# tsy935/eeg-gnn-ssl

Hardware: AMD Instinct MI355X
Metric: EEG clips/sec (60s, 19ch, K=2, 2-layer x64) fwd+bwd (higher is better)
Workload: dtype f32

## Files before the change

eeg_gnn_ssl_amd/_lib.py:

```python
from __future__ import annotations

import ctypes
import os
from ctypes import POINTER, c_char_p, c_float, c_int, c_int32, c_int64, c_size_t, c_void_p

_HERE = os.path.dirname(os.path.abspath(__file__))
HIP_LIB_PATH = os.path.join(_HERE, "libeeg_dcrnn_hip.so")
DEV_LIB_PATH = os.path.join(_HERE, "libeeg_dcrnn_hip_dev.so")
ABI_VERSION = 5


class LayerDims(ctypes.Structure):
    _fields_ = [("T", c_int32), ("B", c_int32), ("N", c_int32), ("H", c_int32), ("Fin", c_int32),
                ("M", c_int32), ("act", c_int32), ("p_batched", c_int32), ("x_planes_ready", c_int32),
                ("x_batch_major", c_int32), ("x_plane_stride", c_int64), ("pack3", c_void_p), ("spectral", c_void_p),
                ("spack", c_void_p)]


class DecoderDims(ctypes.Structure):
    _fields_ = [("T", c_int32), ("B", c_int32), ("N", c_int32), ("H", c_int32), ("Dout", c_int32),
                ("M", c_int32), ("L", c_int32), ("act", c_int32), ("p_batched", c_int32), ("dropout_p", c_float),
                ("teacher_on_device", c_int32)]


# ... 39 lines not shown
    "eeg_dcrnn_decoder_bwd_ws_floats": (c_size_t, [POINTER(DecoderDims)]),
    "eeg_dcrnn_decoder_is_persistent": (c_int, [POINTER(DecoderDims)]),
    "eeg_dcrnn_decoder_fwd": (c_int, [POINTER(DecoderDims), _FP, c_void_p, _FP, _FP, POINTER(c_void_p), _FP, _FP,
                                      _FP, _FP, _FP, _FP, c_void_p]),
    "eeg_dcrnn_decoder_bwd": (c_int, [POINTER(DecoderDims), c_void_p, _FP, POINTER(c_void_p), _FP, _FP, _FP, _FP, _FP,
                                      POINTER(c_void_p), POINTER(c_void_p), POINTER(c_void_p), POINTER(c_void_p),
                                      _FP, _FP, _FP, c_void_p]),
    "eeg_dcrnn_teacher_flags": (c_int, [_FP, _FP, c_int64, ctypes.c_double, c_int, _FP, c_void_p]),
    "eeg_dcrnn_fft_features_pair": (c_int, [_FP, _FP, c_int, c_int, c_int, c_int, c_int, _FP, _FP, c_float, c_float, _FP, _FP, _FP, c_void_p]),
    "eeg_dcrnn_augment_features": (c_int, [_FP, _FP, c_int, c_int, c_int, c_int, c_int, _FP, _FP, _FP, _FP, c_void_p]),
    "eeg_dcrnn_window_features": (c_int, [_FP, c_int, c_int, c_int, c_int, _FP, _FP, c_float, c_float, _FP, c_void_p]),
    "eeg_dcrnn_window_features_pair": (c_int, [_FP, _FP, c_int, c_int, c_int, c_int, c_int, _FP, _FP, c_float, c_float, _FP, _FP, c_void_p]),
    "eeg_dcrnn_augment_windows": (c_int, [_FP, _FP, c_int, c_int, c_int, c_int, c_int, _FP, _FP, _FP, _FP, _FP, c_void_p]),
    "eeg_dcrnn_corr_graph_rows_ws_floats": (c_size_t, [c_int, c_int, c_int]),
    "eeg_dcrnn_corr_graph_rows": (c_int, [_FP, c_int, c_int, c_int, c_int, ctypes.c_longlong, c_int, _FP, _FP, _FP, _FP, c_void_p]),
    "eeg_dcrnn_fft_features_len": (c_int, [_FP, c_int, c_int, c_int, c_int, _FP, _FP, c_float, c_float, _FP, c_float, _FP, _FP, c_void_p]),
    "eeg_dcrnn_window_features_len": (c_int, [_FP, c_int, c_int, c_int, c_int, _FP, _FP, c_float, c_float, _FP, c_float, _FP, c_void_p]),
    "eeg_dcrnn_corr_graph_len": (c_int, [_FP, c_int, c_int, c_int, c_int, c_int, _FP, _FP, _FP, _FP, _FP, c_void_p]),
    "eeg_dcrnn_corr_graph_rows_len": (c_int, [_FP, c_int, c_int, c_int, c_int, ctypes.c_longlong, c_int, _FP, c_int, _FP, _FP, _FP, _FP, c_void_p]),
    "eeg_dcrnn_augment_draw": (c_int, [_FP, c_int, c_int, _FP, _FP, _FP, _FP, _FP, _FP, c_int, _FP, c_void_p]),
    "eeg_dcrnn_epoch_keys": (c_int, [ctypes.c_uint64, c_int64, c_int64, _FP, c_void_p]),
    "eeg_dcrnn_gather_clips": (c_int, [_FP, _FP, c_size_t, _FP, _FP, c_size_t, _FP, _FP, c_int, _FP, _FP, _FP, c_int64, c_int64, _FP, c_int, c_int,
                                       c_int, c_void_p]),
    "eeg_dcrnn_gather_clips_tail": (c_int, [_FP, _FP, c_size_t, _FP, _FP, c_size_t, _FP, _FP, c_int, _FP, _FP, _FP, c_int64, c_int64, _FP, c_int, c_int,
                                            c_int, _FP, _FP, _FP, c_void_p]),
    "eeg_dcrnn_cls_head_loss_w": (c_int, [_FP, _FP, _FP, _FP, c_int, c_int, c_int, c_int, c_int, c_float, _FP, _FP, _FP, _FP, _FP, _FP, _FP, _FP, _FP,
                                          _FP, _FP, c_void_p]),
    "eeg_dcrnn_bce_logits_w": (c_int, [_FP, _FP, c_int, _FP, _FP, _FP, _FP, c_void_p]),
    "eeg_dcrnn_ce_logits_w": (c_int, [_FP, _FP, c_int, c_int, _FP, _FP, _FP, _FP, c_void_p]),
    "eeg_dcrnn_masked_loss_w": (c_int, [_FP, _FP, c_size_t, c_int, _FP, _FP, c_int, c_float, c_float, c_float, c_int, _FP, _FP, _FP, c_void_p]),
    "eeg_dcrnn_teacher_flags_dev": (c_int, [_FP, _FP, _FP, ctypes.c_double, c_int, _FP, c_void_p]),
    "eeg_dcrnn_pack_cells": (c_int, [c_int, POINTER(c_void_p), POINTER(c_void_p), POINTER(c_void_p), POINTER(c_void_p), POINTER(ctypes.c_int32),
                             c_int, c_int, POINTER(c_void_p), _FP, c_int, POINTER(c_void_p), c_void_p]),
    "eeg_dcrnn_cls_head_loss_ws_floats": (c_size_t, [c_int, c_int, c_int]),
    "eeg_dcrnn_cls_head_loss": (c_int, [_FP, _FP, _FP, _FP, c_int, c_int, c_int, c_int, c_int, c_float, _FP, _FP, _FP, _FP, _FP, _FP, _FP, _FP, _FP,
                                c_void_p]),
    "eeg_dcrnn_gather_last": (c_int, [_FP, _FP, c_int, c_int, c_int, _FP, c_void_p]),
    "eeg_dcrnn_rng_take": (c_int, [_FP, ctypes.c_uint64, _FP, c_void_p]),
    "eeg_dcrnn_cls_head_fwd": (c_int, [_FP, _FP, _FP, c_int, c_int, c_int, c_int, c_float, _FP, _FP, _FP, c_void_p]),
    "eeg_dcrnn_cls_head_bwd": (c_int, [_FP, _FP, _FP, _FP, c_int, c_int, c_int, c_int, c_float, _FP, _FP, _FP, _FP, c_void_p]),
    "eeg_dcrnn_dropout_mask": (c_int, [_FP, c_size_t, c_float, _FP, c_void_p]),
    "eeg_dcrnn_bce_logits": (c_int, [_FP, _FP, c_int, _FP, _FP, c_void_p]),
    "eeg_dcrnn_ce_logits": (c_int, [_FP, _FP, c_int, c_int, _FP, _FP, c_void_p]),
    "eeg_dcrnn_masked_loss_ws_floats": (c_size_t, []),
    "eeg_dcrnn_masked_loss": (c_int, [_FP, _FP, c_size_t, c_int, c_float, c_float, c_float, c_int, _FP, _FP, _FP, c_void_p]),
    "eeg_dcrnn_clip_adam_ws_floats": (c_size_t, []),
    "eeg_dcrnn_clip_adam": (c_int, [_FP, _FP, _FP, _FP, c_size_t, c_float, c_float, c_float, c_float, c_float, c_float,
                                    c_int, c_float, _FP, _FP, c_void_p]),
    "eeg_dcrnn_clip_adam_dev": (c_int, [_FP, _FP, _FP, _FP, c_size_t, c_float, _FP, c_float, c_float, c_float, c_float,
                                        _FP, c_float, _FP, _FP, c_void_p]),
}


_SIGNATURES_DEV = {
    "eeg_dcrnn_set_seq_probe": (c_int, [_FP]),
    "eeg_dcrnn_set_tuning": (c_int, [c_int, c_int]),
}


class EegDcrnnError(RuntimeError):
    """Raised when a library call reports an error (shape/dtype/launch problems)."""


class EegDcrnnLib:
    def __init__(self, path: str = HIP_LIB_PATH, strict: bool = True):
        if not os.path.exists(path):
            raise ImportError(
                f"{path} not found: the MI355X HIP library is not built. Run `python -c 'import "
                f"__graft_entry__ as g; g.build()'` (or `make -C eeg_gnn_ssl_amd/csrc`). There is no CPU fallback.")
        self.path = path
# ... 43 lines not shown
```

eeg_gnn_ssl_amd/csrc/api.cpp:

```cpp
#include <atomic>
#include <cmath>
#include <cstdarg>
#include <cstdio>
#include <cstring>

#include <string>
#include <vector>

#include "../../include/eeg_dcrnn.h"
#include "../../include/eeg_dcrnn_dev.h"
#include "../../include/eeg_dcrnn_prof.h"
#include "kernels_decoder.h"
#include "kernels_diffuse.h"
#include "kernels_data.h"
#include "kernels_feat.h"
#include "kernels_gemm.h"
#include "kernels_gemm_bf.h"
#include "kernels_graph.h"
#include "kernels_head.h"
#include "kernels_pack.h"
#include "spec_common.h"
#include "spec_launch.h"
#include "kernels_tail.h"
#include "prof.h"
// ... 345 lines not shown
    size_t rs = h_stride;
    if (rpl == nullptr) {
        if (diffuse_fwd(RHs, P, d->p_batched, S, d->B, N, H, M, rpl_ws, st)) return 1;
        rpl = rpl_ws;
        rs = (size_t)R * H;
    }
    SegPtrs sr;
    for (int m = 0; m < kMaxM; ++m) sr.p[m] = m == 0 ? RHs : (m < M ? rpl + (size_t)(m - 1) * rs : nullptr);
    if (w.pair) {
        if (launch_tnq_pair(w.thg.q, w.thc.q, sh, sr, M, H, R, dXW, 3 * H, 0, 2 * H, part_g, 2 * H, H, part_c, st, "gemm_tn_h"))
            return fail("gemm_tnq_pair: launch failed");
    } else {
        if (gemm_tn(w.thg, w.chg, sh, dXW, 3 * H, 0, part_g, st, "gemm_tn_hg")) return 1;
        if (gemm_tn(w.thc, w.chc, sr, dXW, 3 * H, 2 * H, part_c, st, "gemm_tn_hc")) return 1;
    }
    ReduceJobs jobs;
    const int Ks[3] = {M * Fin, M * H, M * H}, Os[3] = {3 * H, 2 * H, H}, ns[3] = {w.tx.nsplit, w.thg.nsplit, w.thc.nsplit};
    const float* parts[3] = {part, part_g, part_c};
    int nblocks = 0;
    for (int j = 0; j < 3; ++j) {
        jobs.part[j] = parts[j]; jobs.nsplit[j] = ns[j]; jobs.K[j] = Ks[j]; jobs.O[j] = Os[j];
        jobs.nblocks[j] = ceil_div(Ks[j] * Os[j], 64);
        nblocks += jobs.nblocks[j];
    }
    jobs.bias_part = bias_part; jobs.bias_B = d->B; jobs.dbg = dbg; jobs.dbc = dbc;
    if (bias_part != nullptr) nblocks += ceil_div(3 * H, 16);
    EEG_LAUNCH_P("reduce_unpack", reduce_unpack3_kernel, dim3(nblocks), dim3(256), 256 * sizeof(float4), st, jobs, acc, Fin, H, M, dWg, dWc);
    return check_launch("reduce_unpack");
}

size_t xs_spec(const eeg_layer_dims* d) { return d->x_plane_stride > 0 ? (size_t)d->x_plane_stride : 0; }
int cell_weight_grads_spectral(const eeg_layer_dims* d, const float* Xh, size_t x_gs, const float* hh, size_t hh_gs, const float* rhh,
                               const float* dYh, float* part, const BwdWs& w, float* dWg, float* dWc, hipStream_t st,
                               const float* bias_part, float* dbg, float* dbc) {
    const int S = d->T * d->B, H = d->H, M = d->M, Fin = d->Fin, N = d->N, Sp = spec_rows(S);
    float* part_g = part + (w.part_g - w.partial);
    float* part_c = part + (w.part_c - w.partial);
    const SpecTnPlan& g = w.gs;
    if (spec_plan_error("weight gradients (spectral)", g.error)) return 1;
    if (g.fused) {
        if (launch_tnf(g, Xh, x_gs, Fin, hh, hh_gs, rhh, dYh, Sp, N, part, part_g, part_c, st, "gemm_tn_f")) return fail("gemm_tnf: launch failed");
    } else {
        if (launch_tng(g, Xh, x_gs, Fin, Sp, N, dYh, part, st, "gemm_tn_x")) return fail("gemm_tng: launch failed");
        if (launch_tng_pair(g, hh, hh_gs, rhh, Sp, N, dYh, part_g, part_c, st, "gemm_tn_h")) return fail("gemm_tng_pair: launch failed");
    }
    ReduceJobs jobs{};
    SpecFoldJobs sj{};
    sj.basis = d->spectral; sj.N = N;
    sj.j[0] = SpecFoldJob{part, g.spg_x, Fin, 3 * H, ceil_div(Fin * 3 * H, 64)};
    sj.j[1] = SpecFoldJob{part_g, g.spg_h, H, 2 * H, ceil_div(H * 2 * H, 64)};
    sj.j[2] = SpecFoldJob{part_c, g.spg_h, H, H, ceil_div(H * H, 64)};
    int nblocks = sj.j[0].nblocks + sj.j[1].nblocks + sj.j[2].nblocks;
    jobs.bias_part = bias_part; jobs.bias_B = d->B; jobs.dbg = dbg; jobs.dbc = dbc;
    if (bias_part != nullptr) nblocks += ceil_div(3 * H, 16);
    const int ns_max = N * (g.spg_x > g.spg_h ? g.spg_x : g.spg_h);
    const size_t fold_lds = spec_fold_lds_bytes(M, ns_max);
    EEG_SET_MAX_LDS(reduce_unpack3s_kernel, fold_lds);
    EEG_LAUNCH_P("reduce_unpack", reduce_unpack3s_kernel, dim3(nblocks), dim3(256), fold_lds, st, jobs, sj, 0, Fin, H, M, dWg, dWc);
    return check_launch("reduce_unpack (spectral)");
}

int colsum_rows_per_chunk(int R) { int rpc = ceil_div(R, 512); return rpc < 64 ? 64 : rpc; }
size_t colsum_ws(int R, int C) { return (size_t)ceil_div(R, colsum_rows_per_chunk(R)) * C; }
int colsum(const float* A, int R, int C, int split, float* ws, float* out0, float* out1, hipStream_t st) {
    const int rpc = colsum_rows_per_chunk(R), nchunk = ceil_div(R, rpc);
    if (C % 4 == 0 && C <= 1024) {
        const int nrs = 256 / (C / 4);
        EEG_LAUNCH_P("reduce_bias", colsum_partial4_kernel, dim3(nchunk), dim3(256), (size_t)nrs * C * sizeof(float), st, A, R, C, rpc, ws);
    } else {
        EEG_LAUNCH_P("reduce_bias", colsum_partial_kernel, dim3(nchunk, ceil_div(C, 128)), dim3(256), 256 * sizeof(float), st, A, R, C, rpc, ws);
    }
    if (check_launch("colsum_partial")) return 1;
    EEG_LAUNCH_P("reduce_bias", colsum_final_kernel, dim3(ceil_div(C, 128)), dim3(128), 0, st, ws, nchunk, C, split, out0, out1);
    return check_launch("colsum_final");
}

struct DecLayout {
    size_t xin, proj_pack, proj_bias, hd, saved_total;
    size_t planes[8], hext[8], rs[8], us[8], cs[8], rhs[8], hpl[8], rpl[8];
    size_t dxw[8], dbias[8], dotot, da, dhn, z, partial, projt_pack, colsum, bwd_total;
    TnCall cp;
    TnPlan tp;
    BwdWs lw[8];
    eeg_layer_dims ld[8];
};
size_t align64(size_t v) { return (v + 63) / 64 * 64; }
DecLayout dec_layout(const eeg_decoder_dims* d) {
    DecLayout y;
    const size_t state = (size_t)d->B * d->N * d->H, R = (size_t)d->T * d->B * d->N;
    const int nct_o = ceil_div(d->Dout, 16), nct_h = ceil_div(d->H, 16);
    size_t o = 0;
// ... 171 lines not shown
    if (N < 1 || N > kMaxNodes || F < 4 || F % 4 != 0 || M < 1 || M > kMaxM) return fail("diffuse_adj: bad dims N=%d F=%d M=%d", N, F, M);
    if (S < 1 || B < 1) return fail("diffuse_adj: empty input (S=%d, B=%d)", S, B);
    return diffuse_adj(Z, P, p_batched, S, B, N, F, M, dX, S_(stream));
}

static bool layer_dims_positive(const eeg_layer_dims* d) {
    return d != nullptr && d->T >= 1 && d->B >= 1 && d->N >= 1 && d->H >= 1 && d->Fin >= 1 && d->M >= 1;
}
size_t eeg_dcrnn_layer_fwd_ws_floats(const eeg_layer_dims* d) {
    if (!layer_dims_positive(d)) return 0;
    const size_t xw = (size_t)d->T * d->B * d->N * 3 * d->H;
    return d->spectral != nullptr ? xw + (size_t)d->N * spec_rows(d->T * d->B) * 3 * d->H : xw;
}

size_t eeg_dcrnn_spectral_basis_floats(int N) { return (N >= 1 && N <= kMaxNodes) ? (size_t)spec_basis_floats(N) : 0; }
size_t eeg_dcrnn_spectral_rows(size_t S) { return (S + 15) / 16 * 16; }
int eeg_dcrnn_spectral_basis(const float* support, int N, float* basis, void* stream) {
    if (N < 2 || N > kMaxNodes) return fail("spectral_basis: num_nodes=%d unsupported (2..%d)", N, kMaxNodes);
    if (support == nullptr || basis == nullptr) return fail("spectral_basis: null pointer");
    if (launch_spec_basis(support, N, basis, S_(stream))) return fail("spectral_basis: launch failed");
    return check_launch("spectral_basis");
}
size_t eeg_dcrnn_spectral_pack_floats(int Fin, int H, int M, int N) {
    return (Fin >= 4 && Fin % 4 == 0 && H == 64 && M >= 1 && M <= kMaxM && N >= 1 && N <= kMaxNodes) ? spec_pack_floats(Fin, H, M, N) : 0;
}
int eeg_dcrnn_pack_cell_spectral(const float* Wg, const float* Wc, const float* basis, int Fin, int H, int M, int N, float* spack,
                                 void* stream) {
    if (eeg_dcrnn_spectral_pack_floats(Fin, H, M, N) == 0)
        return fail("pack_cell_spectral: input_dim=%d rnn_units=%d hop matrices=%d nodes=%d: the spectral form exists for 64 units", Fin, H, M, N);
    if (Wg == nullptr || Wc == nullptr || basis == nullptr || spack == nullptr) return fail("pack_cell_spectral: null pointer");
    if (launch_spec_pack(Wg, Wc, basis, Fin, H, M, N, spack, S_(stream))) return fail("pack_cell_spectral: launch failed");
    return check_launch("pack_cell_spectral");
}
int eeg_dcrnn_pack_cells(int n_cells, const float* const* Wg, const float* const* bg, const float* const* Wc, const float* const* bc,
                         const int32_t* Fin, int H, int M, float* const* packs, const float* basis, int N, float* const* spacks,
                         void* stream) {
    if (n_cells < 1 || n_cells > 4) return fail("pack_cells: %d cells (1..4 per launch)", n_cells);
    if (Wg == nullptr || bg == nullptr || Wc == nullptr || bc == nullptr || Fin == nullptr || packs == nullptr) return fail("pack_cells: null pointer table");
    if (!seq_h_supported(H)) return fail("pack_cells: rnn_units=%d unsupported", H);
    if (!seq_m_supported(M)) return fail("pack_cells: num hop matrices M=%d unsupported (1,2,3,4,5,7)", M);
    if ((basis == nullptr) != (spacks == nullptr)) return fail("pack_cells: the per-frequency packs need the basis block and their output table");
    int fin[4];
    for (int c = 0; c < n_cells; ++c) {
        fin[c] = Fin[c];
        if (fin[c] < 4 || fin[c] % 4 != 0) return fail("pack_cells: input dim %d of cell %d must be a positive multiple of 4", fin[c], c);
        if (Wg[c] == nullptr || bg[c] == nullptr || Wc[c] == nullptr || bc[c] == nullptr || packs[c] == nullptr || (spacks != nullptr && spacks[c] == nullptr))
            return fail("pack_cells: null pointer in the tables of cell %d", c);
        if (spacks != nullptr && eeg_dcrnn_spectral_pack_floats(fin[c], H, M, N) == 0)
            return fail("pack_cells: input_dim=%d rnn_units=%d hop matrices=%d nodes=%d: the spectral form exists for 64 units", fin[c], H, M, N);
    }
    if (launch_pack_cells(n_cells, Wg, bg, Wc, bc, fin, H, M, packs, basis, N, spacks, S_(stream))) return fail("pack_cells: launch failed");
    return check_launch("pack_cells");
}
int eeg_dcrnn_spectral_ok(const eeg_layer_dims* d, int need_dx) {
    if (!layer_dims_positive(d) || d->p_batched) return 0;
    if (d->x_planes_ready && d->Fin != d->H) return 0;
    if (check_dims(d->N, d->H, d->Fin, d->M)) return 0;
    return spec_supported(d->T, d->B, d->N, d->H, d->Fin, d->M, need_dx) ? 1 : 0;
}

int eeg_dcrnn_batch_major_ok(const eeg_layer_dims* d) {
    if (!diffuse_streams(d->p_batched, d->T * d->B, d->B, d->N, d->Fin)) return 0;
    const int R = d->T * d->B * d->N;
    const GemmKnobs k = gemm_knobs();
    return (nn_dma_applies(d->Fin, R, 3 * d->H, k) && tn_dma_applies(d->Fin, 3 * d->H, k)) ? 2 : 1;
}

int eeg_dcrnn_layer_fwd(const eeg_layer_dims* d, const float* X, float* Xtm, const float* h0, const float* P,
                        const float* pack, float* planes, float* Hext, float* Rs, float* Us, float* Cs, float* RHs,
                        float* Hplanes, float* RHplanes, float* ws, void* stream) {
    if (check_dims(d->N, d->H, d->Fin, d->M)) return 1;
    if (d->T < 1 || d->B < 1) return fail("layer_fwd: empty sequence/batch (T=%d, B=%d)", d->T, d->B);
    const bool save = Rs != nullptr;
    if (save != (Us != nullptr) || save != (Cs != nullptr) || save != (RHs != nullptr))
        return fail("layer_fwd: Rs/Us/Cs/RHs must be all NULL or all non-NULL");
    hipStream_t st = S_(stream);
    const int S = d->T * d->B, R = S * d->N, H = d->H, M = d->M, Fin = d->Fin;
    const size_t state = (size_t)d->B * d->N * H;
    CellPack p = make_cell_pack(Fin, H, M);
    if (h0 != nullptr && h0 != Hext && copy_floats(Hext, h0, state, st)) return 1;
    const size_t xs = d->x_plane_stride > 0 ? (size_t)d->x_plane_stride : (size_t)R * Fin;
    BtMap bt;
    if (d->x_batch_major) {
        if (Xtm != nullptr || d->x_planes_ready) return fail("layer_fwd: x_batch_major excludes Xtm and x_planes_ready");
        if (d->spectral == nullptr && eeg_dcrnn_batch_major_ok(d) != 2) return fail("layer_fwd: x_batch_major is not available for this shape (eeg_dcrnn_batch_major_ok)");
        bt.T = d->T; bt.B = d->B; bt.N = d->N;
    }
    float* XW = ws;
    if (d->spectral != nullptr) {
        if (!eeg_dcrnn_spectral_ok(d, 0)) return fail("layer_fwd: the spectral form does not cover this shape (eeg_dcrnn_spectral_ok)");
        if (Xtm != nullptr || d->spack == nullptr) return fail("layer_fwd: spectral excludes Xtm and needs spack");
        if ((Hplanes != nullptr) != (RHplanes != nullptr)) return fail("layer_fwd: Hplanes/RHplanes must be both NULL or both non-NULL");
        const SpecPack sp = make_spec_pack(Fin, H, M, d->N);
        const int N = d->N, Sp = spec_rows(S), SpE = d->B + Sp;
        const size_t xgs = d->x_plane_stride > 0 ? (size_t)d->x_plane_stride : (size_t)Sp * Fin;
        float* Yh = ws + (size_t)R * 3 * H;
        if (!d->x_planes_ready && spec_mix(1, X, d->spectral, N, d->T, d->B, Fin, d->x_batch_major ? 1 : 0, planes, st, "spec_mix_x")) return 1;
        const SpecNnPlan nn = spec_nn_plan(Fin, Sp, N, sp.nct_x, num_cus(), spec_knobs());
        if (spec_plan_error("layer_fwd (spectral x-part)", nn.error)) return 1;
        const bool regs = nn.kind == SpecNnKind::Regs;
        if (launch_spec_nn(nn, planes, xgs, Fin, Sp, N, d->spack + (regs ? sp.sxr : sp.sxq), regs ? sp.sxr_stride : sp.sxq_stride, Yh, st, "gemm_nn_xw",
                           pack + p.bias, d->spectral + spec_csum_offset(N))) return fail("gemm_nn (spectral): launch failed");
        SeqFwdArgs a{XW, h0 != nullptr ? Hext : nullptr, P, d->p_batched, pack + p.bhg, pack + p.bhc, Hext + state, Rs, Us, Cs, RHs, nullptr, nullptr,
                     (size_t)0, d->T, d->B, N, d->act, seq_probe_arg(st)};
        SeqCall call = seq_fwd_call(H, M, N, d->T, d->B, 0, a.probe);
        call.spectral = true; call.Sp = Sp; call.SpE = SpE;
        const SeqPlan plan = seq_fwd_plan(call);
        if (plan.kind == SeqKind::TwoWaveSpec) {
            a.XW = Yh; a.Hpl = Hplanes; a.RHpl = RHplanes; a.spec_U = d->spectral; a.spec_Sp = Sp; a.spec_SpE = SpE;
            if (seq_fwd(H, M, plan, a, st)) return 1;
            if (Hplanes != nullptr) {
                if (launch_spec_zero_rows(Hplanes, N, (d->T + 1) * d->B, SpE, H, st)) return fail("spec_zero_rows: launch failed");
                if (launch_spec_zero_pad(RHplanes, N, S, H, st)) return fail("spec_zero_pad: launch failed");
            }
        } else {
            if (spec_mix(0, Yh, d->spectral, N, d->T, d->B, 3 * H, 0, XW, st, "spec_mix_y")) return 1;
            if (seq_fwd(H, M, plan, a, st)) return 1;
            if (Hplanes != nullptr) {
                if (spec_mix(1, Hext, d->spectral, N, d->T + 1, d->B, H, 0, Hplanes, st, "spec_mix_h", SpE)) return 1;
                if (spec_mix(1, RHs, d->spectral, N, d->T, d->B, H, 0, RHplanes, st, "spec_mix_h")) return 1;
            }
        }
        return check_launch("layer_fwd (spectral)");
    } else if (d->x_planes_ready) {
        if (Xtm != nullptr) return fail("layer_fwd: x_planes_ready excludes a batch-major input");
    } else {
        if (diffuse_fwd(X, P, d->p_batched, S, d->B, d->N, Fin, M, planes, st, xs, d->x_batch_major ? 2 : (Xtm != nullptr ? 1 : 0), Xtm)) return 1;
        if (Xtm != nullptr) X = Xtm;
    }
    SegPtrs segs;
    for (int m = 0; m < kMaxM; ++m) segs.p[m] = m == 0 ? X : (m < M ? planes + (size_t)(m - 1) * xs : nullptr);
    const bool bf3 = d->pack3 != nullptr && pack3_supported(Fin, H, M);
    const Pack3 q = make_pack3(Fin, H, M);
    const NnCall cxw = nn_call(M, Fin, R, 3 * H / 16, 3 * H, 3 * H, bt, p.has_bxq, bf3 ? q.xw_nct : 0);
    if (gemm_nn(gemm_nn_plan(cxw), cxw, segs, NnRhs{pack + p.bx, pack + p.bxq, bf3 ? d->pack3 + q.xw : nullptr}, pack + p.bias, XW, st, "gemm_nn_xw", bt)) return 1;
    if ((Hplanes != nullptr) != (RHplanes != nullptr)) return fail("layer_fwd: Hplanes/RHplanes must be both NULL or both non-NULL");
    SeqFwdArgs a{XW, h0 != nullptr ? Hext : nullptr, P, d->p_batched, pack + p.bhg, pack + p.bhc, Hext + state, Rs, Us, Cs, RHs, Hplanes, RHplanes,
                 (size_t)(d->T + 1) * state, d->T, d->B, d->N, d->act, seq_probe_arg(st)};
    return seq_fwd(H, M, seq_fwd_plan(seq_fwd_call(H, M, d->N, d->T, d->B, a.plane_stride, a.probe)), a, st);
}

size_t eeg_dcrnn_layer_bwd_ws_floats(const eeg_layer_dims* d, int need_dx) { return layer_dims_positive(d) ? bwd_ws(d, need_dx).total : 0; }

int eeg_dcrnn_layer_bwd(const eeg_layer_dims* d, const float* X, const float* P, const float* pack,
                        const float* planes, const float* Hext, const float* Rs, const float* Us, const float* Cs,
                        const float* RHs, const float* Hplanes, const float* RHplanes, const float* dHseq,
// ... 11 lines not shown
    float* dbias = ws + w.dbias;
    SeqBwdArgs a{Hext + state, Hext, Rs, Us, Cs, dHseq, d_at_end, d_at_len,
                 reinterpret_cast<const long long*>(lengths), P, d->p_batched, pack + p.b1, pack + p.b2,
                 dXW, dh0, dbias, d->T, d->B, N, d->act, seq_probe_arg(st)};
    SeqCall call = seq_bwd_call(H, M, N, d->T, d->B, a.probe);
    call.spectral = d->spectral != nullptr; call.Sp = spec_rows(S); call.SpE = d->B + spec_rows(S);
    const SeqPlan plan = seq_bwd_plan(call);
    const bool dyh_done = plan.kind == SeqKind::TwoWaveSpec;
    if (dyh_done) { a.spec_U = d->spectral; a.dYh = ws + w.dyh; a.spec_Sp = call.Sp; }
    if (seq_bwd(H, M, plan, a, st)) return 1;
    const size_t xs = d->x_plane_stride > 0 ? (size_t)d->x_plane_stride : (size_t)R * Fin;
    BtMap bt;
    if (d->x_batch_major) {
        if (d->spectral == nullptr && eeg_dcrnn_batch_major_ok(d) != 2) return fail("layer_bwd: x_batch_major is not available for this shape");
        bt.T = d->T; bt.B = d->B; bt.N = N;
    }
    if (d->spectral != nullptr) {
        if (!eeg_dcrnn_spectral_ok(d, dX != nullptr)) return fail("layer_bwd: the spectral form does not cover this shape (eeg_dcrnn_spectral_ok)");
        if (d->spack == nullptr) return fail("layer_bwd: spectral needs spack");
        if ((Hplanes != nullptr) != (RHplanes != nullptr)) return fail("layer_bwd: Hplanes/RHplanes must be both NULL or both non-NULL");
        const SpecPack sp = make_spec_pack(Fin, H, M, N);
        const int Sp = spec_rows(S), SpE = d->B + Sp;
        float* dYh = ws + w.dyh;
        if (dyh_done) {
            if (launch_spec_zero_pad(dYh, N, S, 3 * H, st)) return fail("spec_zero_pad: launch failed");
        } else if (spec_mix(1, dXW, d->spectral, N, d->T, d->B, 3 * H, 0, dYh, st, "spec_mix_dy")) return 1;
        const float *hh = Hplanes, *rhh = RHplanes;
        size_t hh_gs = (size_t)SpE * H;
        if (hh == nullptr) {
            if (spec_mix(1, Hext, d->spectral, N, d->T, d->B, H, 0, ws + w.hplanes, st, "spec_mix_h")) return 1;
            if (spec_mix(1, RHs, d->spectral, N, d->T, d->B, H, 0, ws + w.rhplanes, st, "spec_mix_h")) return 1;
            hh = ws + w.hplanes; rhh = ws + w.rhplanes; hh_gs = 0;
        }
        if (cell_weight_grads_spectral(d, planes, xs_spec(d), hh, hh_gs, rhh, dYh, ws + w.partial, w, dWg, dWc, st, dbias, dbg, dbc)) return 1;
        if (dX != nullptr) {
            const SpecDxPlan dx = spec_dx_plan(Fin, N, d->T, d->B, num_cus(), spec_knobs());
            if (spec_plan_error("layer_bwd (spectral dX)", dx.error)) return 1;
            if (dx.kind == SpecDxKind::Fused) {
                if (launch_dxf(dx, dYh, Sp, S, N, d->spack + sp.sxtq, sp.sxtq_stride, d->spectral, dX, st, "gemm_dx_f")) return fail("gemm_dxf: launch failed");
            } else {
                float* dXh = ws + w.z;
                if (launch_spec_nn(dx.nn, dYh, 0, 3 * H, Sp, N, d->spack + sp.sxtq, sp.sxtq_stride, dXh, st, "gemm_nn_dx")) return fail("gemm_nng: launch failed");
                if (launch_spec_mix(dx.mix, dXh, d->spectral, N, d->T, d->B, Fin, 0, dX, st, "spec_mix_dx")) return fail("spec_mix: launch failed");
            }
        }
        return check_launch("layer_bwd (spectral)");
    }
    if (cell_weight_grads(d, X, planes, xs, Hext, RHs, dXW, P, Hplanes, RHplanes, (size_t)(d->T + 1) * state,
                          ws + w.hplanes, ws + w.rhplanes, ws + w.partial, w, false, dWg, dWc, st, bt, dbias, dbg, dbc)) return 1;
    if (dX != nullptr) {
        float* Z = ws + w.z;
        SegPtrs sd;
        for (int m = 0; m < kMaxM; ++m) sd.p[m] = m == 0 ? dXW : nullptr;
        const bool bf3 = d->pack3 != nullptr && pack3_supported(Fin, H, M);
        const Pack3 q = make_pack3(Fin, H, M);
        const NnCall cdx = nn_call(1, 3 * H, R, round_up(M * Fin, 16) / 16, M * Fin, M * Fin, BtMap(), p.has_bxtq, bf3 ? q.dx_nct : 0);
        if (gemm_nn(gemm_nn_plan(cdx), cdx, sd, NnRhs{pack + p.bxt, pack + p.bxtq, bf3 ? d->pack3 + q.dx : nullptr}, nullptr, Z, st, "gemm_nn_dx")) return 1;
        if (diffuse_adj(Z, P, d->p_batched, S, d->B, N, Fin, M, dX, st)) return 1;
    }
    return 0;
}


static int fft_features(const float* raw, int B, int N, int T, int W, const int32_t* perm, const float* log_scale, float mean, float std_,
                        const int64_t* lengths, float pad_val, float* feat_raw, float* feat_std, void* stream) {
    const long long* len = reinterpret_cast<const long long*>(lengths);
    if (B < 1 || N < 1 || T < 1) return fail("fft_features: empty input (B=%d, N=%d, T=%d)", B, N, T);
    if (W < 4 || W % 4 != 0 || W / 4 + 1 > 64) return fail("fft_features: window=%d unsupported (multiple of 4, <= 252)", W);
    if (feat_raw == nullptr && feat_std == nullptr) return fail("fft_features: no output requested");
    if (feat_std != nullptr && !(std_ != 0.f)) return fail("fft_features: std must be non-zero");
    if (W == kFftWin) {
        const long long n_windows = (long long)B * N * T;
// ... 661 lines not shown
        dz == nullptr || dW == nullptr || dbias == nullptr || loss == nullptr || ws == nullptr)
        return fail("cls_head_loss: null pointer");
    const int O = C * H + C, nblk = ceil_div(B, 4);
    const size_t lds = (size_t)(4 * cls_tail_wave_floats(N, H, C) + 4 * (O + 1)) * sizeof(float);
    if (lds > kMaxLdsBytes) return fail("cls_head_loss: N=%d x (classes=%d + rnn_units=%d) floats of four clips do not fit the %zu-byte LDS", N, C, H, (size_t)kMaxLdsBytes);
    if (clip_w != nullptr) {
        EEG_SET_MAX_LDS(cls_head_loss_w_kernel, lds);
        EEG_LAUNCH_P("cls_head_loss", cls_head_loss_w_kernel, dim3(nblk), dim3(256), lds, S_(stream), z, W, bias, targets, kind, B, N, H, C, drop,
                     reinterpret_cast<const unsigned long long*>(rng_used), clip_w, denom, logits, reinterpret_cast<int*>(arg), dlogits, dz, ws);
        if (check_launch("cls_head_loss_w")) return 1;
        EEG_LAUNCH_P("cls_head_loss", cls_head_loss_w_finish_kernel, dim3(1), dim3(256), 0, S_(stream), ws, nblk, denom, H, C, dW, dbias, loss);
        return check_launch("cls_head_loss_w_finish");
    }
    EEG_SET_MAX_LDS(cls_head_loss_kernel, lds);
    EEG_LAUNCH_P("cls_head_loss", cls_head_loss_kernel, dim3(nblk), dim3(256), lds, S_(stream), z, W, bias, targets, kind, B, N, H, C, drop,
                 reinterpret_cast<const unsigned long long*>(rng_used), logits, reinterpret_cast<int*>(arg), dlogits, dz, ws);
    if (check_launch("cls_head_loss")) return 1;
    EEG_LAUNCH_P("cls_head_loss", cls_head_loss_finish_kernel, dim3(1), dim3(256), 0, S_(stream), ws, nblk, B, H, C, dW, dbias, loss);
    return check_launch("cls_head_loss_finish");
}
int eeg_dcrnn_cls_head_loss(const float* z, const float* W, const float* bias, const void* targets, int kind, int B, int N, int H, int C,
                            float dropout_p, const uint64_t* rng_used, float* logits, int32_t* arg, float* dlogits, float* dz,
                            float* dW, float* dbias, float* loss, float* ws, void* stream) {
    return cls_head_loss_launch(z, W, bias, targets, kind, B, N, H, C, dropout_p, rng_used, nullptr, nullptr, logits, arg, dlogits, dz, dW, dbias,
                                loss, ws, stream);
}
int eeg_dcrnn_cls_head_loss_w(const float* z, const float* W, const float* bias, const void* targets, int kind, int B, int N, int H, int C,
                              float dropout_p, const uint64_t* rng_used, const float* clip_w, const float* denom, float* logits, int32_t* arg,
                              float* dlogits, float* dz, float* dW, float* dbias, float* loss, float* ws, void* stream) {
    if (clip_w == nullptr || denom == nullptr) return fail("cls_head_loss_w: null clip_w / denom");
    return cls_head_loss_launch(z, W, bias, targets, kind, B, N, H, C, dropout_p, rng_used, clip_w, denom, logits, arg, dlogits, dz, dW, dbias,
                                loss, ws, stream);
}
size_t eeg_dcrnn_dconv_fwd_ws_floats(int B, int N, int F, int M, int O) {
    if (B < 1 || N < 1 || F < 1 || M < 1 || O < 1) return 0;
    return (size_t)(M - 1) * B * N * F + (size_t)F * M * O;
}
int eeg_dcrnn_dconv_fwd(const float* X, const float* P, int p_batched, int B, int N, int F, int M,
                        const float* W, const float* bias, int O, float* out, float* ws, void* stream) {
    if (N < 1 || N > kMaxNodes || F < 4 || F % 4 != 0 || M < 1 || M > kMaxM) return fail("dconv_fwd: bad dims N=%d F=%d M=%d", N, F, M);
    if (B < 1) return fail("dconv_fwd: empty batch (B=%d)", B);
    if (O % 16 != 0) return fail("dconv_fwd: output_dim=%d must be a multiple of 16", O);
    hipStream_t st = S_(stream);
    float* planes = ws;
    float* pack = ws + (size_t)(M - 1) * B * N * F;
    if (diffuse_fwd(X, P, p_batched, B, B, N, F, M, planes, st)) return 1;
    EEG_LAUNCH_P("pack_dense", pack_dense_kernel, dim3(256), dim3(256), 0, st, W, F, M, O, pack);
    if (check_launch("pack_dense")) return 1;
    SegPtrs segs;
    for (int m = 0; m < kMaxM; ++m) segs.p[m] = m == 0 ? X : (m < M ? planes + (size_t)(m - 1) * B * N * F : nullptr);
    return gemm_nn(segs, M, F, B * N, pack, O / 16, bias, out, O, O, st);
}
size_t eeg_dcrnn_dconv_bwd_ws_floats(int B, int N, int F, int M, int O) {
    if (B < 1 || N < 1 || F < 1 || M < 1 || O < 1) return 0;
    const int R = B * N;
    const int nsplit = gemm_tn_plan(tn_call(M, F, R, O)).nsplit;
    return (size_t)(M - 1) * R * F + align64((size_t)nsplit * M * F * O) + align64((size_t)(O / 4) * (round_up(M * F, 16) / 16) * 64)
           + (size_t)R * M * F + align64(colsum_ws(R, O));
}
int eeg_dcrnn_dconv_bwd(const float* X, const float* P, int p_batched, int B, int N, int F, int M, const float* W, int O,
                        const float* dOut, float* dX, float* dW, float* dbias, float* ws, void* stream) {
    if (N < 1 || N > kMaxNodes || F < 4 || F % 4 != 0 || M < 1 || M > kMaxM) return fail("dconv_bwd: bad dims N=%d F=%d M=%d", N, F, M);
    if (B < 1) return fail("dconv_bwd: empty batch (B=%d)", B);
    if (O % 16 != 0 || O > 192) return fail("dconv_bwd: output_dim=%d must be a multiple of 16 (<= 192)", O);
    hipStream_t st = S_(stream);
    const int R = B * N;
// ... 130 lines not shown
```

eeg_gnn_ssl_amd/csrc/kernels_head.h:

```cpp
#pragma once
#include "common.h"

namespace eeg {

__device__ __forceinline__ f32x4 ld4g(const float* p) {
    const float4 v = *reinterpret_cast<const float4*>(p);
    return (f32x4){v.x, v.y, v.z, v.w};
}

__global__ void gather_last_kernel(const float* __restrict__ Htop, const long long* __restrict__ lengths,
                                   int T, int B, int NH, float* __restrict__ last) {
    const size_t total = (size_t)B * NH;
    for (size_t i = (size_t)blockIdx.x * blockDim.x + threadIdx.x; i < total; i += (size_t)gridDim.x * blockDim.x) {
        const int b = i / NH, e = i % NH;
        int t = (int)lengths[b] - 1;
        t = t < 0 ? 0 : (t >= T ? T - 1 : t);
        last[i] = Htop[((size_t)t * B + b) * NH + e];
    }
}

__global__ void cls_head_fwd_kernel(const float* __restrict__ z, const float* __restrict__ W,
                                    const float* __restrict__ bias, int B, int N, int H, int C, DropCfg drop,
                                    const unsigned long long* __restrict__ used, float* __restrict__ logits, int* __restrict__ arg) {
    EEG_DYN_SMEM(sm);
// ... 52 lines not shown
                                      const int* __restrict__ arg, int B, int N, int H, int C, DropCfg drop,
                                      const unsigned long long* __restrict__ used, float* __restrict__ dW,
                                      float* __restrict__ dbias) {
    EEG_DYN_SMEM(sm);
    const int o = threadIdx.x & 15, q = threadIdx.x >> 4;
    const int i = blockIdx.x * 16 + o;
    float s = 0.f;
    if (i < C * H) {
        const int c = i / H, h = i % H;
        for (int b = q; b < B; b += 16) {
            const int n = arg[(size_t)b * C + c];
            const size_t e = ((size_t)b * N + n) * H + h;
            s = fmaf(dlogits[(size_t)b * C + c], fmaxf(z[e], 0.f) * head_mask(drop, used, e), s);
        }
    } else if (i < C * H + C) {
        const int c = i - C * H;
        for (int b = q; b < B; b += 16) s += dlogits[(size_t)b * C + c];
    }
    sm[q * 16 + o] = s;
    __syncthreads();
    if (q == 0 && i < C * H + C) {
        float t = 0.f;
        for (int k = 0; k < 16; ++k) t += sm[k * 16 + o];
        if (i < C * H) dW[i] = t; else dbias[i - C * H] = t;
    }
}

__host__ __device__ inline int cls_tail_wave_floats(int N, int H, int C) { return N * C + N * H + 2 * C; }
template <bool kWeighted>
__device__ __forceinline__ void cls_head_loss_body(const float* __restrict__ z, const float* __restrict__ W, const float* __restrict__ bias,
                                                   const void* __restrict__ targets, int kind, int B, int N, int H, int C, const DropCfg& drop,
                                                   const unsigned long long* __restrict__ used, float* __restrict__ logits,
                                                   int* __restrict__ arg, float* __restrict__ dlogits, float* __restrict__ dz,
                                                   float* __restrict__ partial, const float* __restrict__ clip_w,
                                                   const float* __restrict__ denom) {
    EEG_DYN_SMEM(sm);
    const int w = threadIdx.x >> 6, lane = threadIdx.x & 63, b = blockIdx.x * 4 + w, O = C * H + C;
    float* nl = sm + w * cls_tail_wave_floats(N, H, C);
    float* zs = nl + N * C;
    float* dl = zs + N * H;
    int* ag = reinterpret_cast<int*>(dl + C);
    float* contrib = sm + 4 * cls_tail_wave_floats(N, H, C);
    const bool live = b < B;
    const int groups = N * H / 4;
    if (live) {
        const unsigned long long seed = drop.on ? used[0] : 0ull, off = drop.on ? used[1] : 0ull;
        for (int g = lane; g < groups; g += 64) {
            const size_t gg = (size_t)b * groups + g;
            const f32x4 v = ld4g(z + 4 * gg);
            f32x4 m = {1.f, 1.f, 1.f, 1.f};
            if (drop.on) m = dropout_mask4(seed, off, gg, drop.thr, drop.scale);
#pragma unroll
            for (int j = 0; j < 4; ++j) zs[4 * g + j] = fmaxf(v[j], 0.f) * m[j];
        }
        EEG_WAVE_SYNC();
        if (lane < N) {
            for (int c = 0; c < C; ++c) {
                float s = bias[c];
                for (int h = 0; h < H; ++h) s = fmaf(zs[lane * H + h], W[c * H + h], s);
                nl[lane * C + c] = s;
            }
        }
        EEG_WAVE_SYNC();
        for (int c = lane; c < C; c += 64) {
            float best = nl[c];
            int bi = 0;
            for (int q = 1; q < N; ++q)
                if (nl[q * C + c] > best) { best = nl[q * C + c]; bi = q; }
            logits[(size_t)b * C + c] = best;
            arg[(size_t)b * C + c] = bi;
            dl[c] = best;
            ag[c] = bi;
        }
        EEG_WAVE_SYNC();
        if (lane == 0) {
            float term;
            const float div = kWeighted ? denom[0] : (float)B;
            if (kWeighted && clip_w[b] == 0.f) {
                term = 0.f;
                for (int c = 0; c < C; ++c) dl[c] = 0.f;
            } else if (kind == 0) {
                const float v = dl[0], t = reinterpret_cast<const float*>(targets)[b];
// ... 27 lines not shown
#pragma unroll
            for (int j = 0; j < 4; ++j) o[j] = zs[4 * g + j] > 0.f ? o[j] * keep : 0.f;
            *reinterpret_cast<float4*>(dz + ((size_t)b * groups + g) * 4) = make_float4(o[0], o[1], o[2], o[3]);
        }
        for (int i = lane; i < O; i += 64) {
            float v;
            if (i < C * H) { const int c = i / H, h = i % H; v = dl[c] * zs[ag[c] * H + h]; }
            else v = dl[i - C * H];
            contrib[w * (O + 1) + i] = v;
        }
    }
    __syncthreads();
    const int nlive = B - blockIdx.x * 4 < 4 ? B - blockIdx.x * 4 : 4;
    for (int i = threadIdx.x; i <= O; i += blockDim.x) {
        float s = 0.f;
        for (int q = 0; q < nlive; ++q) s += contrib[q * (O + 1) + i];
        partial[(size_t)blockIdx.x * (O + 1) + i] = s;
    }
}
__global__ __launch_bounds__(256) void cls_head_loss_kernel(const float* __restrict__ z, const float* __restrict__ W, const float* __restrict__ bias,
                                                            const void* __restrict__ targets, int kind, int B, int N, int H, int C, DropCfg drop,
                                                            const unsigned long long* __restrict__ used, float* __restrict__ logits,
                                                            int* __restrict__ arg, float* __restrict__ dlogits, float* __restrict__ dz,
                                                            float* __restrict__ partial) {
    cls_head_loss_body<false>(z, W, bias, targets, kind, B, N, H, C, drop, used, logits, arg, dlogits, dz, partial, nullptr, nullptr);
}
__global__ __launch_bounds__(256) void cls_head_loss_w_kernel(const float* __restrict__ z, const float* __restrict__ W, const float* __restrict__ bias,
                                                              const void* __restrict__ targets, int kind, int B, int N, int H, int C, DropCfg drop,
                                                              const unsigned long long* __restrict__ used, const float* __restrict__ clip_w,
                                                              const float* __restrict__ denom, float* __restrict__ logits, int* __restrict__ arg,
                                                              float* __restrict__ dlogits, float* __restrict__ dz, float* __restrict__ partial) {
    cls_head_loss_body<true>(z, W, bias, targets, kind, B, N, H, C, drop, used, logits, arg, dlogits, dz, partial, clip_w, denom);
}
__device__ __forceinline__ void cls_head_loss_finish_body(const float* __restrict__ partial, int nblk, float div, int H, int C,
                                                          float* __restrict__ dW, float* __restrict__ dbias, float* __restrict__ loss) {
    const int O = C * H + C;
    for (int i = threadIdx.x; i <= O; i += blockDim.x) {
        float s = 0.f;
        int q = 0;
        for (; q + 8 <= nblk; q += 8) {
            float v[8];
#pragma unroll
            for (int u = 0; u < 8; ++u) v[u] = partial[(size_t)(q + u) * (O + 1) + i];
#pragma unroll
            for (int u = 0; u < 8; ++u) s += v[u];
        }
        for (; q < nblk; ++q) s += partial[(size_t)q * (O + 1) + i];
        if (i < C * H) dW[i] = s;
        else if (i < O) dbias[i - C * H] = s;
        else loss[0] = s / div;
    }
}
__global__ __launch_bounds__(256) void cls_head_loss_finish_kernel(const float* __restrict__ partial, int nblk, int B, int H, int C,
                                                                   float* __restrict__ dW, float* __restrict__ dbias, float* __restrict__ loss) {
    cls_head_loss_finish_body(partial, nblk, (float)B, H, C, dW, dbias, loss);
}
__global__ __launch_bounds__(256) void cls_head_loss_w_finish_kernel(const float* __restrict__ partial, int nblk, const float* __restrict__ denom,
                                                                     int H, int C, float* __restrict__ dW, float* __restrict__ dbias,
                                                                     float* __restrict__ loss) {
    cls_head_loss_finish_body(partial, nblk, denom[0], H, C, dW, dbias, loss);
}

__global__ void rng_take_kernel(unsigned long long* __restrict__ state, unsigned long long* __restrict__ used, unsigned long long groups) {
    if (blockIdx.x == 0 && threadIdx.x == 0) {
        const unsigned long long seed = state[0], off = state[1];
        used[0] = seed;
        used[1] = off;
        state[1] = off + groups;
    }
}
__device__ __forceinline__ void teacher_flags_body(unsigned long long* __restrict__ state, long long* __restrict__ seen, long long inc,
                                                   double decay_steps, int T, int* __restrict__ flags) {
    const unsigned long long seed = state[0], off = state[1];
    const long long n = seen[0];
    const double ratio = decay_steps / (decay_steps + exp((double)n / decay_steps));
    for (int t0 = 0; t0 < T; t0 += 4) {
        unsigned w[4];
        const unsigned long long c = off + (unsigned long long)(t0 >> 2);
        philox4x32_10((unsigned)c, (unsigned)(c >> 32), 0u, 0u, (unsigned)seed, (unsigned)(seed >> 32), w);
        for (int j = 0; j < 4 && t0 + j < T; ++j) flags[t0 + j] = ((double)w[j] * (1.0 / 4294967296.0) < ratio) ? 1 : 0;
    }
    state[1] = off + (unsigned long long)((T + 3) / 4);
    seen[0] = n + inc;
}
__global__ void teacher_flags_kernel(unsigned long long* __restrict__ state, long long* __restrict__ seen, long long inc,
                                     double decay_steps, int T, int* __restrict__ flags) {
    if (blockIdx.x != 0 || threadIdx.x != 0) return;
    teacher_flags_body(state, seen, inc, decay_steps, T, flags);
}
__global__ void teacher_flags_dev_kernel(unsigned long long* __restrict__ state, long long* __restrict__ seen, const long long* __restrict__ inc,
                                         double decay_steps, int T, int* __restrict__ flags) {
    if (blockIdx.x != 0 || threadIdx.x != 0) return;
    teacher_flags_body(state, seen, inc[0], decay_steps, T, flags);
// ... 22 lines not shown
```

eeg_gnn_ssl_amd/csrc/kernels_seq.h:

```cpp
#pragma once
#include "common.h"
#include "lds_diffuse.h"

namespace eeg {

constexpr int seq_nks(int N) { return N <= 20 ? 5 : 8; }
constexpr bool seq_has_two_wave(int H, int M, int nks) { return H == 64 && nks == 5 && M <= 3; }
constexpr bool seq_has_spec(int H, int M, int nks) { return seq_has_two_wave(H, M, nks) && M >= 2; }
constexpr bool seq_has_probe(int H, int M, int nks) { return kDevBuild && H == 64 && M == 3 && nks == 5; }
constexpr bool seq_has_stream(int H, int M) { return H == 64 && M <= 5; }

template <int H, int M>
struct SeqGeom {
    static constexpr int KA = M * H, KAP = lds_stride_x(KA), KS = KA / 4;
    static constexpr int KG = M * 2 * H, KGP = lds_stride_x(KG), KSG = KG / 4;
    static constexpr int NGT = 2 * H / 16, NCT = H / 16;
    static constexpr int GT = ceil_div(NGT, 4), CT = ceil_div(NCT, 4);
};
constexpr size_t seq_fwd_lds_floats(int H, int M) { return (size_t)(M - 1) * kPFloats + 2 * 32 * lds_stride_x(M * H); }
constexpr size_t seq_fwd2_lds_floats(int H, int M, bool spec) {
    return seq_fwd_lds_floats(H, M) + 16 * 64 + (spec ? 3 * 16 * 64 + 4 * 64 + 4 * (M * H / 4 / 4) * 256 : 0);
}
constexpr size_t seq_bwd_lds_floats(int H, int M, int rows) {
    return (size_t)(M - 1) * kPFloats + (size_t)rows * (lds_stride_x(M * H) + lds_stride_x(M * 2 * H));
// ... 478 lines not shown
        }
        pp.mark(5);
        if (t + 1 < T || Hpl != nullptr) diffuse_own(A, Hpl, t + 1);
        pp.mark(6);
    }
    }
    pp.dump(probe, 0);
}

template <int H, int M, int NKS, bool PROBE = false, bool SPEC = false>
__global__ __launch_bounds__(512, 1) void seq_fwd2_kernel(
    const float* __restrict__ XW, const float* __restrict__ h0, const float* __restrict__ P, int p_batched,
    const float* __restrict__ bhg, const float* __restrict__ bhc,
    float* __restrict__ Hseq, float* __restrict__ Rs, float* __restrict__ Us, float* __restrict__ Cs,
    float* __restrict__ RHs, float* __restrict__ Hpl, float* __restrict__ RHpl, size_t plane_stride,
    int T, int B, int N, int act, long long* probe, const float* __restrict__ spec_U = nullptr, int spec_Sp = 0, int spec_SpE = 0) {
    using G = SeqGeom<H, M>;
    PhaseProbe<PROBE> pp;
    pp.start();
    static_assert(G::CT == 1 && NKS == 5, "one column tile per wave, second node tile on the 4x4x1 MFMA");
    constexpr int KAP = G::KAP, KS = G::KS, NGT = G::NGT, NCT = G::NCT, UST = 64;
    EEG_DYN_SMEM(sm);
    float* Pl = sm;
    float* A = Pl + (M - 1) * kPFloats;
    float* A2 = A + 32 * KAP;
    const int tid = threadIdx.x, lane = tid & 63, wave8 = SPEC ? wave_uniform(tid >> 6) : (tid >> 6), role = wave8 >> 2, wave = wave8 & 3;
    const int lr = lane & 15, lg = lane >> 4;
    float* U = A2 + 32 * KAP;
    float* XR = U + 16 * UST;
    float* XC = XR + 16 * UST;
    float* XRr = XC + 2 * 16 * UST;
    float* W1L = XRr + 4 * 64;
    const bool save = Rs != nullptr;
    const int ct = wave;
    const wbuf_t bH = make_wbuf(Hseq), bR = make_wbuf(save ? Rs : Hseq), bU = make_wbuf(save ? Us : Hseq),
                 bC = make_wbuf(save ? Cs : Hseq), bRH = make_wbuf(save ? RHs : Hseq);

    float w0[1][KS], w1[1][KS];
#pragma unroll
    for (int ks = 0; ks < KS; ++ks) w0[0][ks] = bhg[((size_t)ks * NGT + (role == 0 ? ct : NCT + ct)) * 64 + lane];
    if (!SPEC || role == 0) {
#pragma unroll
        for (int ks = 0; ks < KS; ++ks) w1[0][ks] = bhc[((size_t)ks * NCT + ct) * 64 + lane];
    } else {
#pragma unroll
        for (int q = 0; q < KS / 4; ++q) {
            f32x4 v;
#pragma unroll
            for (int j = 0; j < 4; ++j) v[j] = bhc[((size_t)(4 * q + j) * NCT + ct) * 64 + lane];
            st4(W1L + (ct * (KS / 4) + q) * 256 + 4 * lane, v);
        }
    }
    auto clip = [&](const int b, auto ROLE_T) __attribute__((always_inline)) {
    constexpr int ROLE_C = decltype(ROLE_T)::value;
    __syncthreads();
    for (int e = tid; e < 2 * 32 * KAP; e += 512) A[e] = 0.f;
    lds_load_polys(Pl, P, p_batched ? b : 0, M, N);
    __syncthreads();
    if (h0 != nullptr) {
        for (int e = tid; e < N * H; e += 512) A[lds_sw(e / H, e % H, KAP)] = h0[(size_t)b * N * H + e];
    } else {
        for (int e = tid; e < N * H; e += 512) (Hseq - (size_t)B * N * H)[(size_t)b * N * H + e] = 0.f;
    }
    __syncthreads();

    const bool valid[2] = {lr < N, 16 + lr < N};
// ... 32 lines not shown
        cs.begin(probe, cs_me);
        constexpr int QSA = KS / 4 / M;
        f32x4 rc[5] = {zero4, zero4, zero4, zero4, zero4};
        f32x4 ra = zero4;
        bool pre_r = false;
        for (int t = 0; t < T; ++t) {
            const size_t s = (size_t)t * B + b;
            f32x4 ar[1][2] = {{nxr0, (f32x4){nxr1, 0.f, 0.f, 0.f}}}, ac[1][2] = {{nxc, zero4}};
            const unsigned so = (unsigned)(s * N * H);
            EEG_LDS_BARRIER();
            pp.mark(0);
            if constexpr (SPEC) {
                ar[0][0] = ld4(XR + lds_sw(lr, col, UST));
                ar[0][1][0] = XRr[ct * 64 + lane];
                if (M > 1 && pre_r) ra += ar[0][0];
            }

            if (M > 1 && pre_r) {
                ar[0][0] = ra;
                mfma_nodes32<1, KS, true, 0, 0, false, true, true, (M > 1 ? QSA : 0)>(A, KAP, lane, lr, lg, w0, ar, rc);
            } else
                mfma_nodes32<1, KS, true, 0, 0, false, true, true>(A, KAP, lane, lr, lg, w0, ar);
            pp.mark(1);
            {
                const f32x4 rg = sigmoid4_(ar[0][0]);
                f32x4 rh = rg * ld4(A + lds_sw(lr, col, KAP));
                rh = valid[0] ? rh : zero4;
                st4(A2 + lds_sw(lr, col, KAP), rh);
                const float rg1 = sigmoidf_(ar[0][1][0]);
                const float rh1 = valid1 ? rg1 * A[l1] : 0.f;
                A2[l1] = rh1;
                if (save && valid[0]) {
                    wbuf_st4(bR, oh0, so, rg);
                    wbuf_st4(bRH, oh0, so, rh);
                }
                if (save && valid1) {
                    wbuf_st1(bR, oh1, so, rg1);
                    wbuf_st1(bRH, oh1, so, rh1);
                }
            }
            pp.mark(2);
            diffuse_own(A2, RHpl, t);
            pp.mark(7);
            EEG_LDS_BARRIER();
            pp.mark(3);
            if (t + 1 < T) fetch_xw(t + 1);
            if constexpr (SPEC) ac[0][0] = ld4(XC + (t & 1) * (16 * UST) + lds_sw(lr, col, UST));
            mfma_nodes32<1, KS, true, 1>(A2, KAP, lane, lr, lg, w1, ac);
            pp.mark(4);
            {
                const f32x4 u = ld4(U + lds_sw(lr, col, UST)), h = ld4(A + lds_sw(lr, col, KAP));
                const f32x4 c = act == 0 ? tanh4_(ac[0][0]) : relu4_(ac[0][0]);
                f32x4 hn = u * h + (1.f - u) * c;
                hn = valid[0] ? hn : zero4;
                st4(A + lds_sw(lr, col, KAP), hn);
                if (valid[0]) {
                    wbuf_st4(bH, oh0, so, hn);
                    if (save) wbuf_st4(bC, oh0, so, c);
                }
            }
            pp.mark(5);
            EEG_LDS_BARRIER();
            if (t + 1 < T || (!SPEC && Hpl != nullptr)) diffuse_own(A, Hpl, t + 1);
            pre_r = M > 1 && t + 1 < T;
            if (pre_r) {
                ra = SPEC ? zero4 : nxr0;
                rc[0] = rc[1] = rc[2] = rc[3] = rc[4] = zero4;
                f32x4 rr4[4] = {zero4, zero4, zero4, zero4};
                mfma_tile_quads<KS, 0, QSA>(A, KAP, lane, lr, lg, w0[0], ra, rc[4], rr4);
                rc[0] = rr4[0]; rc[1] = rr4[1]; rc[2] = rr4[2]; rc[3] = rr4[3];
            }
// ... 690 lines not shown
```

eeg_gnn_ssl_amd/csrc/kernels_spectral.h:

```cpp
#pragma once
#include "spec_common.h"
#include "spec_launch.h"

namespace eeg {

__global__ __launch_bounds__(256) void spectral_basis_kernel(const float* __restrict__ S, int N, float* __restrict__ out) {
    EEG_DYN_SMEM(sm);
    double* A = reinterpret_cast<double*>(sm);
    double* V = A + 32 * 32;
    double* cs = V + 32 * 32;
    int* pq = reinterpret_cast<int*>(cs + 32);
    double* red = reinterpret_cast<double*>(pq + 32);
    const int tid = threadIdx.x;
    const int NP = (N + 1) & ~1, NH = NP / 2;
    for (int e = tid; e < 32 * 32; e += 256) {
        const int i = e >> 5, j = e & 31;
        A[e] = (i < N && j < N) ? 0.5 * ((double)S[i * N + j] + (double)S[j * N + i]) : 0.0;
        V[e] = i == j ? 1.0 : 0.0;
    }
    __syncthreads();
    for (int sweep = 0; sweep < kSpecSweeps; ++sweep) {
        for (int r = 0; r < NP - 1; ++r) {
            if (tid < NH) {
                int p = tid == 0 ? NP - 1 : (r + tid) % (NP - 1);
// ... 211 lines not shown
#pragma unroll
        for (int v = 0; v < 16; ++v) acc[v] = bv;
        if (r < S) {
            float b[KS];
#pragma unroll
            for (int ks = 0; ks < KS; ++ks) {
                int k = 2 * ks + hh;
                if (k >= N) k = N - 1;
                b[ks] = DIR == 0 ? in[(s * N + k) * F + fc] : in[((size_t)k * Sp + r) * F + fc];
            }
#pragma unroll
            for (int ks = 0; ks < KS; ++ks) acc = mfma32(a[ks], b[ks], acc);
        }
        if (f < F) {
#pragma unroll
            for (int v = 0; v < 16; ++v) {
                const int o = 8 * (v >> 2) + 4 * hh + (v & 3);
                if (2 * KS <= 8 * (v >> 2)) continue;
                if (o < N) {
                    if (DIR == 0) out[((size_t)o * Sp + r) * F + f] = acc[v];
                    else out[(s * N + o) * F + f] = acc[v];
                }
            }
        }
    }
}

__global__ void spec_zero_pad_kernel(float* __restrict__ Xh, int N, int S, int Sp, int F) {
    const int per = (Sp - S) * F, total = N * per;
    for (int e = blockIdx.x * blockDim.x + threadIdx.x; e < total; e += gridDim.x * blockDim.x) {
        const int i = e / per, r = e - i * per;
        Xh[((size_t)i * Sp + S) * F + r] = 0.f;
    }
}

__global__ __launch_bounds__(256) void spec_mix_generic_kernel(const float* __restrict__ in, const float* __restrict__ basis,
                                                              const float* __restrict__ bias, int N, int S, int Sp, int F, int map,
                                                              int T, int B, int to_nodes, float* __restrict__ out) {
    EEG_DYN_SMEM(sm);
    for (int e = threadIdx.x; e < N * N; e += blockDim.x) sm[e] = basis[e];
    __syncthreads();
    const int F4 = F / 4;
    const size_t total = (size_t)(to_nodes ? Sp : S) * N * F4;
    for (size_t e = (size_t)blockIdx.x * blockDim.x + threadIdx.x; e < total; e += (size_t)gridDim.x * blockDim.x) {
        const int c4 = (int)(e % F4), o = (int)((e / F4) % N);
        const size_t r = e / ((size_t)F4 * N);
        const size_t s = r < (size_t)S ? spec_sample(r, map, T, B) : r;
        float4 a = make_float4(0.f, 0.f, 0.f, 0.f);
        if (to_nodes) {
            if (r < (size_t)S) {
                for (int n = 0; n < N; ++n) {
                    const float u = sm[n * N + o];
                    const float4 x = reinterpret_cast<const float4*>(in)[(s * N + n) * F4 + c4];
                    a.x = fmaf(u, x.x, a.x); a.y = fmaf(u, x.y, a.y); a.z = fmaf(u, x.z, a.z); a.w = fmaf(u, x.w, a.w);
                }
            }
            reinterpret_cast<float4*>(out)[((size_t)o * Sp + r) * F4 + c4] = a;
        } else {
            if (bias != nullptr) a = reinterpret_cast<const float4*>(bias)[c4];
            for (int i = 0; i < N; ++i) {
                const float u = sm[o * N + i];
                const float4 y = reinterpret_cast<const float4*>(in)[((size_t)i * Sp + r) * F4 + c4];
                a.x = fmaf(u, y.x, a.x); a.y = fmaf(u, y.y, a.y); a.z = fmaf(u, y.z, a.z); a.w = fmaf(u, y.w, a.w);
            }
            reinterpret_cast<float4*>(out)[(s * N + o) * F4 + c4] = a;
        }
// ... 5 lines not shown
```

eeg_gnn_ssl_amd/csrc/pack_cell.h:

```cpp
#pragma once
#include "common.h"
#include "nnq_order.h"

namespace eeg {

struct CellPack {
    int Fin, H, M;
    size_t bx;
    size_t bias;
    size_t bhg;
    size_t bhc;
    size_t b1;
    size_t b2;
    size_t bxt;
    size_t c1;
    size_t c2;
    size_t bxq;
    size_t bxtq;
    bool has_bxq, has_bxtq;
    size_t total;
};

__host__ __device__ inline CellPack make_cell_pack(int Fin, int H, int M) {
    CellPack p;
    p.Fin = Fin; p.H = H; p.M = M;
    size_t o = 0;
    p.bx = o;   o += (size_t)M * Fin * 3 * H;
    p.bias = o; o += (size_t)round_up(3 * H, 64);
    p.bhg = o;  o += (size_t)M * H * 2 * H;
    p.bhc = o;  o += (size_t)M * H * H;
    p.b1 = o;   o += (size_t)M * H * H;
    p.b2 = o;   o += (size_t)M * 2 * H * H;
    p.bxt = o;  o += (size_t)3 * H * round_up(M * Fin, 16);
    p.c1 = o;   o += (size_t)M * H * cell_pack_cx_cols(Fin, H);
    p.c2 = o;   o += (size_t)M * 2 * H * cell_pack_cx_cols(Fin, H);
    p.has_bxq = (3 * H) % 192 == 0;
    p.has_bxtq = (M * Fin) % 192 == 0 && (3 * H) % 4 == 0 && make_nnq_order(1, 3 * H).ntail <= 2;
    p.bxq = o;  o += p.has_bxq ? (size_t)round_up(make_nnq_order(M, Fin).nch, 4) * (3 * H / 16) * 256 : 0;
    p.bxtq = o; o += p.has_bxtq ? (size_t)make_nnq_order(1, 3 * H).nch * (M * Fin / 16) * 256 : 0;
    p.total = o;
    return p;
}

__device__ __forceinline__ float ref_wg(const float* Wg, int M, int H, int f_all, int m, int o) {
    return Wg[((size_t)f_all * M + m) * (2 * H) + o];
}
__device__ __forceinline__ float ref_wc(const float* Wc, int M, int H, int f_all, int m, int o) {
    return Wc[((size_t)f_all * M + m) * H + o];
}

__device__ __forceinline__ void pack_cell_body(const float* __restrict__ Wg, const float* __restrict__ bg,
                                               const float* __restrict__ Wc, const float* __restrict__ bc,
                                               float* __restrict__ out, const CellPack& p, int bid, int nb) {
    const int Fin = p.Fin, H = p.H, M = p.M;
    const size_t stride = (size_t)nb * blockDim.x;
    for (size_t idx = (size_t)bid * blockDim.x + threadIdx.x; idx < p.total; idx += stride) {
        float v = 0.f;
        if (idx < p.bias) {
            const size_t e = idx - p.bx;
            const int lane = e & 63, nct = 3 * H / 16;
            const int ct = (e >> 6) % nct, ks = (e >> 6) / nct;
            const int k = 4 * ks + (lane >> 4), j = 16 * ct + (lane & 15);
            const int m = k / Fin, f = k % Fin;
            v = j < 2 * H ? ref_wg(Wg, M, H, f, m, j) : ref_wc(Wc, M, H, f, m, j - 2 * H);
        } else if (idx < p.bhg) {
            const int j = idx - p.bias;
            v = j < 2 * H ? bg[j] : (j < 3 * H ? bc[j - 2 * H] : 0.f);
        } else if (idx < p.bhc) {
            const size_t e = idx - p.bhg;
            const int lane = e & 63, nct = 2 * H / 16;
            const int ct = (e >> 6) % nct, ks = (e >> 6) / nct;
            const int k = kperm(ks, lane >> 4), j = 16 * ct + (lane & 15);
            v = ref_wg(Wg, M, H, Fin + k % H, k / H, j);
        } else if (idx < p.b1) {
            const size_t e = idx - p.bhc;
            const int lane = e & 63, nct = H / 16;
            const int ct = (e >> 6) % nct, ks = (e >> 6) / nct;
            const int k = kperm(ks, lane >> 4), j = 16 * ct + (lane & 15);
            v = ref_wc(Wc, M, H, Fin + k % H, k / H, j);
        } else if (idx < p.b2) {
            const size_t e = idx - p.b1;
            const int lane = e & 63, nct = H / 16;
            const int ct = (e >> 6) % nct, ks = (e >> 6) / nct;
            const int k = kperm(ks, lane >> 4), f = 16 * ct + (lane & 15);
            v = ref_wc(Wc, M, H, Fin + f, k / H, k % H);
        } else if (idx < p.bxt) {
            const size_t e = idx - p.b2;
            const int lane = e & 63, nct = H / 16;
            const int ct = (e >> 6) % nct, ks = (e >> 6) / nct;
// ... 40 lines not shown
```

eeg_gnn_ssl_amd/csrc/platform.h:

```cpp
#pragma once
#include <hip/hip_runtime.h>

typedef float f32x4 __attribute__((ext_vector_type(4)));
typedef float f32x2 __attribute__((ext_vector_type(2)));
#define EEG_DYN_SMEM(name) extern __shared__ __attribute__((aligned(16))) float name[]
#define EEG_LAUNCH(kern, grid, block, smem, stream, ...) \
    hipLaunchKernelGGL(kern, (grid), (block), (smem), (stream), __VA_ARGS__)
#define EEG_SET_MAX_LDS(kern, bytes) \
    (void)hipFuncSetAttribute(reinterpret_cast<const void*>(kern), hipFuncAttributeMaxDynamicSharedMemorySize, (int)(bytes))
__device__ __forceinline__ f32x4 mfma16(float a, float b, f32x4 c) {
    return __builtin_amdgcn_mfma_f32_16x16x4f32(a, b, c, 0, 0, 0);
}
__device__ __forceinline__ f32x4 mfma4(float a, float b, f32x4 c) {
    return __builtin_amdgcn_mfma_f32_4x4x1f32(a, b, c, 0, 0, 0);
}
typedef float f32x16 __attribute__((ext_vector_type(16)));
__device__ __forceinline__ f32x16 mfma32(float a, float b, f32x16 c) {
    return __builtin_amdgcn_mfma_f32_32x32x2f32(a, b, c, 0, 0, 0);
}
typedef short bf16x8 __attribute__((ext_vector_type(8)));
typedef unsigned u32x4 __attribute__((ext_vector_type(4)));
__device__ __forceinline__ f32x4 mfma_bf16(bf16x8 a, bf16x8 b, f32x4 c) {
    return __builtin_amdgcn_mfma_f32_16x16x32_bf16(a, b, c, 0, 0, 0);
}
// ... 39 lines not shown
    const unsigned long long v = reinterpret_cast<unsigned long long>(p);
    const unsigned lo = __builtin_amdgcn_readfirstlane((unsigned)v), hi = __builtin_amdgcn_readfirstlane((unsigned)(v >> 32));
    return __builtin_amdgcn_make_buffer_rsrc(reinterpret_cast<void*>(((unsigned long long)hi << 32) | lo), 0,
                                             (int)__builtin_amdgcn_readfirstlane(nbytes), 0x00020000);
}
__device__ __forceinline__ float wbuf_ld(wbuf_t b, unsigned voff, unsigned soff) {
    return __builtin_bit_cast(float, __builtin_amdgcn_raw_buffer_load_b32(b, 4u * voff, 4u * soff, 0));
}
__device__ __forceinline__ f32x4 wbuf_ld4(wbuf_t b, unsigned voff, unsigned soff) {
    return __builtin_bit_cast(f32x4, __builtin_amdgcn_raw_buffer_load_b128(b, 4u * voff, 4u * soff, 0));
}
__device__ __forceinline__ void wbuf_st4(wbuf_t b, unsigned voff, unsigned soff, f32x4 v) {
    typedef unsigned u32x4_ __attribute__((ext_vector_type(4)));
    __builtin_amdgcn_raw_buffer_store_b128(__builtin_bit_cast(u32x4_, v), b, 4u * voff, 4u * soff, 0);
}
template <int AUX>
__device__ __forceinline__ void wbuf_st4_aux(wbuf_t b, unsigned voff, unsigned soff, f32x4 v) {
    typedef unsigned u32x4_ __attribute__((ext_vector_type(4)));
    __builtin_amdgcn_raw_buffer_store_b128(__builtin_bit_cast(u32x4_, v), b, 4u * voff, 4u * soff, AUX);
}
__device__ __forceinline__ void wbuf_st2(wbuf_t b, unsigned voff, unsigned soff, float x, float y) {
    typedef unsigned u32x2_ __attribute__((ext_vector_type(2)));
    __builtin_amdgcn_raw_buffer_store_b64((u32x2_){__builtin_bit_cast(unsigned, x), __builtin_bit_cast(unsigned, y)}, b, 4u * voff, 4u * soff, 0);
}
__device__ __forceinline__ void wbuf_st1(wbuf_t b, unsigned voff, unsigned soff, float x) {
    __builtin_amdgcn_raw_buffer_store_b32(__builtin_bit_cast(unsigned, x), b, 4u * voff, 4u * soff, 0);
}
__device__ __forceinline__ void wbuf_dma16(wbuf_t b, float* lds_wave_base, unsigned voff_bytes, unsigned soff_bytes) {
    __builtin_amdgcn_raw_ptr_buffer_load_lds(b, (__attribute__((address_space(3))) void*)lds_wave_base, 16, voff_bytes, soff_bytes, 0, 0);
}

__device__ __forceinline__ unsigned long long atomic_add_u64(unsigned long long* p, unsigned long long v) { return atomicAdd(p, v); }

namespace eeg {
__device__ __forceinline__ float fast_exp(float x) { return __builtin_amdgcn_exp2f(x * 1.44269504088896340736f); }
__device__ __forceinline__ float fast_rcp(float x) { return __builtin_amdgcn_rcpf(x); }
__device__ __forceinline__ float fast_exp2(float x) { return __builtin_amdgcn_exp2f(x); }
__device__ __forceinline__ float fast_log2(float x) { return __builtin_amdgcn_logf(x); }
__device__ __forceinline__ float unfused_mul_add(float a, float b, float c) {
#pragma clang fp contract(off)
    const float p = a * b;
    return p + c;
}

constexpr int kPlatformIsDevice = 1;
inline int platform_num_cus() {
    static int n = 0;
    if (n == 0) {
        int dev = 0, v = 0;
        if (hipGetDevice(&dev) == hipSuccess && hipDeviceGetAttribute(&v, hipDeviceAttributeMultiprocessorCount, dev) == hipSuccess && v > 0) n = v;
        else n = 256;
    }
    return n;
}
inline bool platform_copy_floats(float* dst, const float* src, size_t n, hipStream_t st) {
    return hipMemcpyAsync(dst, src, n * sizeof(float), hipMemcpyDeviceToDevice, st) == hipSuccess;
}
inline bool platform_stream_is_capturing(hipStream_t st) {
    hipStreamCaptureStatus cs = hipStreamCaptureStatusNone;
    return hipStreamIsCapturing(st, &cs) == hipSuccess && cs != hipStreamCaptureStatusNone;
}
}
```

eeg_gnn_ssl_amd/csrc/spec_inst.cpp:

```cpp
#include "kernels_gemm_g.h"
#include "kernels_gemm_f.h"
#include "kernels_spectral.h"
#include "pack_cell.h"
#include "spec_launch.h"
#include "prof.h"

namespace eeg {

constexpr int kMaxPackJobs = 8;
struct PackJob {
    const float *Wg, *bg, *Wc, *bc, *basis;
    float* out;
    int spectral;
    CellPack cp;
    SpecPack sp;
};
struct PackJobs { PackJob j[kMaxPackJobs]; };
__global__ void pack_cells_kernel(PackJobs jobs) {
    const PackJob& jb = jobs.j[blockIdx.y];
    if (jb.spectral) pack_spectral_body(jb.Wg, jb.Wc, jb.basis, jb.out, jb.sp, (int)blockIdx.x, (int)gridDim.x);
    else pack_cell_body(jb.Wg, jb.bg, jb.Wc, jb.bc, jb.out, jb.cp, (int)blockIdx.x, (int)gridDim.x);
}


size_t spec_pack_floats(int Fin, int H, int M, int N) { return make_spec_pack(Fin, H, M, N).total; }

int launch_spec_basis(const float* S, int N, float* basis, hipStream_t st) {
    EEG_SET_MAX_LDS(spectral_basis_kernel, kSpecBasisLds);
    EEG_LAUNCH_P("spec_basis", spectral_basis_kernel, dim3(1), dim3(256), kSpecBasisLds, st, S, N, basis);
    return hipGetLastError() == hipSuccess ? 0 : 2;
}

int launch_spec_pack(const float* Wg, const float* Wc, const float* basis, int Fin, int H, int M, int N, float* spack, hipStream_t st) {
    const SpecPack p = make_spec_pack(Fin, H, M, N);
    EEG_LAUNCH_P("pack_cell", pack_spectral_kernel, dim3(1024), dim3(256), 0, st, Wg, Wc, basis, spack, p);
    return hipGetLastError() == hipSuccess ? 0 : 2;
}

int launch_pack_cells(int n_cells, const float* const* Wg, const float* const* bg, const float* const* Wc, const float* const* bc,
                      const int* Fin, int H, int M, float* const* packs, const float* basis, int N, float* const* spacks, hipStream_t st) {
    PackJobs jobs{};
    int n = 0;
    for (int c = 0; c < n_cells; ++c) {
        if (n + (spacks != nullptr ? 2 : 1) > kMaxPackJobs) return 1;
        PackJob& a = jobs.j[n++];
        a.Wg = Wg[c]; a.bg = bg[c]; a.Wc = Wc[c]; a.bc = bc[c]; a.basis = nullptr; a.out = packs[c]; a.spectral = 0;
        a.cp = make_cell_pack(Fin[c], H, M);
        if (spacks != nullptr) {
            PackJob& b = jobs.j[n++];
            b.Wg = Wg[c]; b.bg = nullptr; b.Wc = Wc[c]; b.bc = nullptr; b.basis = basis; b.out = spacks[c]; b.spectral = 1;
            b.sp = make_spec_pack(Fin[c], H, M, N);
        }
    }
    EEG_LAUNCH_P("pack_cell", pack_cells_kernel, dim3(256, n), dim3(256), 0, st, jobs);
    return hipGetLastError() == hipSuccess ? 0 : 2;
}

int launch_spec_mix(const SpecMixPlan& p, const float* in, const float* basis, int N, int T, int B, int F, int bm, float* out,
                    hipStream_t st, const char* tag) {
    const float* bias = nullptr;
    const dim3 grid(p.grid), block(p.block);
#define EEG_MIX_MFMA(DIR, KS) EEG_LAUNCH_P(tag, (spec_mix_mfma_kernel<DIR, KS>), grid, block, p.lds, st, in, basis, bias, N, p.S, p.Sp, F, bm, T, B, out)
    if (p.kind == SpecMixKind::Mfma) {
        if (p.ks == 10) { if (p.to_nodes) EEG_MIX_MFMA(0, 10); else EEG_MIX_MFMA(1, 10); }
        else { if (p.to_nodes) EEG_MIX_MFMA(0, 16); else EEG_MIX_MFMA(1, 16); }
    } else if (p.kind == SpecMixKind::Valu19) {
        if (p.to_nodes) EEG_LAUNCH_P(tag, spec_mix_in_kernel<19>, grid, block, p.lds, st, in, basis, p.S, p.Sp, F, bm, T, B, out);
        else EEG_LAUNCH_P(tag, spec_mix_out_kernel<19>, grid, block, p.lds, st, in, basis, bias, p.S, p.Sp, F, bm, T, B, out);
    } else {
        EEG_LAUNCH_P(tag, spec_mix_generic_kernel, grid, block, p.lds, st, in, basis, bias, N, p.S, p.Sp, F, bm, T, B, p.to_nodes, out);
    }
#undef EEG_MIX_MFMA
    return hipGetLastError() == hipSuccess ? 0 : 2;
}

int launch_spec_zero_rows(float* Xh, int N, int S, int Sp, int F, hipStream_t st) {
    if (Sp <= S) return 0;
    EEG_LAUNCH_P("zero", spec_zero_pad_kernel, dim3(ceil_div(N * (Sp - S) * F, 256)), dim3(256), 0, st, Xh, N, S, Sp, F);
    return hipGetLastError() == hipSuccess ? 0 : 2;
}

namespace {
template <int KQ, bool SWZ>
void launch_nnf_one(const SpecNnPlan& p, const float* A, size_t ags, int K, int Sp, int G, const float* Wr, size_t wstride, float* C, hipStream_t st,
                    const char* tag, const float* bias, const float* gscale) {
    EEG_SET_MAX_LDS((gemm_nnf_kernel<KQ, SWZ>), p.lds);
    EEG_LAUNCH_P(tag, (gemm_nnf_kernel<KQ, SWZ>), dim3(p.grid), dim3(p.block), p.lds, st, A, (long long)ags, K, Sp, G, Wr, (unsigned)wstride, C, bias, gscale);
}
template <int NJ>
void launch_nng_one(const SpecNnPlan& p, const float* A, size_t ags, int F, int Sp, int G, const float* Wq, size_t wstride, float* C, hipStream_t st,
                    const char* tag, const float* bias, const float* gscale) {
    EEG_SET_MAX_LDS((gemm_nng_kernel<NJ, 2>), p.lds);
    EEG_LAUNCH_P(tag, (gemm_nng_kernel<NJ, 2>), dim3(p.grid), dim3(p.block), p.lds, st, A, (unsigned)ags, F, Sp, G, Wq, (unsigned)wstride, C, 64 * NJ, bias, gscale);
}
}
int launch_spec_nn(const SpecNnPlan& p, const float* A, size_t a_gstride, int K, int Sp, int G, const float* W, size_t wstride, float* C,
                   hipStream_t st, const char* tag, const float* bias, const float* gscale) {
    const size_t ags = a_gstride != 0 ? a_gstride : (size_t)Sp * K;
#define EEG_NNF(KQ, SWZ) launch_nnf_one<KQ, SWZ>(p, A, ags, K, Sp, G, W, wstride, C, st, tag, bias, gscale)
    if (p.kind == SpecNnKind::Regs) {
        switch (p.kq) {
            case 8: EEG_NNF(8, true); break;
            case 13: EEG_NNF(13, false); break;
            case 9: EEG_NNF(9, false); break;
            case 5: EEG_NNF(5, false); break;
            case 2: EEG_NNF(2, false); break;
            default: return 1;
        }
    } else if (p.nj == 3) {
        launch_nng_one<3>(p, A, ags, K, Sp, G, W, wstride, C, st, tag, bias, gscale);
    } else if (p.nj == 1) {
// ... 77 lines not shown
```

eeg_gnn_ssl_amd/csrc/spec_launch.h:

```cpp
#pragma once
#include "common.h"
#include "nnq_order.h"
#include "spec_common.h"

namespace eeg {

struct SpecKnobs {
    int nn_grouped = 0;
    int tn_separate = 0;
    int dx_passes = 0;
};
enum SpecPlanError { kSpecOk = 0, kSpecBadNct, kSpecNotCovered };

inline bool spec_desc_reaches(double floats) { return floats * sizeof(float) < 2147483648.0; }

inline bool spec_supported(int T, int B, int N, int H, int Fin, int M, int need_dx) {
    if (T < 1 || B < 1 || N < 2 || N > kMaxNodes || H != 64 || Fin < 4 || Fin % 4 != 0 || M < 2 || M > kMaxM) return false;
    if (need_dx && Fin != 64) return false;
    if (Fin / 4 > 256 || make_nnq_order(1, Fin).ntail > 1) return false;
    return spec_desc_reaches((double)N * spec_rows(T * B) * (Fin > 192 ? Fin : 192));
}

constexpr size_t kSpecBasisLds = (2 * 32 * 32 + 32 + 256) * sizeof(double) + 32 * sizeof(int);
__host__ __device__ constexpr size_t spec_mix_generic_lds_bytes(int N) { return (size_t)N * N * sizeof(float); }
// ... 154 lines not shown
    int nt;
    int grid, block;
    size_t lds;
    bool needs_dxh;
    SpecNnPlan nn;
    SpecMixPlan mix;
    int error;
};
inline SpecDxPlan spec_dx_plan(int Fin, int N, int T, int B, int num_cus, const SpecKnobs& k) {
    SpecDxPlan p{};
    const int S = T * B, Sp = spec_rows(S);
    if (k.dx_passes == 0 && Fin == 64 && N >= 1 && N <= kDxfMaxN && S >= 1 && spec_desc_reaches((double)Sp * 192) &&
        spec_desc_reaches((double)S * N * 64)) {
        p.kind = SpecDxKind::Fused;
        p.nt = N == 19 ? 19 : 0;
        p.grid = ceil_div(Sp, kDxfRows); p.block = 256;
        p.lds = dxf_lds_bytes();
        return p;
    }
    p.kind = SpecDxKind::TwoPass;
    p.needs_dxh = true;
    SpecKnobs grouped = k;
    grouped.nn_grouped = 1;
    p.nn = spec_nn_plan(192, Sp, N, round_up(Fin, 16) / 16, num_cus, grouped);
    p.mix = spec_mix_plan(0, N, T, B, Fin);
    p.error = p.nn.error;
    return p;
}

size_t spec_pack_floats(int Fin, int H, int M, int N);
int launch_spec_basis(const float* S, int N, float* basis, hipStream_t st);
int launch_spec_pack(const float* Wg, const float* Wc, const float* basis, int Fin, int H, int M, int N, float* spack, hipStream_t st);
int launch_pack_cells(int n_cells, const float* const* Wg, const float* const* bg, const float* const* Wc, const float* const* bc,
                      const int* Fin, int H, int M, float* const* packs, const float* basis, int N, float* const* spacks, hipStream_t st);
int launch_spec_mix(const SpecMixPlan& p, const float* in, const float* basis, int N, int T, int B, int F, int bm, float* out,
                    hipStream_t st, const char* tag);
int launch_spec_zero_rows(float* Xh, int N, int S, int Sp, int F, hipStream_t st);
inline int launch_spec_zero_pad(float* Xh, int N, int S, int F, hipStream_t st) { return launch_spec_zero_rows(Xh, N, S, spec_rows(S), F, st); }
int launch_spec_nn(const SpecNnPlan& p, const float* A, size_t a_gstride, int K, int Sp, int G, const float* W, size_t wstride, float* C,
                   hipStream_t st, const char* tag, const float* bias = nullptr, const float* gscale = nullptr);
int launch_tnf(const SpecTnPlan& p, const float* Xh, size_t x_gstride, int Fin, const float* Hh, size_t h_gstride, const float* RHh,
               const float* dY, int Sp, int G, float* part_x, float* part_g, float* part_c, hipStream_t st, const char* tag);
int launch_tng(const SpecTnPlan& p, const float* A, size_t a_gstride, int F, int Sp, int G, const float* dY, float* partial, hipStream_t st,
               const char* tag);
int launch_tng_pair(const SpecTnPlan& p, const float* Ah, size_t ah_gstride, const float* Arh, int Sp, int G, const float* dY, float* part_g,
                    float* part_c, hipStream_t st, const char* tag);
int launch_dxf(const SpecDxPlan& p, const float* dYh, int Sp, int S, int N, const float* Wtq, size_t wstride, const float* basis, float* dX,
               hipStream_t st, const char* tag);

}
```

eeg_gnn_ssl_amd/model/cell.py:

```python
import math

import torch
import torch.nn as nn

from .. import ops


class DiffusionGraphConv(nn.Module):

    def __init__(self, num_supports, input_dim, hid_dim, num_nodes, max_diffusion_step, output_dim,
                 bias_start=0.0, filter_type="laplacian"):
        super().__init__()
        self._num_matrices = num_supports * max_diffusion_step + 1
        self._input_size = input_dim + hid_dim
        self._input_dim = input_dim
        self._hid_dim = hid_dim
        self._num_nodes = num_nodes
        self._max_diffusion_step = max_diffusion_step
        self._filter_type = filter_type
        self.weight = nn.Parameter(torch.empty(self._input_size * self._num_matrices, output_dim))
        self.biases = nn.Parameter(torch.empty(output_dim))
        nn.init.xavier_normal_(self.weight, gain=1.414)
        nn.init.constant_(self.biases, bias_start)

# ... 17 lines not shown
        self._num_nodes = num_nodes
        self._num_units = num_units
        self._input_dim = input_dim
        self._max_diffusion_step = max_diffusion_step
        self._use_gc_for_ru = use_gc_for_ru
        if not use_gc_for_ru:
            raise NotImplementedError("use_gc_for_ru=False is a stub (`_fc` is `pass`) in the reference as well")
        if max_diffusion_step < 0:
            raise ValueError("max_diffusion_step must be >= 0")
        self._num_supports = 2 if filter_type == "dual_random_walk" else 1
        self._filter_type = filter_type
        common = dict(num_supports=self._num_supports, input_dim=input_dim, hid_dim=num_units,
                      num_nodes=num_nodes, max_diffusion_step=max_diffusion_step, filter_type=filter_type)
        self.dconv_gate = DiffusionGraphConv(output_dim=num_units * 2, **common)
        self.dconv_candidate = DiffusionGraphConv(output_dim=num_units, **common)

    @property
    def output_size(self):
        return self._num_nodes * self._num_units

    @property
    def num_matrices(self):
        return self._num_supports * self._max_diffusion_step + 1

    def _check_supports(self, supports):
        if len(supports) != self._num_supports:
            raise RuntimeError(f"filter_type={self._filter_type!r} expects {self._num_supports} support(s), "
                               f"got {len(supports)}")
        n = self._num_nodes
        for i, s in enumerate(supports):
            if s.dim() not in (2, 3) or s.shape[-1] != n or s.shape[-2] != n:
                raise RuntimeError(f"supports[{i}] has shape {tuple(s.shape)}, expected ({n}, {n}) or (B, {n}, {n})")

    def run_sequence(self, x, h0, p, p_batched, lengths=None, x_off=0, x_planes=None, want_hsel=True, basis=None, pack=None, spack=None):
        return ops.dcgru_layer_ex(x, x_off, h0, p, p_batched, self.dconv_gate.weight, self.dconv_gate.biases,
                                  self.dconv_candidate.weight, self.dconv_candidate.biases,
                                  self._num_nodes, self._num_units, self.num_matrices,
                                  self._activation_name, lengths, x_planes, want_hsel, basis, pack, spack)

    def forward(self, supports, inputs, state):
        self._check_supports(supports)
        b = inputs.shape[0]
        p, p_batched = ops.hop_polys(supports, self._max_diffusion_step, b)
        x = inputs.reshape(1, b, self._num_nodes, self._input_dim)
        new_state = self.run_sequence(x, state, p, p_batched).hsel
        return new_state, new_state

    def init_hidden(self, batch_size):
        return torch.zeros(batch_size, self._num_nodes * self._num_units,
                           device=self.dconv_gate.weight.device)
```

eeg_gnn_ssl_amd/model/model.py:

```python
import random

import torch
import torch.nn as nn

from .. import ops
from .. import utils
from .cell import DCGRUCell


class _FusedDropout:

    def _init_dropout_rng(self, stream_id: int):
        self.register_buffer("_dropout_rng", ops.make_rng_state("cpu", stream_id), persistent=False)
        self._ddp_params_and_buffers_to_ignore = ["_dropout_rng"]

    def _drop_p(self) -> float:
        return float(self.dropout.p) if self.training else 0.0

    def set_dropout_seed(self, seed: int, offset: int = 0):
        st = self._dropout_rng
        st.copy_(torch.tensor([int(seed), int(offset)], dtype=torch.int64), non_blocking=False)

    def dropout_rng_state(self):
        seed, offset = self._dropout_rng.tolist()
        return int(seed), int(offset)

    def _rng_state(self, device) -> torch.Tensor:
        st = self._dropout_rng
        device = torch.device(device)
        if st.device.type != device.type or (device.index is not None and st.device.index != device.index):
            if device.type == "cuda" and torch.cuda.is_current_stream_capturing():
                raise RuntimeError("the fused dropout generator state is not on the device of the inputs: move the model "
                                   "with .to(device) before capturing its forward into a HIP graph")
            st = st.to(device)
            self._buffers["_dropout_rng"] = st
        return st


class DCRNNEncoder(nn.Module):

    def __init__(self, input_dim, max_diffusion_step, hid_dim, num_nodes, num_rnn_layers,
                 dcgru_activation=None, filter_type="laplacian", device=None):
        super().__init__()
        self.hid_dim = hid_dim
        self.num_rnn_layers = num_rnn_layers
        self.num_nodes = num_nodes
        self.max_diffusion_step = max_diffusion_step
        self._device = device
        cells = []
        for layer in range(num_rnn_layers):
            cells.append(DCGRUCell(input_dim=input_dim if layer == 0 else hid_dim, num_units=hid_dim,
                                   max_diffusion_step=max_diffusion_step, num_nodes=num_nodes,
                                   nonlinearity=dcgru_activation, filter_type=filter_type))
        self.encoding_cells = nn.ModuleList(cells)

    def run(self, inputs, initial_hidden_state, supports, lengths=None, want_finals=True):
        t_len, b = inputs.shape[0], inputs.shape[1]
        self.encoding_cells[0]._check_supports(supports)
        p, p_batched = ops.hop_polys(supports, self.max_diffusion_step, b)
        basis = ops.shared_spectral_basis(supports, self.max_diffusion_step)
        cur, x_off, planes = inputs.reshape(t_len, b, self.num_nodes, -1), 0, None
        finals, top_sel, out = [], None, None
        packs = ops.pack_encoder_cells(self.encoding_cells, basis, self.num_nodes)
        for layer, cell in enumerate(self.encoding_cells):
            h0 = None if initial_hidden_state is None else initial_hidden_state[layer]
            is_top = layer == self.num_rnn_layers - 1
            out = cell.run_sequence(cur, h0, p, p_batched, lengths if is_top else None, x_off, planes,
                                    want_hsel=want_finals or (is_top and lengths is not None), basis=basis,
                                    pack=None if packs is None else packs[0][layer], spack=None if packs is None else packs[1][layer])
            if is_top and lengths is not None:
                top_sel = out.hsel
                finals.append(out.hext[t_len] if want_finals else None)
            else:
                finals.append(out.hsel if want_finals else None)
            cur, x_off, planes = out.hext.view(t_len + 1, b, self.num_nodes, self.hid_dim), 1, out.hpl
        return (torch.stack(finals, dim=0) if want_finals else None), out.hseq, top_sel

    def forward(self, inputs, initial_hidden_state, supports):
        finals, top, _ = self.run(inputs, initial_hidden_state, supports)
        return finals, top

    def init_hidden(self, batch_size):
        return torch.stack([c.init_hidden(batch_size) for c in self.encoding_cells], dim=0)


class DCGRUDecoder(_FusedDropout, nn.Module):

    def __init__(self, input_dim, max_diffusion_step, num_nodes, hid_dim, output_dim, num_rnn_layers,
                 dcgru_activation=None, filter_type="laplacian", device=None, dropout=0.0):
        super().__init__()
        self.input_dim = input_dim
        self.hid_dim = hid_dim
        self.num_nodes = num_nodes
        self.output_dim = output_dim
        self.num_rnn_layers = num_rnn_layers
        self.max_diffusion_step = max_diffusion_step
        self._device = device
        shared = DCGRUCell(input_dim=hid_dim, num_units=hid_dim, max_diffusion_step=max_diffusion_step,
                           num_nodes=num_nodes, nonlinearity=dcgru_activation, filter_type=filter_type)
        first = DCGRUCell(input_dim=input_dim, num_units=hid_dim, max_diffusion_step=max_diffusion_step,
                          num_nodes=num_nodes, nonlinearity=dcgru_activation, filter_type=filter_type)
        self.decoding_cells = nn.ModuleList([first] + [shared] * (num_rnn_layers - 1))
# ... 17 lines not shown
                                 None if shared is None else cell_params(shared), self.projection_layer.weight,
                                 self.projection_layer.bias, self.num_nodes, self.hid_dim, self.output_dim,
                                 first.num_matrices, self.num_rnn_layers, first._activation_name, teacher,
                                 dropout_p=drop_p, rng_state=self._rng_state(inputs.device) if drop_p > 0 else None)


class DCRNNModel_classification(_FusedDropout, nn.Module):

    def __init__(self, args, num_classes, device=None, strict_lengths=False):
        super().__init__()
        self.num_nodes = args.num_nodes
        self.num_rnn_layers = args.num_rnn_layers
        self.rnn_units = args.rnn_units
        self._device = device
        self.num_classes = num_classes
        self.strict_lengths = bool(strict_lengths)
        self.encoder = DCRNNEncoder(input_dim=args.input_dim, max_diffusion_step=args.max_diffusion_step,
                                    hid_dim=args.rnn_units, num_nodes=args.num_nodes,
                                    num_rnn_layers=args.num_rnn_layers,
                                    dcgru_activation=args.dcgru_activation, filter_type=args.filter_type)
        self.fc = nn.Linear(args.rnn_units, num_classes)
        self.dropout = nn.Dropout(args.dropout)
        self.relu = nn.ReLU()
        self._init_dropout_rng(0)

    def encode_last(self, input_seq, seq_lengths, supports):
        b = input_seq.shape[0]
        if self.strict_lengths:
            utils.check_seq_lengths(seq_lengths, input_seq.shape[1])
        x = input_seq.transpose(0, 1)
        _, _, last = self.encoder.run(x, None, supports, lengths=seq_lengths, want_finals=False)
        return last.view(b, self.num_nodes, self.rnn_units)

    def forward(self, input_seq, seq_lengths, supports):
        b = input_seq.shape[0]
        last = self.encode_last(input_seq, seq_lengths, supports)
        drop_p = self._drop_p()
        return ops.cls_head(last.view(b, self.num_nodes, self.rnn_units), self.fc.weight, self.fc.bias, drop_p,
                            self._rng_state(last.device) if drop_p > 0 else None)


class DCRNNModel_nextTimePred(nn.Module):

    def __init__(self, args, device=None):
        super().__init__()
        self.num_nodes = args.num_nodes
        self.num_rnn_layers = args.num_rnn_layers
        self.rnn_units = args.rnn_units
        self._device = device
        self.output_dim = args.output_dim
        self.cl_decay_steps = args.cl_decay_steps
        self.use_curriculum_learning = bool(args.use_curriculum_learning)
        self.batches_seen_increment = 0
        self._ddp_params_and_buffers_to_ignore = ["decoder._dropout_rng"]
        self.encoder = DCRNNEncoder(input_dim=args.input_dim, max_diffusion_step=args.max_diffusion_step,
                                    hid_dim=args.rnn_units, num_nodes=args.num_nodes,
                                    num_rnn_layers=args.num_rnn_layers,
                                    dcgru_activation=args.dcgru_activation, filter_type=args.filter_type)
        self.decoder = DCGRUDecoder(input_dim=args.output_dim, max_diffusion_step=args.max_diffusion_step,
                                    num_nodes=args.num_nodes, hid_dim=args.rnn_units,
                                    output_dim=args.output_dim, num_rnn_layers=args.num_rnn_layers,
                                    dcgru_activation=args.dcgru_activation, filter_type=args.filter_type,
                                    device=device, dropout=args.dropout)

    def forward(self, encoder_inputs, decoder_inputs, supports, batches_seen=None):
        b, t_out, n, _ = decoder_inputs.shape
# ... 13 lines not shown
```

eeg_gnn_ssl_amd/ops.py:

```python
from __future__ import annotations

import ctypes
from typing import List, Optional, Sequence, Tuple

import torch

from . import _lib
from ._lib import DecoderDims, LayerDims

ACT_CODES = {"tanh": 0, "relu": 1, None: 1}
NS = "eeg_dcrnn"
_libdef = torch.library.Library(NS, "DEF")


import os as _os

GEMM_MODE = 1 if _os.environ.get("EEG_DCRNN_SPLIT_BF16", "0") not in ("", "0") else 0


def set_gemm_mode(mode: int) -> int:
    global GEMM_MODE
    if mode not in (0, 1):
        raise ValueError("gemm mode must be 0 (fp32 MFMA) or 1 (three-term bf16 split)")
    prev, GEMM_MODE = GEMM_MODE, int(mode)
# ... 210 lines not shown
    lib.call("eeg_dcrnn_spectral_basis", _p(sup), n, _p(out), _stream(sup))
    return out


def _spectral_basis_floats(n):
    return int(_lib.get_lib().query("eeg_dcrnn_spectral_basis_floats", int(n)))


_define("spectral_basis", "(Tensor support) -> Tensor", _spectral_basis_impl,
        lambda support: support.new_empty((_spectral_basis_floats(support.shape[0]),), dtype=torch.float32))


def _pack_cell_spectral_impl(wg, wc, basis, fin: int, h: int, m: int, n: int) -> torch.Tensor:
    lib = _lib.get_lib()
    wg, wc = wg.detach(), wc.detach()
    for t, nm in ((wg, "dconv_gate.weight"), (wc, "dconv_candidate.weight"), (basis, "basis")):
        _check(lib, t, nm)
    rows = (fin + h) * m
    if tuple(wg.shape) != (rows, 2 * h) or tuple(wc.shape) != (rows, h) or basis.numel() != _spectral_basis_floats(n):
        raise RuntimeError(f"pack_cell_spectral: operands {tuple(wg.shape)}, {tuple(wc.shape)}, basis {tuple(basis.shape)} do not match "
                           f"input_dim={fin}, num_units={h}, num_matrices={m}, num_nodes={n}")
    size = lib.query("eeg_dcrnn_spectral_pack_floats", fin, h, m, n)
    if size == 0:
        raise RuntimeError(f"pack_cell_spectral: the spectral form exists for 64 units (got num_units={h}, input_dim={fin})")
    out = _new((size,), wg)
    lib.call("eeg_dcrnn_pack_cell_spectral", _p(wg), _p(wc), _p(basis), fin, h, m, n, _p(out), _stream(out))
    return out


_define("pack_cell_spectral", "(Tensor wg, Tensor wc, Tensor basis, int fin, int h, int m, int n) -> Tensor", _pack_cell_spectral_impl,
        lambda wg, wc, basis, fin, h, m, n: wg.new_empty((int(_lib.get_lib().query("eeg_dcrnn_spectral_pack_floats", fin, h, m, n)),)))


def _pack_cells_impl(wgs, bgs, wcs, bcs, h: int, m: int, basis, n: int):
    lib = _lib.get_lib()
    cells = len(wgs)
    if not (cells == len(bgs) == len(wcs) == len(bcs)) or cells < 1 or cells > 4:
        raise RuntimeError(f"pack_cells: {cells} cells (1..4, one weight / bias tensor of each kind per cell)")
    wgs, bgs, wcs, bcs = ([t.detach() for t in ts] for ts in (wgs, bgs, wcs, bcs))
    fins, packs, spacks = [], [], []
    for c in range(cells):
        fin = wgs[c].shape[0] // m - h
        rows = (fin + h) * m
        for t, nm in ((wgs[c], "dconv_gate.weight"), (bgs[c], "dconv_gate.biases"), (wcs[c], "dconv_candidate.weight"), (bcs[c], "dconv_candidate.biases")):
            _check(lib, t, nm)
        if fin < 4 or tuple(wgs[c].shape) != (rows, 2 * h) or tuple(wcs[c].shape) != (rows, h) or tuple(bgs[c].shape) != (2 * h,) \
                or tuple(bcs[c].shape) != (h,):
            raise RuntimeError(f"pack_cells: cell {c} parameter shapes {tuple(wgs[c].shape)}, {tuple(bgs[c].shape)}, {tuple(wcs[c].shape)}, "
                               f"{tuple(bcs[c].shape)} do not match num_units={h}, num_matrices={m}")
        if _pack3_halves(fin, h, m) > 0:
            raise RuntimeError("pack_cells: the opt-in bf16 split packs its cells one by one (ops.pack_cell)")
        fins.append(fin)
        packs.append(_new((_pack_base_floats(fin, h, m),), wgs[c]))
        if basis is not None:
            size = lib.query("eeg_dcrnn_spectral_pack_floats", fin, h, m, n)
            if size == 0:
                raise RuntimeError(f"pack_cells: the spectral form exists for 64 units (got num_units={h}, input_dim={fin})")
            spacks.append(_new((size,), wgs[c]))
    if basis is not None:
        _check(lib, basis, "basis")
        if basis.numel() != _spectral_basis_floats(n):
            raise RuntimeError(f"pack_cells: basis {tuple(basis.shape)} is not the block of a {n}-node support")
    tab = lambda ts: (ctypes.c_void_p * cells)(*[t.data_ptr() for t in ts])
    fin_arr = (ctypes.c_int32 * cells)(*fins)
    lib.call("eeg_dcrnn_pack_cells", cells, tab(wgs), tab(bgs), tab(wcs), tab(bcs), fin_arr, h, m, tab(packs), _p(basis), n,
             tab(spacks) if basis is not None else None, _stream(packs[0]))
    return packs + spacks


def _pack_cells_fake(wgs, bgs, wcs, bcs, h, m, basis, n):
    fins = [w.shape[0] // m - h for w in wgs]
    out = [wgs[0].new_empty((_pack_floats(f, h, m),)) for f in fins]
    if basis is not None:
        out += [wgs[0].new_empty((int(_lib.get_lib().query("eeg_dcrnn_spectral_pack_floats", f, h, m, n)),)) for f in fins]
    return out


_define("pack_cells", "(Tensor[] wg, Tensor[] bg, Tensor[] wc, Tensor[] bc, int h, int m, Tensor? basis, int n) -> Tensor[]",
        _pack_cells_impl, _pack_cells_fake)


def _diffusion_hops_impl(x, p, p_batched: int, batch: int) -> torch.Tensor:
    lib = _lib.get_lib()
    _check(lib, x, "x")
    _check(lib, p, "P")
    s, n, f = x.shape
    if p.dim() != 4:
        raise RuntimeError(f"P has shape {tuple(p.shape)}, expected (graphs, hop matrices - 1, num_nodes, num_nodes)")
    m = p.shape[1] + 1
    _check_polys(p, p_batched, batch, n, m)
    if batch < 1 or s % max(batch, 1) != 0:
        raise RuntimeError(f"diffusion_hops: {s} samples are not a multiple of the batch {batch}")
    out = _new((m - 1, s, n, f), x)
    lib.call("eeg_dcrnn_diffuse_fwd", _p(x), _p(p), p_batched, s, batch, n, f, m, _p(out), _stream(x))
    return out


_define("diffusion_hops", "(Tensor x, Tensor P, int p_batched, int batch) -> Tensor", _diffusion_hops_impl,
        lambda x, p, p_batched, batch: x.new_empty((p.shape[1],) + tuple(x.shape)))


def _dconv_impl(x, p, p_batched: int, weight, biases) -> torch.Tensor:
    lib = _lib.get_lib()
    x = x.contiguous()
    w, bvec = weight.detach().contiguous(), biases.detach().contiguous()
    for t, nm in ((x, "inputs_and_state"), (p, "P"), (w, "weight"), (bvec, "biases")):
        _check(lib, t, nm)
    b, n, f = x.shape
    if p.dim() != 4:
        raise RuntimeError(f"P has shape {tuple(p.shape)}, expected (graphs, hop matrices - 1, num_nodes, num_nodes)")
    m, o = p.shape[1] + 1, w.shape[1]
# ... 60 lines not shown

    def __enter__(self):
        self.armed = True
        self.written = [False] * len(self.params)
        return self

    def __exit__(self, *exc):
        self.armed = False
        return False

    @staticmethod
    def take(param: torch.Tensor) -> Optional[torch.Tensor]:
        ref = getattr(param, "_eeg_grad_sink", None)
        if ref is None:
            return None
        sink, i = ref
        tgt = param.grad
        if (not sink.armed or sink.written[i] or sink.params[i] is not param or tgt is None or not tgt.is_contiguous()
                or tgt.shape != param.shape):
            return None
        sink.written[i] = True
        return tgt


def _layer_dims(t_len, b, n, h, fin, m, act, p_batched, planes_ready):
    dims = LayerDims(t_len, b, n, h, fin, m, act, p_batched)
    if planes_ready:
        dims.x_planes_ready = 1
        dims.x_plane_stride = (t_len + 1) * b * n * fin
    return dims


def _dcgru_layer_impl(x, x_off: int, h0, p, p_batched: int, wg, bg, wc, bc, lengths, x_planes, n: int, h: int, m: int,
                      act: int, save: bool, want_hsel: bool, basis=None, pack=None, spack=None):
    lib = _lib.get_lib()
    if x.dim() != 4 or x.shape[2] != n:
        raise RuntimeError(f"inputs have shape {tuple(x.shape)}, expected (T, B, num_nodes={n}, input_dim)")
    t_len, b, fin = x.shape[0] - x_off, x.shape[1], x.shape[3]
    if not lib.query("eeg_dcrnn_supported", n, h, fin, m):
        raise RuntimeError("eeg_gnn_ssl_amd: " + lib.last_error())
    _check_polys(p, p_batched, b, n, m)
    if lengths is not None:
        _check_lengths(lengths, b)
    if h0 is not None and h0.numel() != b * n * h:
        raise RuntimeError(f"initial_hidden_state has shape {tuple(h0.shape)}, expected ({b}, {n * h})")
    ready = x_planes is not None
    spec = basis is not None
    dims = _layer_dims(t_len, b, n, h, fin, m, act, p_batched, ready)
    if spec:
        _check(lib, basis, "basis")
        sp_rows = int(lib.query("eeg_dcrnn_spectral_rows", t_len * b))
        if ready:
            dims.x_plane_stride = (b + sp_rows) * fin
        if p_batched or basis.numel() != _spectral_basis_floats(n) or not lib.query("eeg_dcrnn_spectral_ok", ctypes.byref(dims), 0):
            raise RuntimeError("dcgru_layer: the spectral form needs one shared support (p_batched = 0) and a shape "
                               "eeg_dcrnn_spectral_ok accepts")
        if ready and tuple(x_planes.shape) != (n, b + sp_rows, fin):
            raise RuntimeError(f"x_planes has shape {tuple(x_planes.shape)}, expected {(n, b + sp_rows, fin)} (the layer below's U^T h)")
    empty = _new((0,), p)
    xsrc, xtm = None, None
    bm = 0
    if not x.is_contiguous() and x_off == 0 and not ready and x.transpose(0, 1).is_contiguous():
        bm = 2 if spec else lib.query("eeg_dcrnn_batch_major_ok", ctypes.byref(dims))
    if bm:
        xsrc = x.transpose(0, 1)
        _check(lib, xsrc, "inputs")
        if bm == 2:
# ... 25 lines not shown
            spack = torch.ops.eeg_dcrnn.pack_cell_spectral(wg, wc, basis, fin, h, m, n)
        elif spack.numel() != lib.query("eeg_dcrnn_spectral_pack_floats", fin, h, m, n):
            raise RuntimeError(f"dcgru_layer: spack has {spack.numel()} floats, expected {lib.query('eeg_dcrnn_spectral_pack_floats', fin, h, m, n)}")
        dims.spectral, dims.spack = basis.data_ptr(), spack.data_ptr()
        if ready:
            _check(lib, x_planes, "x_planes")
            planes, planes_ptr = _new((0,), p), x_planes.data_ptr() + 4 * b * fin
        else:
            planes = _new((n, sp_rows, fin), x)
            planes_ptr = planes.data_ptr()
    elif ready:
        _check(lib, x_planes, "x_planes")
        if tuple(x_planes.shape) != (m - 1, t_len + 1, b, n, fin):
            raise RuntimeError(f"x_planes has shape {tuple(x_planes.shape)}, expected {(m - 1, t_len + 1, b, n, fin)}")
        planes, planes_ptr = _new((0,), p), x_planes.data_ptr() + 4 * b * n * fin
    else:
        planes = _new((m - 1, s, n, fin), x)
        planes_ptr = planes.data_ptr()
    hext = _new((t_len + 1, b, n * h), x)
    if save:
        rs, us, cs, rhs = (_new((t_len, b, n * h), x) for _ in range(4))
        if spec:
            hpl, rhpl = _new((n, b + sp_rows, h), x), _new((n, sp_rows, h), x)
        else:
            hpl, rhpl = (_new((m - 1, t_len + 1, b, n, h), x) for _ in range(2))
    else:
        rs = us = cs = rhs = hpl = rhpl = None
    ws = _new((lib.query("eeg_dcrnn_layer_fwd_ws_floats", ctypes.byref(dims)),), x)
    lib.call("eeg_dcrnn_layer_fwd", ctypes.byref(dims), _p(xsrc if xsrc is not None else xk), _p(xtm) if (xsrc is not None and bm != 2) else None,
             _p(h0), _p(p), _p(pack), planes_ptr, _p(hext), _p(rs), _p(us), _p(cs), _p(rhs), _p(hpl), _p(rhpl), _p(ws), _stream(x))
    if lengths is not None:
        lengths = lengths.to(device=x.device, dtype=torch.int64).contiguous()
        hsel = _new((b, n * h), x)
        lib.call("eeg_dcrnn_gather_last", _p(hext[1:]), _p(lengths), t_len, b, n * h, _p(hsel), _stream(x))
    elif want_hsel:
        hsel = hext[t_len].clone()
    else:
        hsel = _new((0,), x)
    if not save:
        return hext, hsel, []
    return hext, hsel, [xtm if xtm is not None else empty, _new((0,), p) if pack_given else pack, planes, rs, us, cs, rhs, hpl, rhpl,
                        _new((0,), p) if (spack_given or not spec) else spack]


def _dcgru_layer_fake(x, x_off, h0, p, p_batched, wg, bg, wc, bc, lengths, x_planes, n, h, m, act, save, want_hsel, basis=None,
                      pack=None, spack=None):
    t_len, b, fin = x.shape[0] - x_off, x.shape[1], x.shape[3]
    ne = lambda *shape: x.new_empty(shape)
    hext, hsel = ne(t_len + 1, b, n * h), (ne(b, n * h) if (want_hsel or lengths is not None) else ne(0))
    if not save:
        return hext, hsel, []
    zero_copy = False
    spec = basis is not None
    if not x.is_contiguous() and x_off == 0 and x_planes is None and x.transpose(0, 1).is_contiguous():
        dims = _layer_dims(t_len, b, n, h, fin, m, act, p_batched, False)
        zero_copy = spec or _lib.get_lib().query("eeg_dcrnn_batch_major_ok", ctypes.byref(dims)) == 2
    xtm = ne(t_len, b, n, fin) if (not x.is_contiguous() and not zero_copy) else ne(0)
    planes = ne(0) if x_planes is not None else ne(m - 1, t_len * b, n, fin)
    spack_in, spack = spack, ne(0)
    byp = [ne(m - 1, t_len + 1, b, n, h) for _ in range(2)]
    if spec:
        lib = _lib.get_lib()
        sp_rows = int(lib.query("eeg_dcrnn_spectral_rows", t_len * b))
        if x_planes is None:
            planes = ne(n, sp_rows, fin)
        if spack_in is None:
            spack = ne(int(lib.query("eeg_dcrnn_spectral_pack_floats", fin, h, m, n)))
        byp = [ne(n, b + sp_rows, h), ne(n, sp_rows, h)]
    return hext, hsel, [xtm, ne(0) if pack is not None else ne(_pack_floats(fin, h, m)), planes] + [ne(t_len, b, n * h) for _ in range(4)] + byp + [spack]


def _dcgru_layer_bwd_impl(d_hext, d_hsel, x, x_off: int, p, p_batched: int, pack, planes, x_planes, hext, rs, us, cs, rhs,
                          hpl, rhpl, lengths, has_h0: bool, n: int, h: int, m: int, act: int, need_dx: bool, need_dh0: bool,
                          dwg, dbg, dwc, dbc, basis=None, spack=None):
    lib = _lib.get_lib()
    t_len, b, fin = hext.shape[0] - 1, hext.shape[1], x.shape[3]
    ready = x_planes is not None
    dims = _layer_dims(t_len, b, n, h, fin, m, act, p_batched, ready)
    if not x.is_contiguous():
# ... 11 lines not shown
                               "input width is not 64?)")
        dims.spectral, dims.spack = basis.data_ptr(), spack.data_ptr()
    state = b * n * h
    if d_hext is not None:
        d_hext = d_hext.contiguous()
        _check(lib, d_hext, "grad of hext")
    if d_hsel is not None:
        d_hsel = d_hsel.contiguous()
    d_hseq_ptr = ctypes.c_void_p(d_hext.data_ptr() + 4 * state) if d_hext is not None else None
    d_at_end = d_hsel if lengths is None else None
    d_at_len = d_hsel if lengths is not None else None
    xk_ptr = ctypes.c_void_p(x.data_ptr() + 4 * x_off * b * n * fin)
    dx = _new((t_len + x_off, b, n, fin), hext) if need_dx else _new((0,), hext)
    if need_dx and x_off:
        lib.call("eeg_dcrnn_zero", _p(dx), 4 * x_off * b * n * fin, _stream(dx))
    dx_ptr = ctypes.c_void_p(dx.data_ptr() + 4 * x_off * b * n * fin) if need_dx else None
    dh0 = _new((b, n * h), hext) if (need_dh0 and has_h0) else _new((0,), hext)
    ws = _new((lib.query("eeg_dcrnn_layer_bwd_ws_floats", ctypes.byref(dims), 1 if need_dx else 0),), hext)
    lib.call("eeg_dcrnn_layer_bwd", ctypes.byref(dims), xk_ptr, _p(p), _p(pack), planes_ptr, _p(hext), _p(rs),
             _p(us), _p(cs), _p(rhs), _p(_none_if_empty(hpl)), _p(_none_if_empty(rhpl)), d_hseq_ptr, _p(d_at_end), _p(d_at_len), _p(lengths), dx_ptr,
             _p(dh0) if dh0.numel() else None, _p(dwg), _p(dbg), _p(dwc), _p(dbc), _p(ws), _stream(hext))
    return dx, dh0


def _dcgru_layer_bwd_fake(d_hext, d_hsel, x, x_off, p, p_batched, pack, planes, x_planes, hext, rs, us, cs, rhs, hpl, rhpl,
                          lengths, has_h0, n, h, m, act, need_dx, need_dh0, dwg, dbg, dwc, dbc, basis=None, spack=None):
    t_len, b, fin = hext.shape[0] - 1, hext.shape[1], x.shape[3]
    return (hext.new_empty((t_len + x_off, b, n, fin) if need_dx else (0,)),
            hext.new_empty((b, n * h) if (need_dh0 and has_h0) else (0,)))


_define("dcgru_layer",
        "(Tensor x, int x_off, Tensor? h0, Tensor P, int p_batched, Tensor wg, Tensor bg, Tensor wc, Tensor bc, Tensor? lengths, "
        "Tensor? x_planes, int n, int h, int m, int act, bool save, bool want_hsel, Tensor? basis, Tensor? pack=None, Tensor? spack=None) -> "
        "(Tensor hext, Tensor hsel, Tensor[] saved)",
        _dcgru_layer_impl, _dcgru_layer_fake)
_define("dcgru_layer_bwd",
        "(Tensor? d_hext, Tensor? d_hsel, Tensor x, int x_off, Tensor P, int p_batched, Tensor pack, Tensor planes, Tensor? x_planes, "
        "Tensor hext, Tensor rs, Tensor us, Tensor cs, Tensor rhs, Tensor hpl, Tensor rhpl, Tensor? lengths, bool has_h0, int n, int h, "
        "int m, int act, bool need_dx, bool need_dh0, Tensor(a!) dwg, Tensor(b!) dbg, Tensor(c!) dwc, Tensor(d!) dbc, "
        "Tensor? basis, Tensor? spack) -> (Tensor, Tensor)",
        _dcgru_layer_bwd_impl, _dcgru_layer_bwd_fake)


def _dcgru_layer_setup(ctx, inputs, output):
    (x, x_off, h0, p, p_batched, wg, bg, wc, bc, lengths, x_planes, n, h, m, act, save, want_hsel, basis, _pack, _spack) = inputs
    hext, _, saved = output
    ctx.set_materialize_grads(False)
    ctx.saved_ok = bool(save) and len(saved) == 10
    ctx.meta = (x_off, p_batched, n, h, m, act, h0 is not None)
    ctx.params = (wg, bg, wc, bc)
    if ctx.saved_ok:
        xtm = saved[0]
        lens = None if lengths is None else lengths.to(device=x.device, dtype=torch.int64).contiguous()
        kept = list(saved[1:])
        if _pack is not None:
            kept[0] = _pack
        if _spack is not None and basis is not None:
            kept[8] = _spack
        ctx.save_for_backward(xtm if xtm.numel() else x, p, x_planes, lens, basis, hext, *kept)


def _dcgru_layer_backward(ctx, d_hext, d_hsel, d_saved):
    if not ctx.saved_ok:
        raise RuntimeError("eeg_dcrnn::dcgru_layer was run with save=False: nothing was kept for the backward pass")
    xk, p, x_planes, lens, basis, hext, pack, planes, rs, us, cs, rhs, hpl, rhpl, spack = ctx.saved_tensors
    x_off, p_batched, n, h, m, act, has_h0 = ctx.meta
    need_dx, need_dh0 = ctx.needs_input_grad[0], has_h0 and ctx.needs_input_grad[2]
    fin = xk.shape[3]
    rows = (fin + h) * m
    shapes = ((rows, 2 * h), (2 * h,), (rows, h), (h,))
    sunk = [GradSink.take(q) for q in ctx.params]
    bufs = [t if t is not None else _new(sh, hext) for t, sh in zip(sunk, shapes)]
    dx, dh0 = torch.ops.eeg_dcrnn.dcgru_layer_bwd(d_hext, d_hsel, xk, x_off, p, p_batched, pack, planes, x_planes, hext,
                                                  rs, us, cs, rhs, hpl, rhpl, lens, has_h0, n, h, m, act, need_dx, need_dh0, *bufs,
                                                  basis, spack if basis is not None else None)
    ret = [None if t is not None else g for t, g in zip(sunk, bufs)]
    grads = (dx if need_dx else None, None, dh0 if need_dh0 else None, None, None, *ret, None, None, None, None, None, None, None, None,
             None, None, None)
    return grads[:len(ctx.needs_input_grad)]


torch.library.register_autograd(f"{NS}::dcgru_layer", _dcgru_layer_backward, setup_context=_dcgru_layer_setup, lib=_libdef)


def _dec_dims(meta, dropout_p=0.0, teacher_on_device=False):
    t_len, b, n, h, dout, m, n_layers, act, p_batched = meta
    return DecoderDims(t_len, b, n, h, dout, m, n_layers, act, p_batched, float(dropout_p), 1 if teacher_on_device else 0)


def _teacher_arg(lib, teacher, teacher_dev, t_len):
    if teacher_dev is not None:
        _check(lib, teacher_dev, "teacher_dev", torch.int32)
        if teacher_dev.numel() != t_len:
            raise RuntimeError(f"teacher_dev: expected int32[{t_len}], got {tuple(teacher_dev.shape)}")
        return _p(teacher_dev), teacher_dev, True
    if len(teacher) > 0 and any(teacher):
        arr = (ctypes.c_int32 * t_len)(*[1 if teacher[i] else 0 for i in range(t_len)])
        return ctypes.cast(arr, ctypes.c_void_p), arr, False
    return None, None, False


def make_rng_state(device, stream_id: int = 0) -> torch.Tensor:
    rank = 0
    if torch.distributed.is_available() and torch.distributed.is_initialized():
        rank = torch.distributed.get_rank()
    g = torch.Generator().manual_seed((torch.initial_seed() + 0x9E3779B97F4A7C15 * int(stream_id) + 0xD1B54A32D192ED03 * rank) % (1 << 63))
    seed = int(torch.randint(0, 2 ** 62, (1,), generator=g).item())
    return torch.tensor([seed, 0], dtype=torch.int64, device=device)


def _check_rng(lib, t, name):
# ... 213 lines not shown
    if z.dim() != 3:
        raise RuntimeError(f"cls_head_loss: head input has shape {tuple(z.shape)}, expected (B, num_nodes, rnn_units)")
    b, n, h = z.shape
    c = w.shape[0]
    if tuple(w.shape) != (c, h) or bias.numel() != c or tuple(dw.shape) != (c, h) or db.numel() != c or not dw.is_contiguous() or not db.is_contiguous():
        raise RuntimeError(f"cls_head_loss: fc operands {tuple(w.shape)}, {tuple(bias.shape)}, gradients {tuple(dw.shape)}, {tuple(db.shape)} do not "
                           f"fit a head input of {h} units")
    if kind == 0:
        tg = targets.to(torch.float32).contiguous().view(-1)
        _check(lib, tg, "targets")
    else:
        tg = targets.to(torch.int64).contiguous().view(-1)
        _check(lib, tg, "targets", torch.int64)
    if tg.numel() != b:
        raise RuntimeError(f"cls_head_loss: {tg.numel()} targets for {b} clips")
    drop = dropout_p > 0
    if drop:
        if rng_used is None:
            raise RuntimeError("cls_head_loss: dropout_p > 0 needs rng_used (ops.rng_take)")
        _check_rng(lib, rng_used, "rng_used")
    loss, logits, arg = _new((1,), z), _new((b, c), z), _new((b, c), z, torch.int32)
    dlogits, dz = _new((b, c), z), torch.empty_like(z)
    ws = _new((lib.query("eeg_dcrnn_cls_head_loss_ws_floats", b, h, c),), z)
    if clip_w is None:
        lib.call("eeg_dcrnn_cls_head_loss", _p(z), _p(w), _p(bias), _p(tg), int(kind), b, n, h, c, float(dropout_p), _p(rng_used) if drop else None,
                 _p(logits), _p(arg), _p(dlogits), _p(dz), _p(dw), _p(db), _p(loss), _p(ws), _stream(z))
    else:
        clip_w, denom = _clip_weights("cls_head_loss", clip_w, denom, b, z)
        lib.call("eeg_dcrnn_cls_head_loss_w", _p(z), _p(w), _p(bias), _p(tg), int(kind), b, n, h, c, float(dropout_p), _p(rng_used) if drop else None,
                 _p(clip_w), _p(denom), _p(logits), _p(arg), _p(dlogits), _p(dz), _p(dw), _p(db), _p(loss), _p(ws), _stream(z))
    return loss, logits, arg, dlogits, dz


def _cls_head_loss_w_impl(z, w, bias, targets, kind: int, dropout_p: float, rng_used, clip_w, denom, dw, db):
    return _cls_head_loss_impl(z, w, bias, targets, kind, dropout_p, rng_used, dw, db, clip_w, denom)


def _cls_head_loss_fake(z, w, bias, targets, kind, dropout_p, rng_used, dw, db):
    b, c = z.shape[0], w.shape[0]
    return (z.new_empty((1,)), z.new_empty((b, c)), z.new_empty((b, c), dtype=torch.int32), z.new_empty((b, c)), torch.empty_like(z))


_define("cls_head_loss", "(Tensor z, Tensor w, Tensor bias, Tensor targets, int kind, float dropout_p, Tensor? rng_used, Tensor(a!) dw, Tensor(b!) db) "
        "-> (Tensor, Tensor, Tensor, Tensor, Tensor)", _cls_head_loss_impl, _cls_head_loss_fake)
_define("cls_head_loss_w", "(Tensor z, Tensor w, Tensor bias, Tensor targets, int kind, float dropout_p, Tensor? rng_used, Tensor clip_w, Tensor denom, "
        "Tensor(a!) dw, Tensor(b!) db) -> (Tensor, Tensor, Tensor, Tensor, Tensor)", _cls_head_loss_w_impl,
        lambda z, w, bias, targets, kind, dropout_p, rng_used, clip_w, denom, dw, db: _cls_head_loss_fake(z, w, bias, targets, kind, dropout_p, rng_used, dw, db))


def _gather_last_impl(htop, lengths):
    lib = _lib.get_lib()
    htop = htop.contiguous()
    _check(lib, htop, "output")
    t_len, b, d = htop.shape
    _check_lengths(lengths, b)
    lengths = lengths.to(device=htop.device, dtype=torch.int64).contiguous()
    out = _new((b, d), htop)
    lib.call("eeg_dcrnn_gather_last", _p(htop), _p(lengths), t_len, b, d, _p(out), _stream(htop))
    return out


_define("gather_last", "(Tensor htop, Tensor lengths) -> Tensor", _gather_last_impl,
        lambda htop, lengths: htop.new_empty((htop.shape[1], htop.shape[2])))


def _corr_graph_impl(x, top_k: int, lengths=None):
    lib = _lib.get_lib()
    x = x.contiguous()
    _check(lib, x, "clips")
    if x.dim() != 4:
        raise RuntimeError(f"clips must be (B,T,N,D), got {tuple(x.shape)}")
    b, t_len, n, d = x.shape
    if lengths is not None:
        lengths = _clip_lengths("corr_graph_len", lengths, b, x)
    adj, s1, s2 = (_new((b, n, n), x) for _ in range(3))
    ws = _new((lib.query("eeg_dcrnn_corr_graph_ws_floats", b, t_len),), x)
    if lengths is None:
# ... 633 lines not shown
        if window < 4 or window % 4 != 0 or raw.shape[2] % window != 0 or raw.shape[2] == 0:
            raise RuntimeError(f"correlation_supports_raw: rows of {raw.shape[2]} samples are not whole steps of window={window} samples "
                               f"(a positive multiple of 4)")
        _clip_lengths("correlation_supports_raw", lengths, raw.shape[0], raw)
        adj, s1, s2 = torch.ops.eeg_dcrnn.corr_graph_rows_len(raw, int(top_k), lengths, int(raw.shape[2] // window))
        return ([s1, s2], adj) if return_adj else [s1, s2]
    adj, s1, s2 = torch.ops.eeg_dcrnn.corr_graph_rows(raw, int(top_k))
    return ([s1, s2], adj) if return_adj else [s1, s2]


def pack_cell(wg, bg, wc, bc, fin: int, h: int, m: int) -> torch.Tensor:
    return torch.ops.eeg_dcrnn.pack_cell(wg, bg, wc, bc, fin, h, m)


def diffusion_hops(x: torch.Tensor, p: torch.Tensor, p_batched: int, batch: int) -> torch.Tensor:
    return torch.ops.eeg_dcrnn.diffusion_hops(x, p, int(p_batched), int(batch))


def dconv(x, p, p_batched, weight, biases):
    return torch.ops.eeg_dcrnn.dconv(x, p, int(p_batched), weight, biases)


class LayerOut:
    __slots__ = ("hext", "hsel", "hpl")

    def __init__(self, hext, hsel, hpl):
        self.hext, self.hsel, self.hpl = hext, hsel, hpl

    @property
    def hseq(self):
        return self.hext[1:]


def pack_encoder_cells(cells, basis, num_nodes):
    cells = list(cells)
    if len(cells) < 2 or len(cells) > 4 or GEMM_MODE != 0:
        return None
    h, m = cells[0]._num_units, cells[0].num_matrices
    if basis is not None and h != 64:
        basis = None
    out = torch.ops.eeg_dcrnn.pack_cells([c.dconv_gate.weight.detach() for c in cells], [c.dconv_gate.biases.detach() for c in cells],
                                         [c.dconv_candidate.weight.detach() for c in cells], [c.dconv_candidate.biases.detach() for c in cells],
                                         h, m, basis, int(num_nodes))
    k = len(cells)
    return out[:k], (out[k:] if basis is not None else [None] * k)


def dcgru_layer_ex(x, x_off, h0, p, p_batched, wg, bg, wc, bc, n, h, m, activation="tanh", lengths=None, x_planes=None,
                   want_hsel=True, basis=None, pack=None, spack=None) -> LayerOut:
    act = ACT_CODES.get(activation, 1)
    save = torch.is_grad_enabled() and any(t is not None and t.requires_grad for t in (x, h0, wg, bg, wc, bc))
    if basis is not None:
        need_dx = 1 if (save and x.requires_grad) else 0
        dims = _layer_dims(x.shape[0] - x_off, x.shape[1], n, h, x.shape[3], m, act, int(p_batched), False)
        if p_batched or not _lib.get_lib().query("eeg_dcrnn_spectral_ok", ctypes.byref(dims), need_dx):
            basis = None
        else:
            if x_planes is not None and x_planes.dim() != 3:
                x_planes = None
            global spectral_layer_calls
            spectral_layer_calls += 1
    if basis is None and x_planes is not None and x_planes.dim() != 5:
        x_planes = None
    if x_planes is not None:
        global hop_plane_handovers
        hop_plane_handovers += 1
    hext, hsel, saved = torch.ops.eeg_dcrnn.dcgru_layer(x, int(x_off), h0, p, int(p_batched), wg, bg, wc, bc, lengths, x_planes,
                                                        n, h, m, act, save, bool(want_hsel), basis, pack,
                                                        spack if basis is not None else None)
    return LayerOut(hext, hsel, saved[7].detach() if (save and saved[7].numel()) else None)


_basis_cache = {}


def shared_spectral_basis(supports, max_diffusion_step: int):
    if not SPECTRAL_MODE or max_diffusion_step < 1 or len(supports) != 1:
        return None
    sup = supports[0]
    if sup.dim() != 2 or sup.shape[0] != sup.shape[1] or sup.shape[0] < 2 or sup.shape[0] > 32:
        return None
    import weakref
    key = (sup.data_ptr(), sup._version, str(sup.device), tuple(sup.shape), sup.dtype)
    hit = _basis_cache.get(key)
    if hit is not None and hit[0]() is sup:
        return hit[1]
    if sup.is_cuda and torch.cuda.is_current_stream_capturing():
        return None
    if len(_basis_cache) > 64:
        for k in [k for k, v in _basis_cache.items() if v[0]() is None]:
            del _basis_cache[k]
    basis = torch.ops.eeg_dcrnn.spectral_basis(sup)
    n = sup.shape[0]
    info = basis[n * n + 256:n * n + 259].tolist()
    ok = info[0] <= SPECTRAL_TOL * max(info[2], 1e-30) and info[1] <= 1e-9 * max(info[2], 1e-30)
    _basis_cache[key] = (weakref.ref(sup), basis if ok else None)
    return basis if ok else None


def dcgru_layer(x, h0, p, p_batched, wg, bg, wc, bc, n, h, m, activation="tanh", lengths=None):
    out = dcgru_layer_ex(x, 0, h0, p, p_batched, wg, bg, wc, bc, n, h, m, activation, lengths)
    return out.hseq, out.hsel
# ... 15 lines not shown

def cls_head(z, w, bias, dropout_p=0.0, rng_state=None, return_rng_used=False):
    used = rng_take(rng_state, z.numel() // 4) if dropout_p > 0 else None
    logits, _ = torch.ops.eeg_dcrnn.cls_head(z, w, bias, float(dropout_p), used)
    return (logits, used) if return_rng_used else logits


def _weights_together(what, clip_w, denom, ref):
    if (clip_w is None) != (denom is None):
        raise RuntimeError(f"{what}: clip_w and denom come together (one of them is None)")
    if clip_w is not None:
        _clip_weights(what, clip_w, denom, clip_w.numel() if torch.is_tensor(clip_w) and clip_w.dim() == 1 else -1, ref)


def cls_head_loss(z, fc_weight, fc_bias, targets, task="detection", dropout_p=0.0, rng_state=None, clip_w=None, denom=None):
    _weights_together("cls_head_loss", clip_w, denom, z)
    used = rng_take(rng_state, z.numel() // 4) if dropout_p > 0 else None
    sunk = [GradSink.take(q) for q in (fc_weight, fc_bias)]
    dw = sunk[0] if sunk[0] is not None else torch.empty_like(fc_weight)
    db = sunk[1] if sunk[1] is not None else torch.empty_like(fc_bias)
    kind = 0 if task == "detection" else 1
    if clip_w is None:
        loss, logits, _arg, _dl, dz = torch.ops.eeg_dcrnn.cls_head_loss(z.detach(), fc_weight.detach(), fc_bias.detach(), targets,
                                                                        kind, float(dropout_p), used, dw, db)
    else:
        loss, logits, _arg, _dl, dz = torch.ops.eeg_dcrnn.cls_head_loss_w(z.detach(), fc_weight.detach(), fc_bias.detach(), targets,
                                                                          kind, float(dropout_p), used, clip_w, denom, dw, db)
    for q, buf, sk in ((fc_weight, dw, sunk[0]), (fc_bias, db, sunk[1])):
        if sk is None and q.requires_grad:
            q.grad = buf if q.grad is None else q.grad + buf
    return loss[0], logits, dz


def rng_take(rng_state, groups):
    if rng_state is None:
        raise RuntimeError("dropout_p > 0 needs a device generator state (ops.make_rng_state)")
    return torch.ops.eeg_dcrnn.rng_take_(rng_state, int(groups))


def dropout_mask(rng_used, n, dropout_p):
    return torch.ops.eeg_dcrnn.dropout_mask(rng_used, int(n), float(dropout_p))


def gather_last(htop: torch.Tensor, lengths: torch.Tensor) -> torch.Tensor:
    return torch.ops.eeg_dcrnn.gather_last(htop, lengths)


def masked_regression_loss(y_predicted, y_true, mean=None, std=None, loss_fn="mae", mask_val=0.0, clip_w=None, denom=None):
    _weights_together("masked_regression_loss", clip_w, denom, y_predicted)
    scaled = mean is not None
    args = (y_predicted, y_true, scaled, float(mean) if scaled else 0.0, float(std) if scaled else 1.0, float(mask_val), 0 if loss_fn == "mae" else 1)
    if clip_w is None:
        return torch.ops.eeg_dcrnn.masked_loss(*args)[0]
    return torch.ops.eeg_dcrnn.masked_loss_w(*args, clip_w, denom)[0]


def bce_with_logits(logits, y, clip_w=None, denom=None):
    _weights_together("bce_with_logits", clip_w, denom, logits)
    if clip_w is None:
        return torch.ops.eeg_dcrnn.bce_logits(logits, y)[0]
    return torch.ops.eeg_dcrnn.bce_logits_w(logits, y, clip_w, denom)[0]


def cross_entropy(logits, y, clip_w=None, denom=None):
    _weights_together("cross_entropy", clip_w, denom, logits)
    if clip_w is None:
# ... 53 lines not shown
```

eeg_gnn_ssl_amd/train_step.py:

```python
from __future__ import annotations

from typing import Optional, Sequence

import torch
import torch.distributed as dist

from . import ops


class FlatParameters:

    def __init__(self, module: torch.nn.Module):
        params, seen = [], set()
        for p in module.parameters():
            if id(p) not in seen:
                seen.add(id(p))
                params.append(p)
        self.params = params
        total = sum(p.numel() for p in params)
        dev, dt = params[0].device, params[0].dtype
        self.flat = torch.empty(total, device=dev, dtype=dt)
        self.flat_grad = torch.zeros(total, device=dev, dtype=dt)
        off = 0
        with torch.no_grad():
# ... 18 lines not shown
                 scaler_mean: Optional[float] = None, scaler_std: Optional[float] = None,
                 always_reduce: bool = False, raw_window: Optional[int] = None, raw_mean: float = 0.0, raw_std: float = 1.0,
                 shared_graph: bool = True, data_augment: bool = False, swap_perm=None, reflected_supports=None,
                 feature_std: Optional[float] = None, use_fft: bool = True, feature_mean: Optional[float] = None,
                 padding_val: Optional[float] = None):
        assert task in ("detection", "classification", "ssl")
        if padding_val is not None and task == "ssl":
            raise ValueError("TrainStep: padding_val (variable-length clips) is for the supervised tasks; the SSL pair has no seq_lengths")
        self.padding_val = None if padding_val is None else float(padding_val)
        self.model, self.task, self.max_grad_norm = model, task, max_grad_norm
        self.fp = FlatParameters(model)
        self.lr, self.weight_decay, self.betas, self.eps = lr, weight_decay, (0.9, 0.999), 1e-8
        self.exp_avg = torch.zeros_like(self.fp.flat)
        self.exp_avg_sq = torch.zeros_like(self.fp.flat)
        self.ws = torch.zeros(64, device=self.fp.flat.device, dtype=torch.float32)
        self.grad_norm = torch.zeros(1, device=self.fp.flat.device, dtype=torch.float32)
        self.step_count = 0
        dev = self.fp.flat.device
        self.step_dev = torch.zeros(1, device=dev, dtype=torch.int32)
        self.lr_dev = torch.full((1,), float(lr), device=dev, dtype=torch.float32)
        self.samples_seen = 0
        self.samples_seen_dev = torch.zeros(1, device=dev, dtype=torch.int64)
        has_pg = dist.is_available() and dist.is_initialized()
        self.world = dist.get_world_size() if has_pg else 1
        self.reduce = has_pg and (self.world > 1 or always_reduce)
        self.scaler_mean, self.scaler_std = scaler_mean, scaler_std
        self.raw_window, self.raw_mean, self.raw_std = raw_window, float(raw_mean), float(raw_std)
        self.shared_graph = bool(shared_graph)
        self.use_fft = bool(use_fft)
        self.feature_mean = None if feature_mean is None else float(feature_mean)
        self.last_scale = None
        self.fused_head = True
        self.last_logits = None
        self.data_augment = bool(data_augment)
        self.feature_std = None if feature_std is None else float(feature_std)
        self.swap_perm, self.reflected_supports, self._augment_rng = None, None, None
        if self.data_augment:
            from . import utils
            if not use_fft and raw_window is None and (feature_std is None or feature_mean is None):
                raise ValueError("TrainStep: data_augment on time-domain windows (use_fft=False) needs feature_mean and feature_std (the "
                                 "StandardScaler's: the reference multiplies the signals BEFORE it standardises)")
            if raw_window is None and feature_std is None:
                raise ValueError("TrainStep: data_augment on feature inputs needs feature_std (the StandardScaler's std: the reference "
                                 "adds log(scale) BEFORE it standardises)")
            sp = utils.swap_permutation(model.num_nodes) if swap_perm is None else torch.as_tensor(swap_perm)
            if sp.numel() != model.num_nodes:
                raise ValueError(f"TrainStep: swap_perm has {sp.numel()} entries for {model.num_nodes} nodes")
            self.swap_perm = sp.to(device=dev, dtype=torch.int32).contiguous()
            if reflected_supports is not None:
                self.reflected_supports = torch.stack([torch.as_tensor(r, dtype=torch.float32) for r in reflected_supports]).to(dev).contiguous()
            self._augment_rng = ops.make_rng_state(dev, stream_id=2)
        self.last_augmentation = None
        self._graphs = {}
        self.sampler, self._epoch_batches = None, {}
        self._pending_sampler_state = None
        self.device_curriculum = None

    @property
    def step_count(self):
        return self._step_count

    @step_count.setter
    def step_count(self, value):
        self._step_count = int(value)
        if hasattr(self, "step_dev"):
            self.step_dev.fill_(self._step_count)
# ... 66 lines not shown
        perm, log_scale = None, None
        if self.data_augment and self.model.training:
            supports, perm, log_scale = self._draw_augmentation(x.shape[0], supports)
        lens, pad = None, 0.0
        if self.padding_val is not None and seq_lengths is not None:
            lens, pad = seq_lengths.to(device=x.device, dtype=torch.int64), self.padding_val
        if not self.use_fft:
            x, y, supports = self._time_domain_inputs(x, y, supports, perm, log_scale, lens, pad)
        elif self.task == "ssl" and (self.raw_window is not None or perm is not None):
            x, y, supports = self._ssl_pair(x, y, supports, perm, log_scale)
        elif self.raw_window is not None:
            feat_raw, x = ops.fft_features(x, window=self.raw_window, mean=self.raw_mean, std=self.raw_std, perm=perm, log_scale=log_scale,
                                           lengths=lens, padding_val=pad)
            if supports is None:
                supports = ops.correlation_supports(feat_raw, top_k=3, lengths=lens)
        elif perm is not None:
            plain = x
            idx = perm.to(torch.int64)[:, None, :, None].expand(-1, x.shape[1], -1, x.shape[3])
            x = x.gather(2, idx) + (log_scale / self.feature_std)[:, None, None, None]
            if supports is None:
                supports = ops.correlation_supports(plain, top_k=3, lengths=lens)
        if supports is None:
            supports = ops.correlation_supports(x, top_k=3, lengths=lens)
        elif self.shared_graph:
            supports = ops.collapse_shared_supports(supports)
        if self.task == "ssl":
            if self._use_device_curriculum(y.shape[1], y.shape[0]):
                self.model.batches_seen_increment = sampler.n_valid if tail else x.shape[0] * self.world
                out = self.model(x, y, supports, batches_seen=self.samples_seen_dev)
            else:
                out = self.model(x, y, supports, batches_seen=self.samples_seen)
        elif self.fused_head and hasattr(self.model, "encode_last"):
            m = self.model
            last = m.encode_last(x, seq_lengths, supports)
            drop_p = m._drop_p()
            with self.fp.sink:
                loss, self.last_logits, dz = ops.cls_head_loss(last, m.fc.weight, m.fc.bias, y, self.task, drop_p,
                                                               m._rng_state(last.device) if drop_p > 0 else None, clip_w=clip_w, denom=denom)
                last.backward(dz)
            return loss.detach()
        else:
            out = self.model(x, seq_lengths, supports)
        loss, seed = self.loss_and_grad(out.detach(), y, clip_w, denom)
        with self.fp.sink:
            out.backward(seed.view_as(out))
        return loss.detach()

    def _ssl_target_steps(self, y) -> int:
        if self.raw_window is None:
            return y.shape[1]
        w = self.raw_window
        if y.dim() != 3 or y.shape[2] == 0 or y.shape[2] % w != 0:
            raise ValueError(f"TrainStep(task='ssl', raw_window={w}): y is the RAW target (B, num_nodes, Ty*{w}) -- the signals "
                             f"of the seconds to predict, a whole number of {w}-sample windows -- got {tuple(y.shape)}")
        return y.shape[2] // w

    def _ssl_pair(self, x, y, supports, perm, log_scale):
        if self.raw_window is not None:
            self._ssl_target_steps(y)
            if y.shape[:2] != x.shape[:2]:
                raise ValueError(f"TrainStep(task='ssl', raw_window={self.raw_window}): the raw target must be (B, num_nodes, Ty*"
                                 f"{self.raw_window}) with the input's {x.shape[0]} clips and {x.shape[1]} nodes, got {tuple(y.shape)}")
            plain, x, y = ops.fft_features_pair(x, y, window=self.raw_window, mean=self.raw_mean, std=self.raw_std, perm=perm,
                                                log_scale=log_scale)
        else:
            plain = x
            x, y = ops.augment_features(x, y, perm, log_scale, self.feature_std)
        if supports is None:
# ... 356 lines not shown
```

include/eeg_dcrnn.h:

```cpp
#ifndef EEG_DCRNN_H
#define EEG_DCRNN_H
#include <stddef.h>
#include <stdint.h>

#ifdef __cplusplus
extern "C" {
#endif

typedef struct eeg_layer_dims {
    int32_t T, B, N, H, Fin, M;
    int32_t act;
    int32_t p_batched;
    int32_t x_planes_ready;
    int32_t x_batch_major;
    int64_t x_plane_stride;
    const uint16_t* pack3;
    const float* spectral;
    const float* spack;
} eeg_layer_dims;

typedef struct eeg_decoder_dims {
    int32_t T, B, N, H;
    int32_t Dout;
    int32_t M, L;
// ... 39 lines not shown
                              const float* c, float* x_out, float* y_out, void* stream);

size_t eeg_dcrnn_corr_graph_ws_floats(int B, int T);
int eeg_dcrnn_corr_graph(const float* X, int B, int T, int N, int D, int top_k, float* adj, float* S1,
                         float* S2, float* ws, void* stream);

int eeg_dcrnn_corr_graph_len(const float* X, int B, int T, int N, int D, int top_k, const int64_t* lengths, float* adj, float* S1,
                             float* S2, float* ws, void* stream);

size_t eeg_dcrnn_corr_graph_rows_ws_floats(int B, int P, int Q);
int eeg_dcrnn_corr_graph_rows(const float* X, int B, int N, int P, int Q, long long piece_stride, int top_k, float* adj, float* S1,
                              float* S2, float* ws, void* stream);

int eeg_dcrnn_corr_graph_rows_len(const float* X, int B, int N, int P, int Q, long long piece_stride, int top_k, const int64_t* lengths,
                                  int steps, float* adj, float* S1, float* S2, float* ws, void* stream);

size_t eeg_dcrnn_pack_floats(int Fin, int H, int M);
int eeg_dcrnn_pack_cell(const float* Wg, const float* bg, const float* Wc, const float* bc,
                        int Fin, int H, int M, float* pack, void* stream);

size_t eeg_dcrnn_pack3_halves(int Fin, int H, int M);
int eeg_dcrnn_pack_cell_bf16x3(const float* Wg, const float* Wc, int Fin, int H, int M, uint16_t* pack3, void* stream);

size_t eeg_dcrnn_spectral_basis_floats(int N);
int eeg_dcrnn_spectral_basis(const float* support, int N, float* basis, void* stream);
size_t eeg_dcrnn_spectral_pack_floats(int Fin, int H, int M, int N);
int eeg_dcrnn_pack_cell_spectral(const float* Wg, const float* Wc, const float* basis, int Fin, int H, int M, int N,
                                 float* spack, void* stream);
int eeg_dcrnn_pack_cells(int n_cells, const float* const* Wg, const float* const* bg, const float* const* Wc,
                         const float* const* bc, const int32_t* Fin, int H, int M, float* const* packs, const float* basis,
                         int N, float* const* spacks, void* stream);
int eeg_dcrnn_spectral_ok(const eeg_layer_dims* d, int need_dx);
size_t eeg_dcrnn_spectral_rows(size_t S);

int eeg_dcrnn_diffuse_fwd(const float* X, const float* P, int p_batched, int S, int B, int N, int F,
                          int M, float* planes, void* stream);
int eeg_dcrnn_diffuse_adj(const float* Z, const float* P, int p_batched, int S, int B, int N, int F,
                          int M, float* dX, void* stream);

size_t eeg_dcrnn_dconv_fwd_ws_floats(int B, int N, int F, int M, int O);
int eeg_dcrnn_dconv_fwd(const float* X, const float* P, int p_batched, int B, int N, int F, int M,
                        const float* W, const float* bias, int O, float* out, float* ws, void* stream);

size_t eeg_dcrnn_dconv_bwd_ws_floats(int B, int N, int F, int M, int O);
int eeg_dcrnn_dconv_bwd(const float* X, const float* P, int p_batched, int B, int N, int F, int M,
                        const float* W, int O, const float* dOut, float* dX, float* dW, float* dbias,
                        float* ws, void* stream);

size_t eeg_dcrnn_layer_fwd_ws_floats(const eeg_layer_dims* d);
int eeg_dcrnn_batch_major_ok(const eeg_layer_dims* d);
int eeg_dcrnn_layer_fwd(const eeg_layer_dims* d, const float* X, float* Xtm, const float* h0, const float* P,
                        const float* pack, float* planes, float* Hext, float* Rs, float* Us,
                        float* Cs, float* RHs, float* Hplanes, float* RHplanes, float* ws, void* stream);

size_t eeg_dcrnn_layer_bwd_ws_floats(const eeg_layer_dims* d, int need_dx);
int eeg_dcrnn_layer_bwd(const eeg_layer_dims* d, const float* X, const float* P, const float* pack,
                        const float* planes, const float* Hext, const float* Rs, const float* Us,
                        const float* Cs, const float* RHs, const float* Hplanes, const float* RHplanes,
                        const float* dHseq, const float* d_at_end,
                        const float* d_at_len, const int64_t* lengths, float* dX, float* dh0,
                        float* dWg, float* dbg, float* dWc, float* dbc, float* ws, void* stream);

size_t eeg_dcrnn_decoder_saved_floats(const eeg_decoder_dims* d);
size_t eeg_dcrnn_decoder_fwd_ws_floats(const eeg_decoder_dims* d);
size_t eeg_dcrnn_decoder_bwd_ws_floats(const eeg_decoder_dims* d);
int eeg_dcrnn_decoder_is_persistent(const eeg_decoder_dims* d);
// ... 14 lines not shown

int eeg_dcrnn_augment_draw(const uint64_t* rng_used, int B, int N, const int32_t* swap_perm, int32_t* flags, int32_t* perm,
                           float* log_scale, const float* S_plain, const float* S_reflected, int n_supports, float* S_out,
                           void* stream);

int eeg_dcrnn_epoch_keys(uint64_t seed, int64_t epoch, int64_t P, int64_t* keys, void* stream);
int eeg_dcrnn_gather_clips(const float* x_pool, float* x_out, size_t x_row_bytes, const float* y_pool, float* y_out, size_t y_row_bytes,
                           const void* label_pool, void* label_out, int label_bytes, const int64_t* len_pool, int64_t* len_out,
                           const int64_t* perm, int64_t n_perm, int64_t P, int64_t* cursor, int B, int rank, int world, void* stream);

int eeg_dcrnn_gather_clips_tail(const float* x_pool, float* x_out, size_t x_row_bytes, const float* y_pool, float* y_out, size_t y_row_bytes,
                                const void* label_pool, void* label_out, int label_bytes, const int64_t* len_pool, int64_t* len_out,
                                const int64_t* perm, int64_t n_perm, int64_t P, int64_t* cursor, int B, int rank, int world, float* clip_w,
                                float* denom, int64_t* n_valid, void* stream);

int eeg_dcrnn_gather_last(const float* Htop, const int64_t* lengths, int T, int B, int NH,
                          float* last, void* stream);
int eeg_dcrnn_rng_take(uint64_t* rng_state, uint64_t groups, uint64_t* rng_used, void* stream);
int eeg_dcrnn_cls_head_fwd(const float* z, const float* W, const float* bias, int B, int N, int H,
                           int C, float dropout_p, const uint64_t* rng_used,
                           float* logits, int32_t* arg, void* stream);
int eeg_dcrnn_cls_head_bwd(const float* z, const float* W, const float* dlogits, const int32_t* arg,
                           int B, int N, int H, int C, float dropout_p, const uint64_t* rng_used,
                           float* dz, float* dW, float* dbias, void* stream);

size_t eeg_dcrnn_cls_head_loss_ws_floats(int B, int H, int C);
int eeg_dcrnn_cls_head_loss(const float* z, const float* W, const float* bias, const void* targets, int kind, int B, int N,
                            int H, int C, float dropout_p, const uint64_t* rng_used, float* logits, int32_t* arg,
                            float* dlogits, float* dz, float* dW, float* dbias, float* loss, float* ws, void* stream);
int eeg_dcrnn_cls_head_loss_w(const float* z, const float* W, const float* bias, const void* targets, int kind, int B, int N,
                              int H, int C, float dropout_p, const uint64_t* rng_used, const float* clip_w, const float* denom,
                              float* logits, int32_t* arg, float* dlogits, float* dz, float* dW, float* dbias, float* loss, float* ws,
                              void* stream);
int eeg_dcrnn_dropout_mask(const uint64_t* rng_used, size_t n, float dropout_p, float* mask, void* stream);

int eeg_dcrnn_bce_logits(const float* logits, const float* y, int B, float* loss, float* dlogits, void* stream);
int eeg_dcrnn_ce_logits(const float* logits, const int64_t* y, int B, int C, float* loss, float* dlogits,
                        void* stream);
size_t eeg_dcrnn_masked_loss_ws_floats(void);
int eeg_dcrnn_masked_loss(const float* pred, const float* y, size_t n, int use_scaler, float mean, float std_,
                          float mask_val, int kind, float* loss, float* dpred, float* ws, void* stream);
int eeg_dcrnn_bce_logits_w(const float* logits, const float* y, int B, const float* clip_w, const float* denom, float* loss,
                           float* dlogits, void* stream);
int eeg_dcrnn_ce_logits_w(const float* logits, const int64_t* y, int B, int C, const float* clip_w, const float* denom, float* loss,
                          float* dlogits, void* stream);
int eeg_dcrnn_masked_loss_w(const float* pred, const float* y, size_t n, int B, const float* clip_w, const float* denom, int use_scaler,
                            float mean, float std_, float mask_val, int kind, float* loss, float* dpred, float* ws, void* stream);
size_t eeg_dcrnn_clip_adam_ws_floats(void);
int eeg_dcrnn_clip_adam(float* params, float* grads, float* exp_avg, float* exp_avg_sq, size_t n,
                        float max_norm, float lr, float beta1, float beta2, float eps, float weight_decay,
                        int step, float grad_scale, float* ws, float* norm_out, void* stream);

int eeg_dcrnn_clip_adam_dev(float* params, float* grads, float* exp_avg, float* exp_avg_sq, size_t n,
                            float max_norm, const float* lr_dev, float beta1, float beta2, float eps,
                            float weight_decay, int32_t* step_dev, float grad_scale, float* ws, float* norm_out,
                            void* stream);

#ifdef __cplusplus
}
#endif
#endif
```

Baseline: 138,500.

## Fuse last-step gather into single-launch head loss, pack only needed parts, overlap fold

The classification head now reads the top-layer sequence directly, gathers each clip's last valid step and computes loss and gradients in one kernel. It uses a ticket counter to do the final reduction in the last block, replacing separate gather, head and finish launches. Weight packing can now be limited to the parts each layer actually reads, skipping unused pack work. In the spectral backward pass, the weight-gradient fold is forked onto a side stream so it can overlap the fused dX GEMM. This adds stream fork/join overhead and ticket-based cross-block synchronization.

New measurement: 135,900. 0.982x the previous value.

```diff
diff --git a/eeg_gnn_ssl_amd/_lib.py b/eeg_gnn_ssl_amd/_lib.py
--- a/eeg_gnn_ssl_amd/_lib.py
+++ b/eeg_gnn_ssl_amd/_lib.py
@@ -95,10 +95,15 @@
     "eeg_dcrnn_teacher_flags_dev": (c_int, [_FP, _FP, _FP, ctypes.c_double, c_int, _FP, c_void_p]),
     "eeg_dcrnn_pack_cells": (c_int, [c_int, POINTER(c_void_p), POINTER(c_void_p), POINTER(c_void_p), POINTER(c_void_p), POINTER(ctypes.c_int32),
                              c_int, c_int, POINTER(c_void_p), _FP, c_int, POINTER(c_void_p), c_void_p]),
+    "eeg_dcrnn_pack_parts": (c_int, [POINTER(LayerDims), c_int, c_int, c_int]),
+    "eeg_dcrnn_pack_cells_parts": (c_int, [c_int, POINTER(c_void_p), POINTER(c_void_p), POINTER(c_void_p), POINTER(c_void_p), POINTER(ctypes.c_int32),
+                                   c_int, c_int, POINTER(c_void_p), _FP, c_int, POINTER(c_void_p), POINTER(ctypes.c_int32), c_void_p]),
     "eeg_dcrnn_cls_head_loss_ws_floats": (c_size_t, [c_int, c_int, c_int]),
     "eeg_dcrnn_cls_head_loss": (c_int, [_FP, _FP, _FP, _FP, c_int, c_int, c_int, c_int, c_int, c_float, _FP, _FP, _FP, _FP, _FP, _FP, _FP, _FP, _FP,
                                 c_void_p]),
     "eeg_dcrnn_gather_last": (c_int, [_FP, _FP, c_int, c_int, c_int, _FP, c_void_p]),
+    "eeg_dcrnn_cls_head_loss_gather": (c_int, [_FP, _FP, c_int, _FP, _FP, _FP, c_int, c_int, c_int, c_int, c_int, c_float, _FP, _FP, _FP,
+                                               _FP, _FP, _FP, _FP, _FP, _FP, _FP, _FP, _FP, c_void_p]),
     "eeg_dcrnn_rng_take": (c_int, [_FP, ctypes.c_uint64, _FP, c_void_p]),
     "eeg_dcrnn_cls_head_fwd": (c_int, [_FP, _FP, _FP, c_int, c_int, c_int, c_int, c_float, _FP, _FP, _FP, c_void_p]),
     "eeg_dcrnn_cls_head_bwd": (c_int, [_FP, _FP, _FP, _FP, c_int, c_int, c_int, c_int, c_float, _FP, _FP, _FP, _FP, c_void_p]),
diff --git a/eeg_gnn_ssl_amd/csrc/api.cpp b/eeg_gnn_ssl_amd/csrc/api.cpp
--- a/eeg_gnn_ssl_amd/csrc/api.cpp
+++ b/eeg_gnn_ssl_amd/csrc/api.cpp
@@ -401,7 +401,7 @@
 size_t xs_spec(const eeg_layer_dims* d) { return d->x_plane_stride > 0 ? (size_t)d->x_plane_stride : 0; }
 int cell_weight_grads_spectral(const eeg_layer_dims* d, const float* Xh, size_t x_gs, const float* hh, size_t hh_gs, const float* rhh,
                                const float* dYh, float* part, const BwdWs& w, float* dWg, float* dWc, hipStream_t st,
-                               const float* bias_part, float* dbg, float* dbc) {
+                               const float* bias_part, float* dbg, float* dbc, void* side_lane = nullptr) {
     const int S = d->T * d->B, H = d->H, M = d->M, Fin = d->Fin, N = d->N, Sp = spec_rows(S);
     float* part_g = part + (w.part_g - w.partial);
     float* part_c = part + (w.part_c - w.partial);
@@ -425,7 +425,15 @@
     const int ns_max = N * (g.spg_x > g.spg_h ? g.spg_x : g.spg_h);
     const size_t fold_lds = spec_fold_lds_bytes(M, ns_max);
     EEG_SET_MAX_LDS(reduce_unpack3s_kernel, fold_lds);
-    EEG_LAUNCH_P("reduce_unpack", reduce_unpack3s_kernel, dim3(nblocks), dim3(256), fold_lds, st, jobs, sj, 0, Fin, H, M, dWg, dWc);
+    hipStream_t fold_st = st;
+#ifdef EEG_PLATFORM_SIDE_LANE
+    if (side_lane != nullptr) {
+        PlatformSideLane* lane = static_cast<PlatformSideLane*>(side_lane);
+        if (!platform_lane_fork(lane, st)) return fail("reduce_unpack (spectral): fork to the side stream failed");
+        fold_st = lane->st;
+    }
+#endif
+    EEG_LAUNCH_P("reduce_unpack", reduce_unpack3s_kernel, dim3(nblocks), dim3(256), fold_lds, fold_st, jobs, sj, 0, Fin, H, M, dWg, dWc);
     return check_launch("reduce_unpack (spectral)");
 }
 
@@ -663,25 +671,50 @@
     if (launch_spec_pack(Wg, Wc, basis, Fin, H, M, N, spack, S_(stream))) return fail("pack_cell_spectral: launch failed");
     return check_launch("pack_cell_spectral");
 }
-int eeg_dcrnn_pack_cells(int n_cells, const float* const* Wg, const float* const* bg, const float* const* Wc, const float* const* bc,
-                         const int32_t* Fin, int H, int M, float* const* packs, const float* basis, int N, float* const* spacks,
-                         void* stream) {
+static int pack_cells_launch(int n_cells, const float* const* Wg, const float* const* bg, const float* const* Wc, const float* const* bc,
+                             const int32_t* Fin, int H, int M, float* const* packs, const float* basis, int N, float* const* spacks,
+                             const int32_t* parts, void* stream) {
     if (n_cells < 1 || n_cells > 4) return fail("pack_cells: %d cells (1..4 per launch)", n_cells);
     if (Wg == nullptr || bg == nullptr || Wc == nullptr || bc == nullptr || Fin == nullptr || packs == nullptr) return fail("pack_cells: null pointer table");
     if (!seq_h_supported(H)) return fail("pack_cells: rnn_units=%d unsupported", H);
     if (!seq_m_supported(M)) return fail("pack_cells: num hop matrices M=%d unsupported (1,2,3,4,5,7)", M);
     if ((basis == nullptr) != (spacks == nullptr)) return fail("pack_cells: the per-frequency packs need the basis block and their output table");
     int fin[4];
+    unsigned want[4];
     for (int c = 0; c < n_cells; ++c) {
         fin[c] = Fin[c];
+        want[c] = parts != nullptr ? (unsigned)parts[c] : (kPackAll | (spacks != nullptr ? kPackSpec : 0u));
         if (fin[c] < 4 || fin[c] % 4 != 0) return fail("pack_cells: input dim %d of cell %d must be a positive multiple of 4", fin[c], c);
-        if (Wg[c] == nullptr || bg[c] == nullptr || Wc[c] == nullptr || bc[c] == nullptr || packs[c] == nullptr || (spacks != nullptr && spacks[c] == nullptr))
+        if ((want[c] & ~(kPackAll | kPackSpec)) != 0 || (want[c] & kPackRecur) == 0)
+            return fail("pack_cells: parts=%u of cell %d (EEG_PACK_RECUR, plus any of EEG_PACK_X / _DEC / _SPEC)", want[c], c);
+        const bool spec = (want[c] & kPackSpec) != 0;
+        if (spec && spacks == nullptr) return fail("pack_cells: cell %d asks for its per-frequency packs without a basis", c);
+        if (Wg[c] == nullptr || bg[c] == nullptr || Wc[c] == nullptr || bc[c] == nullptr || packs[c] == nullptr || (spec && spacks[c] == nullptr))
             return fail("pack_cells: null pointer in the tables of cell %d", c);
-        if (spacks != nullptr && eeg_dcrnn_spectral_pack_floats(fin[c], H, M, N) == 0)
+        if (spec && eeg_dcrnn_spectral_pack_floats(fin[c], H, M, N) == 0)
             return fail("pack_cells: input_dim=%d rnn_units=%d hop matrices=%d nodes=%d: the spectral form exists for 64 units", fin[c], H, M, N);
     }
-    if (launch_pack_cells(n_cells, Wg, bg, Wc, bc, fin, H, M, packs, basis, N, spacks, S_(stream))) return fail("pack_cells: launch failed");
+    if (launch_pack_cells(n_cells, Wg, bg, Wc, bc, fin, H, M, packs, basis, N, spacks, want, S_(stream))) return fail("pack_cells: launch failed");
     return check_launch("pack_cells");
+}
+int eeg_dcrnn_pack_cells(int n_cells, const float* const* Wg, const float* const* bg, const float* const* Wc, const float* const* bc,
+                         const int32_t* Fin, int H, int M, float* const* packs, const float* basis, int N, float* const* spacks,
+                         void* stream) {
+    return pack_cells_launch(n_cells, Wg, bg, Wc, bc, Fin, H, M, packs, basis, N, spacks, nullptr, stream);
+}
+int eeg_dcrnn_pack_cells_parts(int n_cells, const float* const* Wg, const float* const* bg, const float* const* Wc, const float* const* bc,
+                               const int32_t* Fin, int H, int M, float* const* packs, const float* basis, int N, float* const* spacks,
+                               const int32_t* parts, void* stream) {
+    if (parts == nullptr) return fail("pack_cells_parts: null parts table");
+    return pack_cells_launch(n_cells, Wg, bg, Wc, bc, Fin, H, M, packs, basis, N, spacks, parts, stream);
+}
+int eeg_dcrnn_pack_parts(const eeg_layer_dims* d, int spectral, int need_dx, int decoder) {
+    unsigned parts = kPackRecur;
+    if (decoder) return (int)(parts | kPackX | kPackDec);
+    eeg_layer_dims q = *d;
+    q.x_planes_ready = 0;
+    parts |= (spectral && eeg_dcrnn_spectral_ok(&q, need_dx)) ? kPackSpec : kPackX;
+    return (int)parts;
 }
 int eeg_dcrnn_spectral_ok(const eeg_layer_dims* d, int need_dx) {
     if (!layer_dims_positive(d) || d->p_batched) return 0;
@@ -743,6 +776,8 @@
             if (Hplanes != nullptr) {
                 if (launch_spec_zero_rows(Hplanes, N, (d->T + 1) * d->B, SpE, H, st)) return fail("spec_zero_rows: launch failed");
                 if (launch_spec_zero_pad(RHplanes, N, S, H, st)) return fail("spec_zero_pad: launch failed");
+            } else if (save) {
+                if (launch_spec_rh(Rs, Hext, (size_t)R * H, RHs, st)) return fail("spec_rh: launch failed");
             }
         } else {
             if (spec_mix(0, Yh, d->spectral, N, d->T, d->B, 3 * H, 0, XW, st, "spec_mix_y")) return 1;
@@ -820,12 +855,23 @@
             if (spec_mix(1, RHs, d->spectral, N, d->T, d->B, H, 0, ws + w.rhplanes, st, "spec_mix_h")) return 1;
             hh = ws + w.hplanes; rhh = ws + w.rhplanes; hh_gs = 0;
         }
-        if (cell_weight_grads_spectral(d, planes, xs_spec(d), hh, hh_gs, rhh, dYh, ws + w.partial, w, dWg, dWc, st, dbias, dbg, dbc)) return 1;
+        void* lane = nullptr;
+        SpecDxPlan dx{};
         if (dX != nullptr) {
-            const SpecDxPlan dx = spec_dx_plan(Fin, N, d->T, d->B, num_cus(), spec_knobs());
+            dx = spec_dx_plan(Fin, N, d->T, d->B, num_cus(), spec_knobs());
             if (spec_plan_error("layer_bwd (spectral dX)", dx.error)) return 1;
+#ifdef EEG_PLATFORM_SIDE_LANE
+            if (dx.kind == SpecDxKind::Fused) lane = platform_side_lane(!platform_stream_is_capturing(st));
+#endif
+        }
+        if (cell_weight_grads_spectral(d, planes, xs_spec(d), hh, hh_gs, rhh, dYh, ws + w.partial, w, dWg, dWc, st, dbias, dbg, dbc, lane)) return 1;
+        if (dX != nullptr) {
             if (dx.kind == SpecDxKind::Fused) {
-                if (launch_dxf(dx, dYh, Sp, S, N, d->spack + sp.sxtq, sp.sxtq_stride, d->spectral, dX, st, "gemm_dx_f")) return fail("gemm_dxf: launch failed");
+                const int rc = launch_dxf(dx, dYh, Sp, S, N, d->spack + sp.sxtq, sp.sxtq_stride, d->spectral, dX, st, "gemm_dx_f");
+#ifdef EEG_PLATFORM_SIDE_LANE
+                if (lane != nullptr && !platform_lane_join(static_cast<PlatformSideLane*>(lane), st)) return fail("layer_bwd (spectral): join of the side stream failed");
+#endif
+                if (rc) return fail("gemm_dxf: launch failed");
             } else {
                 float* dXh = ws + w.z;
                 if (launch_spec_nn(dx.nn, dYh, 0, 3 * H, Sp, N, d->spack + sp.sxtq, sp.sxtq_stride, dXh, st, "gemm_nn_dx")) return fail("gemm_nng: launch failed");
@@ -1553,6 +1599,32 @@
     return cls_head_loss_launch(z, W, bias, targets, kind, B, N, H, C, dropout_p, rng_used, clip_w, denom, logits, arg, dlogits, dz, dW, dbias,
                                 loss, ws, stream);
 }
+int eeg_dcrnn_cls_head_loss_gather(const float* Htop, const int64_t* lengths, int T, const float* W, const float* bias, const void* targets,
+                                   int kind, int B, int N, int H, int C, float dropout_p, const uint64_t* rng_used, const float* clip_w,
+                                   const float* denom, float* logits, int32_t* arg, float* dlogits, float* dz, float* dW, float* dbias,
+                                   float* loss, float* ws, uint64_t* ticket, void* stream) {
+    if (T < 1 || B < 1 || N < 1 || H < 1 || C < 1) return fail("cls_head_loss_gather: empty input (T=%d, B=%d, N=%d, H=%d, C=%d)", T, B, N, H, C);
+    if (N > 64) return fail("cls_head_loss_gather: num_nodes=%d unsupported (<= 64)", N);
+    if (H % 4 != 0) return fail("cls_head_loss_gather: rnn_units=%d must be a multiple of 4", H);
+    if (kind != 0 && kind != 1) return fail("cls_head_loss_gather: kind=%d (0 = BCE-with-logits, 1 = cross-entropy)", kind);
+    if (kind == 0 && C != 1) return fail("cls_head_loss_gather: BCE-with-logits takes one logit per clip (num_classes=%d)", C);
+    if (check_dropout_p("cls_head_loss_gather", dropout_p)) return 1;
+    const DropCfg drop = make_drop_cfg(dropout_p);
+    if (drop.on && rng_used == nullptr) return fail("cls_head_loss_gather: dropout_p > 0 needs the {seed, offset} pair of eeg_dcrnn_rng_take");
+    if ((clip_w == nullptr) != (denom == nullptr)) return fail("cls_head_loss_gather: clip_w and denom come together");
+    if (Htop == nullptr || lengths == nullptr || W == nullptr || bias == nullptr || targets == nullptr || logits == nullptr || arg == nullptr ||
+        dlogits == nullptr || dz == nullptr || dW == nullptr || dbias == nullptr || loss == nullptr || ws == nullptr || ticket == nullptr)
+        return fail("cls_head_loss_gather: null pointer");
+    const int O = C * H + C, nblk = ceil_div(B, 4);
+    const size_t lds = (size_t)(4 * cls_tail_wave_floats(N, H, C) + 4 * (O + 1) + cls_head_ticket_floats) * sizeof(float);
+    if (lds > kMaxLdsBytes)
+        return fail("cls_head_loss_gather: N=%d x (classes=%d + rnn_units=%d) floats of four clips do not fit the %zu-byte LDS", N, C, H, (size_t)kMaxLdsBytes);
+    EEG_SET_MAX_LDS(cls_head_loss_gather_kernel, lds);
+    EEG_LAUNCH_P("cls_head_loss", cls_head_loss_gather_kernel, dim3(nblk), dim3(256), lds, S_(stream), Htop, reinterpret_cast<const long long*>(lengths), T,
+                 W, bias, targets, kind, B, N, H, C, drop, reinterpret_cast<const unsigned long long*>(rng_used), clip_w, denom, logits,
+                 reinterpret_cast<int*>(arg), dlogits, dz, ws, reinterpret_cast<unsigned long long*>(ticket), dW, dbias, loss);
+    return check_launch("cls_head_loss_gather");
+}
 size_t eeg_dcrnn_dconv_fwd_ws_floats(int B, int N, int F, int M, int O) {
     if (B < 1 || N < 1 || F < 1 || M < 1 || O < 1) return 0;
     return (size_t)(M - 1) * B * N * F + (size_t)F * M * O;
diff --git a/eeg_gnn_ssl_amd/csrc/kernels_head.h b/eeg_gnn_ssl_amd/csrc/kernels_head.h
--- a/eeg_gnn_ssl_amd/csrc/kernels_head.h
+++ b/eeg_gnn_ssl_amd/csrc/kernels_head.h
@@ -108,8 +108,9 @@
                                                    const void* __restrict__ targets, int kind, int B, int N, int H, int C, const DropCfg& drop,
                                                    const unsigned long long* __restrict__ used, float* __restrict__ logits,
                                                    int* __restrict__ arg, float* __restrict__ dlogits, float* __restrict__ dz,
-                                                   float* __restrict__ partial, const float* __restrict__ clip_w,
-                                                   const float* __restrict__ denom) {
+                                                   float* partial, const float* __restrict__ clip_w,
+                                                   const float* __restrict__ denom, const long long* __restrict__ gather_len = nullptr,
+                                                   int gather_T = 0) {
     EEG_DYN_SMEM(sm);
     const int w = threadIdx.x >> 6, lane = threadIdx.x & 63, b = blockIdx.x * 4 + w, O = C * H + C;
     float* nl = sm + w * cls_tail_wave_floats(N, H, C);
@@ -121,9 +122,16 @@
     const int groups = N * H / 4;
     if (live) {
         const unsigned long long seed = drop.on ? used[0] : 0ull, off = drop.on ? used[1] : 0ull;
+        size_t row = (size_t)b;
+        if (gather_len != nullptr) {
+            int t = (int)gather_len[b] - 1;
+            t = t < 0 ? 0 : (t >= gather_T ? gather_T - 1 : t);
+            row = (size_t)t * B + b;
+        }
+        const float* zb = z + row * groups * 4;
         for (int g = lane; g < groups; g += 64) {
             const size_t gg = (size_t)b * groups + g;
-            const f32x4 v = ld4g(z + 4 * gg);
+            const f32x4 v = ld4g(zb + 4 * g);
             f32x4 m = {1.f, 1.f, 1.f, 1.f};
             if (drop.on) m = dropout_mask4(seed, off, gg, drop.thr, drop.scale);
 #pragma unroll
@@ -217,7 +225,7 @@
                                                               float* __restrict__ dlogits, float* __restrict__ dz, float* __restrict__ partial) {
     cls_head_loss_body<true>(z, W, bias, targets, kind, B, N, H, C, drop, used, logits, arg, dlogits, dz, partial, clip_w, denom);
 }
-__device__ __forceinline__ void cls_head_loss_finish_body(const float* __restrict__ partial, int nblk, float div, int H, int C,
+__device__ __forceinline__ void cls_head_loss_finish_body(const float* partial, int nblk, float div, int H, int C,
                                                           float* __restrict__ dW, float* __restrict__ dbias, float* __restrict__ loss) {
     const int O = C * H + C;
     for (int i = threadIdx.x; i <= O; i += blockDim.x) {
@@ -244,6 +252,32 @@
                                                                      int H, int C, float* __restrict__ dW, float* __restrict__ dbias,
                                                                      float* __restrict__ loss) {
     cls_head_loss_finish_body(partial, nblk, denom[0], H, C, dW, dbias, loss);
+}
+
+constexpr int cls_head_ticket_floats = 4;
+#ifndef EEG_DEVICE_FENCE
+#define EEG_DEVICE_FENCE() ((void)0)
+#endif
+__global__ __launch_bounds__(256) void cls_head_loss_gather_kernel(const float* __restrict__ Htop, const long long* __restrict__ lengths, int T,
+                                                                   const float* __restrict__ W, const float* __restrict__ bias,
+                                                                   const void* __restrict__ targets, int kind, int B, int N, int H, int C,
+                                                                   DropCfg drop, const unsigned long long* __restrict__ used,
+                                                                   const float* __restrict__ clip_w, const float* __restrict__ denom,
+                                                                   float* __restrict__ logits, int* __restrict__ arg, float* __restrict__ dlogits,
+                                                                   float* __restrict__ dz, float* partial, unsigned long long* ticket,
+                                                                   float* __restrict__ dW, float* __restrict__ dbias, float* __restrict__ loss) {
+    if (clip_w != nullptr) cls_head_loss_body<true>(Htop, W, bias, targets, kind, B, N, H, C, drop, used, logits, arg, dlogits, dz, partial, clip_w, denom, lengths, T);
+    else cls_head_loss_body<false>(Htop, W, bias, targets, kind, B, N, H, C, drop, used, logits, arg, dlogits, dz, partial, nullptr, nullptr, lengths, T);
+    EEG_DYN_SMEM(sm);
+    unsigned* last = reinterpret_cast<unsigned*>(sm + 4 * cls_tail_wave_floats(N, H, C) + 4 * (C * H + C + 1));
+    EEG_DEVICE_FENCE();
+    __syncthreads();
+    if (threadIdx.x == 0) last[0] = atomic_add_u64(ticket, 1ull) == (unsigned long long)gridDim.x - 1ull ? 1u : 0u;
+    __syncthreads();
+    if (last[0] == 0u) return;
+    EEG_DEVICE_FENCE();
+    cls_head_loss_finish_body(partial, (int)gridDim.x, clip_w != nullptr ? denom[0] : (float)B, H, C, dW, dbias, loss);
+    if (threadIdx.x == 0) atomic_add_u64(ticket, 0ull - (unsigned long long)gridDim.x);
 }
 
 __global__ void rng_take_kernel(unsigned long long* __restrict__ state, unsigned long long* __restrict__ used, unsigned long long groups) {
diff --git a/eeg_gnn_ssl_amd/csrc/kernels_seq.h b/eeg_gnn_ssl_amd/csrc/kernels_seq.h
--- a/eeg_gnn_ssl_amd/csrc/kernels_seq.h
+++ b/eeg_gnn_ssl_amd/csrc/kernels_seq.h
@@ -534,6 +534,7 @@
     float* XRr = XC + 2 * 16 * UST;
     float* W1L = XRr + 4 * 64;
     const bool save = Rs != nullptr;
+    constexpr bool save_rh = !SPEC;
     const int ct = wave;
     const wbuf_t bH = make_wbuf(Hseq), bR = make_wbuf(save ? Rs : Hseq), bU = make_wbuf(save ? Us : Hseq),
                  bC = make_wbuf(save ? Cs : Hseq), bRH = make_wbuf(save ? RHs : Hseq);
@@ -632,11 +633,11 @@
                 A2[l1] = rh1;
                 if (save && valid[0]) {
                     wbuf_st4(bR, oh0, so, rg);
-                    wbuf_st4(bRH, oh0, so, rh);
+                    if constexpr (save_rh) wbuf_st4(bRH, oh0, so, rh);
                 }
                 if (save && valid1) {
                     wbuf_st1(bR, oh1, so, rg1);
-                    wbuf_st1(bRH, oh1, so, rh1);
+                    if constexpr (save_rh) wbuf_st1(bRH, oh1, so, rh1);
                 }
             }
             pp.mark(2);
diff --git a/eeg_gnn_ssl_amd/csrc/kernels_spectral.h b/eeg_gnn_ssl_amd/csrc/kernels_spectral.h
--- a/eeg_gnn_ssl_amd/csrc/kernels_spectral.h
+++ b/eeg_gnn_ssl_amd/csrc/kernels_spectral.h
@@ -267,6 +267,11 @@
         const int i = e / per, r = e - i * per;
         Xh[((size_t)i * Sp + S) * F + r] = 0.f;
     }
+}
+
+__global__ void spec_rh_kernel(const float* __restrict__ Rs, const float* __restrict__ Hprev, size_t n4, float* __restrict__ RHs) {
+    for (size_t g = (size_t)blockIdx.x * blockDim.x + threadIdx.x; g < n4; g += (size_t)gridDim.x * blockDim.x)
+        st4(RHs + 4 * g, ld4(Rs + 4 * g) * ld4(Hprev + 4 * g));
 }
 
 __global__ __launch_bounds__(256) void spec_mix_generic_kernel(const float* __restrict__ in, const float* __restrict__ basis,
diff --git a/eeg_gnn_ssl_amd/csrc/pack_cell.h b/eeg_gnn_ssl_amd/csrc/pack_cell.h
--- a/eeg_gnn_ssl_amd/csrc/pack_cell.h
+++ b/eeg_gnn_ssl_amd/csrc/pack_cell.h
@@ -3,6 +3,8 @@
 #include "nnq_order.h"
 
 namespace eeg {
+
+enum : unsigned { kPackRecur = 1u, kPackX = 2u, kPackDec = 4u, kPackSpec = 8u, kPackAll = kPackRecur | kPackX | kPackDec };
 
 struct CellPack {
     int Fin, H, M;
@@ -51,10 +53,12 @@
 
 __device__ __forceinline__ void pack_cell_body(const float* __restrict__ Wg, const float* __restrict__ bg,
                                                const float* __restrict__ Wc, const float* __restrict__ bc,
-                                               float* __restrict__ out, const CellPack& p, int bid, int nb) {
+                                               float* __restrict__ out, const CellPack& p, int bid, int nb, unsigned parts = kPackAll) {
     const int Fin = p.Fin, H = p.H, M = p.M;
     const size_t stride = (size_t)nb * blockDim.x;
     for (size_t idx = (size_t)bid * blockDim.x + threadIdx.x; idx < p.total; idx += stride) {
+        const unsigned part = idx < p.bias ? kPackX : (idx < p.bxt ? kPackRecur : (idx < p.c1 ? kPackX : (idx < p.bxq ? kPackDec : kPackX)));
+        if ((parts & part) == 0) continue;
         float v = 0.f;
         if (idx < p.bias) {
             const size_t e = idx - p.bx;
diff --git a/eeg_gnn_ssl_amd/csrc/platform.h b/eeg_gnn_ssl_amd/csrc/platform.h
--- a/eeg_gnn_ssl_amd/csrc/platform.h
+++ b/eeg_gnn_ssl_amd/csrc/platform.h
@@ -95,6 +95,8 @@
 
 __device__ __forceinline__ unsigned long long atomic_add_u64(unsigned long long* p, unsigned long long v) { return atomicAdd(p, v); }
 
+#define EEG_DEVICE_FENCE() __threadfence()
+
 namespace eeg {
 __device__ __forceinline__ float fast_exp(float x) { return __builtin_amdgcn_exp2f(x * 1.44269504088896340736f); }
 __device__ __forceinline__ float fast_rcp(float x) { return __builtin_amdgcn_rcpf(x); }
@@ -119,6 +121,28 @@
 inline bool platform_copy_floats(float* dst, const float* src, size_t n, hipStream_t st) {
     return hipMemcpyAsync(dst, src, n * sizeof(float), hipMemcpyDeviceToDevice, st) == hipSuccess;
 }
+#define EEG_PLATFORM_SIDE_LANE 1
+struct PlatformSideLane { hipStream_t st = nullptr; hipEvent_t fork = nullptr, join = nullptr; int dev = -1; };
+inline PlatformSideLane* platform_side_lane(bool may_create) {
+    constexpr int kMaxDev = 16;
+    thread_local PlatformSideLane lanes[kMaxDev];
+    int dev = 0;
+    if (hipGetDevice(&dev) != hipSuccess || dev < 0 || dev >= kMaxDev) return nullptr;
+    PlatformSideLane& l = lanes[dev];
+    if (l.dev == dev) return &l;
+    if (!may_create) return nullptr;
+    if (hipStreamCreateWithFlags(&l.st, hipStreamNonBlocking) != hipSuccess) return nullptr;
+    if (hipEventCreateWithFlags(&l.fork, hipEventDisableTiming) != hipSuccess || hipEventCreateWithFlags(&l.join, hipEventDisableTiming) != hipSuccess)
+        return nullptr;
+    l.dev = dev;
+    return &l;
+}
+inline bool platform_lane_fork(PlatformSideLane* l, hipStream_t st) {
+    return hipEventRecord(l->fork, st) == hipSuccess && hipStreamWaitEvent(l->st, l->fork, 0) == hipSuccess;
+}
+inline bool platform_lane_join(PlatformSideLane* l, hipStream_t st) {
+    return hipEventRecord(l->join, l->st) == hipSuccess && hipStreamWaitEvent(st, l->join, 0) == hipSuccess;
+}
 inline bool platform_stream_is_capturing(hipStream_t st) {
     hipStreamCaptureStatus cs = hipStreamCaptureStatusNone;
     return hipStreamIsCapturing(st, &cs) == hipSuccess && cs != hipStreamCaptureStatusNone;
diff --git a/eeg_gnn_ssl_amd/csrc/spec_inst.cpp b/eeg_gnn_ssl_amd/csrc/spec_inst.cpp
--- a/eeg_gnn_ssl_amd/csrc/spec_inst.cpp
+++ b/eeg_gnn_ssl_amd/csrc/spec_inst.cpp
@@ -12,6 +12,7 @@
     const float *Wg, *bg, *Wc, *bc, *basis;
     float* out;
     int spectral;
+    unsigned parts;
     CellPack cp;
     SpecPack sp;
 };
@@ -19,7 +20,7 @@
 __global__ void pack_cells_kernel(PackJobs jobs) {
     const PackJob& jb = jobs.j[blockIdx.y];
     if (jb.spectral) pack_spectral_body(jb.Wg, jb.Wc, jb.basis, jb.out, jb.sp, (int)blockIdx.x, (int)gridDim.x);
-    else pack_cell_body(jb.Wg, jb.bg, jb.Wc, jb.bc, jb.out, jb.cp, (int)blockIdx.x, (int)gridDim.x);
+    else pack_cell_body(jb.Wg, jb.bg, jb.Wc, jb.bc, jb.out, jb.cp, (int)blockIdx.x, (int)gridDim.x, jb.parts);
 }
 
 
@@ -38,17 +39,19 @@
 }
 
 int launch_pack_cells(int n_cells, const float* const* Wg, const float* const* bg, const float* const* Wc, const float* const* bc,
-                      const int* Fin, int H, int M, float* const* packs, const float* basis, int N, float* const* spacks, hipStream_t st) {
+                      const int* Fin, int H, int M, float* const* packs, const float* basis, int N, float* const* spacks, const unsigned* parts,
+                      hipStream_t st) {
     PackJobs jobs{};
     int n = 0;
     for (int c = 0; c < n_cells; ++c) {
-        if (n + (spacks != nullptr ? 2 : 1) > kMaxPackJobs) return 1;
+        const bool spec = spacks != nullptr && (parts[c] & kPackSpec) != 0;
+        if (n + (spec ? 2 : 1) > kMaxPackJobs) return 1;
         PackJob& a = jobs.j[n++];
-        a.Wg = Wg[c]; a.bg = bg[c]; a.Wc = Wc[c]; a.bc = bc[c]; a.basis = nullptr; a.out = packs[c]; a.spectral = 0;
+        a.Wg = Wg[c]; a.bg = bg[c]; a.Wc = Wc[c]; a.bc = bc[c]; a.basis = nullptr; a.out = packs[c]; a.spectral = 0; a.parts = parts[c];
         a.cp = make_cell_pack(Fin[c], H, M);
-        if (spacks != nullptr) {
+        if (spec) {
             PackJob& b = jobs.j[n++];
-            b.Wg = Wg[c]; b.bg = nullptr; b.Wc = Wc[c]; b.bc = nullptr; b.basis = basis; b.out = spacks[c]; b.spectral = 1;
+            b.Wg = Wg[c]; b.bg = nullptr; b.Wc = Wc[c]; b.bc = nullptr; b.basis = basis; b.out = spacks[c]; b.spectral = 1; b.parts = 0;
             b.sp = make_spec_pack(Fin[c], H, M, N);
         }
     }
@@ -77,6 +80,12 @@
 int launch_spec_zero_rows(float* Xh, int N, int S, int Sp, int F, hipStream_t st) {
     if (Sp <= S) return 0;
     EEG_LAUNCH_P("zero", spec_zero_pad_kernel, dim3(ceil_div(N * (Sp - S) * F, 256)), dim3(256), 0, st, Xh, N, S, Sp, F);
+    return hipGetLastError() == hipSuccess ? 0 : 2;
+}
+
+int launch_spec_rh(const float* Rs, const float* Hprev, size_t n, float* RHs, hipStream_t st) {
+    const size_t n4 = n / 4, blocks = (n4 + 255) / 256;
+    EEG_LAUNCH_P("spec_rh", spec_rh_kernel, dim3((unsigned)(blocks < 4096 ? blocks : 4096)), dim3(256), 0, st, Rs, Hprev, n4, RHs);
     return hipGetLastError() == hipSuccess ? 0 : 2;
 }
 
diff --git a/eeg_gnn_ssl_amd/csrc/spec_launch.h b/eeg_gnn_ssl_amd/csrc/spec_launch.h
--- a/eeg_gnn_ssl_amd/csrc/spec_launch.h
+++ b/eeg_gnn_ssl_amd/csrc/spec_launch.h
@@ -210,11 +210,13 @@
 int launch_spec_basis(const float* S, int N, float* basis, hipStream_t st);
 int launch_spec_pack(const float* Wg, const float* Wc, const float* basis, int Fin, int H, int M, int N, float* spack, hipStream_t st);
 int launch_pack_cells(int n_cells, const float* const* Wg, const float* const* bg, const float* const* Wc, const float* const* bc,
-                      const int* Fin, int H, int M, float* const* packs, const float* basis, int N, float* const* spacks, hipStream_t st);
+                      const int* Fin, int H, int M, float* const* packs, const float* basis, int N, float* const* spacks, const unsigned* parts,
+                      hipStream_t st);
 int launch_spec_mix(const SpecMixPlan& p, const float* in, const float* basis, int N, int T, int B, int F, int bm, float* out,
                     hipStream_t st, const char* tag);
 int launch_spec_zero_rows(float* Xh, int N, int S, int Sp, int F, hipStream_t st);
 inline int launch_spec_zero_pad(float* Xh, int N, int S, int F, hipStream_t st) { return launch_spec_zero_rows(Xh, N, S, spec_rows(S), F, st); }
+int launch_spec_rh(const float* Rs, const float* Hprev, size_t n, float* RHs, hipStream_t st);
 int launch_spec_nn(const SpecNnPlan& p, const float* A, size_t a_gstride, int K, int Sp, int G, const float* W, size_t wstride, float* C,
                    hipStream_t st, const char* tag, const float* bias = nullptr, const float* gscale = nullptr);
 int launch_tnf(const SpecTnPlan& p, const float* Xh, size_t x_gstride, int Fin, const float* Hh, size_t h_gstride, const float* RHh,
diff --git a/eeg_gnn_ssl_amd/model/cell.py b/eeg_gnn_ssl_amd/model/cell.py
--- a/eeg_gnn_ssl_amd/model/cell.py
+++ b/eeg_gnn_ssl_amd/model/cell.py
@@ -73,11 +73,12 @@
             if s.dim() not in (2, 3) or s.shape[-1] != n or s.shape[-2] != n:
                 raise RuntimeError(f"supports[{i}] has shape {tuple(s.shape)}, expected ({n}, {n}) or (B, {n}, {n})")
 
-    def run_sequence(self, x, h0, p, p_batched, lengths=None, x_off=0, x_planes=None, want_hsel=True, basis=None, pack=None, spack=None):
+    def run_sequence(self, x, h0, p, p_batched, lengths=None, x_off=0, x_planes=None, want_hsel=True, basis=None, pack=None, spack=None,
+                     pack_parts=None, gather_hsel=True):
         return ops.dcgru_layer_ex(x, x_off, h0, p, p_batched, self.dconv_gate.weight, self.dconv_gate.biases,
                                   self.dconv_candidate.weight, self.dconv_candidate.biases,
                                   self._num_nodes, self._num_units, self.num_matrices,
-                                  self._activation_name, lengths, x_planes, want_hsel, basis, pack, spack)
+                                  self._activation_name, lengths, x_planes, want_hsel, basis, pack, spack, pack_parts, gather_hsel)
 
     def forward(self, supports, inputs, state):
         self._check_supports(supports)
diff --git a/eeg_gnn_ssl_amd/model/model.py b/eeg_gnn_ssl_amd/model/model.py
--- a/eeg_gnn_ssl_amd/model/model.py
+++ b/eeg_gnn_ssl_amd/model/model.py
@@ -54,20 +54,21 @@
                                    nonlinearity=dcgru_activation, filter_type=filter_type))
         self.encoding_cells = nn.ModuleList(cells)
 
-    def run(self, inputs, initial_hidden_state, supports, lengths=None, want_finals=True):
+    def run(self, inputs, initial_hidden_state, supports, lengths=None, want_finals=True, gather_top=True):
         t_len, b = inputs.shape[0], inputs.shape[1]
         self.encoding_cells[0]._check_supports(supports)
         p, p_batched = ops.hop_polys(supports, self.max_diffusion_step, b)
         basis = ops.shared_spectral_basis(supports, self.max_diffusion_step)
         cur, x_off, planes = inputs.reshape(t_len, b, self.num_nodes, -1), 0, None
         finals, top_sel, out = [], None, None
-        packs = ops.pack_encoder_cells(self.encoding_cells, basis, self.num_nodes)
+        packs = ops.pack_encoder_cells(self.encoding_cells, basis, self.num_nodes, t_len, b, p_batched, inputs.requires_grad)
         for layer, cell in enumerate(self.encoding_cells):
             h0 = None if initial_hidden_state is None else initial_hidden_state[layer]
             is_top = layer == self.num_rnn_layers - 1
             out = cell.run_sequence(cur, h0, p, p_batched, lengths if is_top else None, x_off, planes,
                                     want_hsel=want_finals or (is_top and lengths is not None), basis=basis,
-                                    pack=None if packs is None else packs[0][layer], spack=None if packs is None else packs[1][layer])
+                                    pack=None if packs is None else packs[0][layer], spack=None if packs is None else packs[1][layer],
+                                    pack_parts=None if packs is None else packs[2][layer], gather_hsel=gather_top or not is_top)
             if is_top and lengths is not None:
                 top_sel = out.hsel
                 finals.append(out.hext[t_len] if want_finals else None)
@@ -151,6 +152,14 @@
         _, _, last = self.encoder.run(x, None, supports, lengths=seq_lengths, want_finals=False)
         return last.view(b, self.num_nodes, self.rnn_units)
 
+    def encode_top(self, input_seq, seq_lengths, supports):
+        b = input_seq.shape[0]
+        if self.strict_lengths:
+            utils.check_seq_lengths(seq_lengths, input_seq.shape[1])
+        x = input_seq.transpose(0, 1)
+        _, top, last = self.encoder.run(x, None, supports, lengths=seq_lengths, want_finals=False, gather_top=False)
+        return top, last.view(b, self.num_nodes, self.rnn_units)
+
     def forward(self, input_seq, seq_lengths, supports):
         b = input_seq.shape[0]
         last = self.encode_last(input_seq, seq_lengths, supports)
diff --git a/eeg_gnn_ssl_amd/ops.py b/eeg_gnn_ssl_amd/ops.py
--- a/eeg_gnn_ssl_amd/ops.py
+++ b/eeg_gnn_ssl_amd/ops.py
@@ -266,7 +266,11 @@
         lambda wg, wc, basis, fin, h, m, n: wg.new_empty((int(_lib.get_lib().query("eeg_dcrnn_spectral_pack_floats", fin, h, m, n)),)))
 
 
-def _pack_cells_impl(wgs, bgs, wcs, bcs, h: int, m: int, basis, n: int):
+PACK_RECUR, PACK_X, PACK_DEC, PACK_SPEC = 1, 2, 4, 8
+PACK_ALL = PACK_RECUR | PACK_X | PACK_DEC
+
+
+def _pack_cells_impl(wgs, bgs, wcs, bcs, h: int, m: int, basis, n: int, parts=None):
     lib = _lib.get_lib()
     cells = len(wgs)
     if not (cells == len(bgs) == len(wcs) == len(bcs)) or cells < 1 or cells > 4:
@@ -286,7 +290,9 @@
             raise RuntimeError("pack_cells: the opt-in bf16 split packs its cells one by one (ops.pack_cell)")
         fins.append(fin)
         packs.append(_new((_pack_base_floats(fin, h, m),), wgs[c]))
-        if basis is not None:
+        if basis is not None and parts is not None and not (parts[c] & PACK_SPEC):
+            spacks.append(_new((0,), wgs[c]))
+        elif basis is not None:
             size = lib.query("eeg_dcrnn_spectral_pack_floats", fin, h, m, n)
             if size == 0:
                 raise RuntimeError(f"pack_cells: the spectral form exists for 64 units (got num_units={h}, input_dim={fin})")
@@ -295,22 +301,31 @@
         _check(lib, basis, "basis")
         if basis.numel() != _spectral_basis_floats(n):
             raise RuntimeError(f"pack_cells: basis {tuple(basis.shape)} is not the block of a {n}-node support")
-    tab = lambda ts: (ctypes.c_void_p * cells)(*[t.data_ptr() for t in ts])
+    tab = lambda ts: (ctypes.c_void_p * cells)(*[t.data_ptr() if t.numel() else None for t in ts])
     fin_arr = (ctypes.c_int32 * cells)(*fins)
-    lib.call("eeg_dcrnn_pack_cells", cells, tab(wgs), tab(bgs), tab(wcs), tab(bcs), fin_arr, h, m, tab(packs), _p(basis), n,
-             tab(spacks) if basis is not None else None, _stream(packs[0]))
+    if parts is None:
+        lib.call("eeg_dcrnn_pack_cells", cells, tab(wgs), tab(bgs), tab(wcs), tab(bcs), fin_arr, h, m, tab(packs), _p(basis), n,
+                 tab(spacks) if basis is not None else None, _stream(packs[0]))
+    else:
+        if len(parts) != cells or (basis is None and any(q & PACK_SPEC for q in parts)):
+            raise RuntimeError(f"pack_cells_parts: parts {list(parts)} for {cells} cells (PACK_SPEC needs a basis)")
+        lib.call("eeg_dcrnn_pack_cells_parts", cells, tab(wgs), tab(bgs), tab(wcs), tab(bcs), fin_arr, h, m, tab(packs), _p(basis), n,
+                 tab(spacks) if basis is not None else None, (ctypes.c_int32 * cells)(*[int(q) for q in parts]), _stream(packs[0]))
     return packs + spacks
 
 
-def _pack_cells_fake(wgs, bgs, wcs, bcs, h, m, basis, n):
+def _pack_cells_fake(wgs, bgs, wcs, bcs, h, m, basis, n, parts=None):
     fins = [w.shape[0] // m - h for w in wgs]
     out = [wgs[0].new_empty((_pack_floats(f, h, m),)) for f in fins]
     if basis is not None:
-        out += [wgs[0].new_empty((int(_lib.get_lib().query("eeg_dcrnn_spectral_pack_floats", f, h, m, n)),)) for f in fins]
+        out += [wgs[0].new_empty((int(_lib.get_lib().query("eeg_dcrnn_spectral_pack_floats", f, h, m, n))
+                                  if (parts is None or parts[c] & PACK_SPEC) else 0,)) for c, f in enumerate(fins)]
     return out
 
 
 _define("pack_cells", "(Tensor[] wg, Tensor[] bg, Tensor[] wc, Tensor[] bc, int h, int m, Tensor? basis, int n) -> Tensor[]",
+        _pack_cells_impl, _pack_cells_fake)
+_define("pack_cells_parts", "(Tensor[] wg, Tensor[] bg, Tensor[] wc, Tensor[] bc, int h, int m, Tensor? basis, int n, int[] parts) -> Tensor[]",
         _pack_cells_impl, _pack_cells_fake)
 
 
@@ -437,7 +452,7 @@
 
 
 def _dcgru_layer_impl(x, x_off: int, h0, p, p_batched: int, wg, bg, wc, bc, lengths, x_planes, n: int, h: int, m: int,
-                      act: int, save: bool, want_hsel: bool, basis=None, pack=None, spack=None):
+                      act: int, save: bool, want_hsel: bool, basis=None, pack=None, spack=None, gather_hsel: bool = True):
     lib = _lib.get_lib()
     if x.dim() != 4 or x.shape[2] != n:
         raise RuntimeError(f"inputs have shape {tuple(x.shape)}, expected (T, B, num_nodes={n}, input_dim)")
@@ -529,7 +544,8 @@
     if lengths is not None:
         lengths = lengths.to(device=x.device, dtype=torch.int64).contiguous()
         hsel = _new((b, n * h), x)
-        lib.call("eeg_dcrnn_gather_last", _p(hext[1:]), _p(lengths), t_len, b, n * h, _p(hsel), _stream(x))
+        if gather_hsel:
+            lib.call("eeg_dcrnn_gather_last", _p(hext[1:]), _p(lengths), t_len, b, n * h, _p(hsel), _stream(x))
     elif want_hsel:
         hsel = hext[t_len].clone()
     else:
@@ -541,7 +557,7 @@
 
 
 def _dcgru_layer_fake(x, x_off, h0, p, p_batched, wg, bg, wc, bc, lengths, x_planes, n, h, m, act, save, want_hsel, basis=None,
-                      pack=None, spack=None):
+                      pack=None, spack=None, gather_hsel=True):
     t_len, b, fin = x.shape[0] - x_off, x.shape[1], x.shape[3]
     ne = lambda *shape: x.new_empty(shape)
     hext, hsel = ne(t_len + 1, b, n * h), (ne(b, n * h) if (want_hsel or lengths is not None) else ne(0))
@@ -619,7 +635,8 @@
 
 _define("dcgru_layer",
         "(Tensor x, int x_off, Tensor? h0, Tensor P, int p_batched, Tensor wg, Tensor bg, Tensor wc, Tensor bc, Tensor? lengths, "
-        "Tensor? x_planes, int n, int h, int m, int act, bool save, bool want_hsel, Tensor? basis, Tensor? pack=None, Tensor? spack=None) -> "
+        "Tensor? x_planes, int n, int h, int m, int act, bool save, bool want_hsel, Tensor? basis, Tensor? pack=None, Tensor? spack=None, "
+        "bool gather_hsel=True) -> "
         "(Tensor hext, Tensor hsel, Tensor[] saved)",
         _dcgru_layer_impl, _dcgru_layer_fake)
 _define("dcgru_layer_bwd",
@@ -631,7 +648,7 @@
 
 
 def _dcgru_layer_setup(ctx, inputs, output):
-    (x, x_off, h0, p, p_batched, wg, bg, wc, bc, lengths, x_planes, n, h, m, act, save, want_hsel, basis, _pack, _spack) = inputs
+    (x, x_off, h0, p, p_batched, wg, bg, wc, bc, lengths, x_planes, n, h, m, act, save, want_hsel, basis, _pack, _spack) = inputs[:20]
     hext, _, saved = output
     ctx.set_materialize_grads(False)
     ctx.saved_ok = bool(save) and len(saved) == 10
@@ -664,7 +681,7 @@
                                                   basis, spack if basis is not None else None)
     ret = [None if t is not None else g for t, g in zip(sunk, bufs)]
     grads = (dx if need_dx else None, None, dh0 if need_dh0 else None, None, None, *ret, None, None, None, None, None, None, None, None,
-             None, None, None)
+             None, None, None, None)
     return grads[:len(ctx.needs_input_grad)]
 
 
@@ -944,6 +961,53 @@
     return loss, logits, arg, dlogits, dz
 
 
+def _cls_head_loss_gather_impl(htop, lengths, n: int, w, bias, targets, kind: int, dropout_p: float, rng_used, clip_w, denom, ticket, dw, db):
+    lib = _lib.get_lib()
+    w, bias = w.detach().contiguous(), bias.detach().contiguous()
+    for t, nm in ((htop, "top layer sequence"), (w, "fc.weight"), (bias, "fc.bias"), (dw, "fc.weight gradient"), (db, "fc.bias gradient")):
+        _check(lib, t, nm)
+    if htop.dim() != 3 or not htop.is_contiguous() or n < 1 or htop.shape[2] % n != 0:
+        raise RuntimeError(f"cls_head_loss_gather: the top layer's sequence has shape {tuple(htop.shape)}, expected contiguous (T, B, "
+                           f"num_nodes*rnn_units) with num_nodes={n}")
+    t_len, b, h = htop.shape[0], htop.shape[1], htop.shape[2] // n
+    c = w.shape[0]
+    if tuple(w.shape) != (c, h) or bias.numel() != c or tuple(dw.shape) != (c, h) or db.numel() != c or not dw.is_contiguous() or not db.is_contiguous():
+        raise RuntimeError(f"cls_head_loss_gather: fc operands {tuple(w.shape)}, {tuple(bias.shape)}, gradients {tuple(dw.shape)}, {tuple(db.shape)} "
+                           f"do not fit a head input of {h} units")
+    _check_lengths(lengths, b)
+    lengths = lengths.to(device=htop.device, dtype=torch.int64).contiguous()
+    if ticket.dtype != torch.int64 or ticket.numel() != 1 or ticket.device != htop.device:
+        raise RuntimeError(f"cls_head_loss_gather: ticket must be one int64 on {htop.device}, got {ticket.dtype} {tuple(ticket.shape)} on {ticket.device}")
+    if kind == 0:
+        tg = targets.to(torch.float32).contiguous().view(-1)
+        _check(lib, tg, "targets")
+    else:
+        tg = targets.to(torch.int64).contiguous().view(-1)
+        _check(lib, tg, "targets", torch.int64)
+    if tg.numel() != b:
+        raise RuntimeError(f"cls_head_loss_gather: {tg.numel()} targets for {b} clips")
+    drop = dropout_p > 0
+    if drop:
+        if rng_used is None:
+            raise RuntimeError("cls_head_loss_gather: dropout_p > 0 needs rng_used (ops.rng_take)")
+        _check_rng(lib, rng_used, "rng_used")
+    if clip_w is not None:
+        clip_w, denom = _clip_weights("cls_head_loss", clip_w, denom, b, htop)
+    loss, logits, arg = _new((1,), htop), _new((b, c), htop), _new((b, c), htop, torch.int32)
+    dlogits, dz = _new((b, c), htop), _new((b, n, h), htop)
+    ws = _new((lib.query("eeg_dcrnn_cls_head_loss_ws_floats", b, h, c),), htop)
+    lib.call("eeg_dcrnn_cls_head_loss_gather", _p(htop), _p(lengths), t_len, _p(w), _p(bias), _p(tg), int(kind), b, n, h, c, float(dropout_p),
+             _p(rng_used) if drop else None, _p(clip_w), _p(denom) if clip_w is not None else None, _p(logits), _p(arg), _p(dlogits), _p(dz),
+             _p(dw), _p(db), _p(loss), _p(ws), _p(ticket), _stream(htop))
+    return loss, logits, arg, dlogits, dz
+
+
+def _cls_head_loss_gather_fake(htop, lengths, n, w, bias, targets, kind, dropout_p, rng_used, clip_w, denom, ticket, dw, db):
+    b, c, h = htop.shape[1], w.shape[0], htop.shape[2] // n
+    return (htop.new_empty((1,)), htop.new_empty((b, c)), htop.new_empty((b, c), dtype=torch.int32), htop.new_empty((b, c)),
+            htop.new_empty((b, n, h)))
+
+
 def _cls_head_loss_w_impl(z, w, bias, targets, kind: int, dropout_p: float, rng_used, clip_w, denom, dw, db):
     return _cls_head_loss_impl(z, w, bias, targets, kind, dropout_p, rng_used, dw, db, clip_w, denom)
 
@@ -955,6 +1019,9 @@
 
 _define("cls_head_loss", "(Tensor z, Tensor w, Tensor bias, Tensor targets, int kind, float dropout_p, Tensor? rng_used, Tensor(a!) dw, Tensor(b!) db) "
         "-> (Tensor, Tensor, Tensor, Tensor, Tensor)", _cls_head_loss_impl, _cls_head_loss_fake)
+_define("cls_head_loss_gather", "(Tensor htop, Tensor lengths, int n, Tensor w, Tensor bias, Tensor targets, int kind, float dropout_p, Tensor? rng_used, "
+        "Tensor? clip_w, Tensor? denom, Tensor(a!) ticket, Tensor(b!) dw, Tensor(c!) db) -> (Tensor, Tensor, Tensor, Tensor, Tensor)",
+        _cls_head_loss_gather_impl, _cls_head_loss_gather_fake)
 _define("cls_head_loss_w", "(Tensor z, Tensor w, Tensor bias, Tensor targets, int kind, float dropout_p, Tensor? rng_used, Tensor clip_w, Tensor denom, "
         "Tensor(a!) dw, Tensor(b!) db) -> (Tensor, Tensor, Tensor, Tensor, Tensor)", _cls_head_loss_w_impl,
         lambda z, w, bias, targets, kind, dropout_p, rng_used, clip_w, denom, dw, db: _cls_head_loss_fake(z, w, bias, targets, kind, dropout_p, rng_used, dw, db))
@@ -1654,22 +1721,34 @@
         return self.hext[1:]
 
 
-def pack_encoder_cells(cells, basis, num_nodes):
+def pack_encoder_cells(cells, basis, num_nodes, t_len=None, batch=None, p_batched=0, x_requires_grad=False):
     cells = list(cells)
     if len(cells) < 2 or len(cells) > 4 or GEMM_MODE != 0:
         return None
     h, m = cells[0]._num_units, cells[0].num_matrices
     if basis is not None and h != 64:
         basis = None
-    out = torch.ops.eeg_dcrnn.pack_cells([c.dconv_gate.weight.detach() for c in cells], [c.dconv_gate.biases.detach() for c in cells],
-                                         [c.dconv_candidate.weight.detach() for c in cells], [c.dconv_candidate.biases.detach() for c in cells],
-                                         h, m, basis, int(num_nodes))
+    tensors = ([c.dconv_gate.weight.detach() for c in cells], [c.dconv_gate.biases.detach() for c in cells],
+               [c.dconv_candidate.weight.detach() for c in cells], [c.dconv_candidate.biases.detach() for c in cells])
     k = len(cells)
-    return out[:k], (out[k:] if basis is not None else [None] * k)
+    if t_len is None or batch is None:
+        out = torch.ops.eeg_dcrnn.pack_cells(*tensors, h, m, basis, int(num_nodes))
+        return out[:k], (out[k:] if basis is not None else [None] * k), [None] * k
+    lib = _lib.get_lib()
+    parts, x_grad = [], torch.is_grad_enabled() and bool(x_requires_grad)
+    for c in cells:
+        fin = c.dconv_gate.weight.shape[0] // m - h
+        dims = _layer_dims(int(t_len), int(batch), int(num_nodes), h, fin, m, 0, int(p_batched), False)
+        parts.append(int(lib.query("eeg_dcrnn_pack_parts", ctypes.byref(dims), 1 if basis is not None else 0, 1 if x_grad else 0, 0)))
+        x_grad = torch.is_grad_enabled() and (x_grad or any(q.requires_grad for q in c.parameters()))
+    if basis is not None and not any(q & PACK_SPEC for q in parts):
+        basis = None
+    out = torch.ops.eeg_dcrnn.pack_cells_parts(*tensors, h, m, basis, int(num_nodes), parts)
+    return out[:k], ([s_ if s_.numel() else None for s_ in out[k:]] if basis is not None else [None] * k), parts
 
 
 def dcgru_layer_ex(x, x_off, h0, p, p_batched, wg, bg, wc, bc, n, h, m, activation="tanh", lengths=None, x_planes=None,
-                   want_hsel=True, basis=None, pack=None, spack=None) -> LayerOut:
+                   want_hsel=True, basis=None, pack=None, spack=None, pack_parts=None, gather_hsel=True) -> LayerOut:
     act = ACT_CODES.get(activation, 1)
     save = torch.is_grad_enabled() and any(t is not None and t.requires_grad for t in (x, h0, wg, bg, wc, bc))
     if basis is not None:
@@ -1682,6 +1761,10 @@
                 x_planes = None
             global spectral_layer_calls
             spectral_layer_calls += 1
+    if pack is not None and pack_parts is not None:
+        reads = PACK_RECUR | (PACK_SPEC if basis is not None else PACK_X)
+        if (reads & ~int(pack_parts)) or (basis is not None and spack is None):
+            pack, spack = None, None
     if basis is None and x_planes is not None and x_planes.dim() != 5:
         x_planes = None
     if x_planes is not None:
@@ -1689,7 +1772,7 @@
         hop_plane_handovers += 1
     hext, hsel, saved = torch.ops.eeg_dcrnn.dcgru_layer(x, int(x_off), h0, p, int(p_batched), wg, bg, wc, bc, lengths, x_planes,
                                                         n, h, m, act, save, bool(want_hsel), basis, pack,
-                                                        spack if basis is not None else None)
+                                                        spack if basis is not None else None, bool(gather_hsel))
     return LayerOut(hext, hsel, saved[7].detach() if (save and saved[7].numel()) else None)
 
 
@@ -1771,6 +1854,26 @@
     return loss[0], logits, dz
 
 
+def cls_head_loss_seq(htop, lengths, num_nodes, fc_weight, fc_bias, targets, ticket, task="detection", dropout_p=0.0, rng_state=None,
+                      clip_w=None, denom=None):
+    _weights_together("cls_head_loss", clip_w, denom, htop)
+    used = rng_take(rng_state, htop.shape[1] * htop.shape[2] // 4) if dropout_p > 0 else None
+    sunk = [GradSink.take(q) for q in (fc_weight, fc_bias)]
+    dw = sunk[0] if sunk[0] is not None else torch.empty_like(fc_weight)
+    db = sunk[1] if sunk[1] is not None else torch.empty_like(fc_bias)
+    loss, logits, _arg, _dl, dz = torch.ops.eeg_dcrnn.cls_head_loss_gather(htop.detach(), lengths, int(num_nodes), fc_weight.detach(),
+                                                                           fc_bias.detach(), targets, 0 if task == "detection" else 1,
+                                                                           float(dropout_p), used, clip_w, denom, ticket, dw, db)
+    for q, buf, sk in ((fc_weight, dw, sunk[0]), (fc_bias, db, sunk[1])):
+        if sk is None and q.requires_grad:
+            q.grad = buf if q.grad is None else q.grad + buf
+    return loss[0], logits, dz
+
+
+def head_ticket(device) -> torch.Tensor:
+    return torch.zeros(1, device=device, dtype=torch.int64)
+
+
 def rng_take(rng_state, groups):
     if rng_state is None:
         raise RuntimeError("dropout_p > 0 needs a device generator state (ops.make_rng_state)")
diff --git a/eeg_gnn_ssl_amd/train_step.py b/eeg_gnn_ssl_amd/train_step.py
--- a/eeg_gnn_ssl_amd/train_step.py
+++ b/eeg_gnn_ssl_amd/train_step.py
@@ -74,6 +74,8 @@
         self.last_scale = None
         self.fused_head = True
         self.last_logits = None
+        self.one_launch_head = True
+        self.head_ticket = ops.head_ticket(dev)
         self.data_augment = bool(data_augment)
         self.feature_std = None if feature_std is None else float(feature_std)
         self.swap_perm, self.reflected_supports, self._augment_rng = None, None, None
@@ -206,8 +208,16 @@
                 out = self.model(x, y, supports, batches_seen=self.samples_seen)
         elif self.fused_head and hasattr(self.model, "encode_last"):
             m = self.model
+            drop_p = m._drop_p()
+            if self.one_launch_head and seq_lengths is not None and hasattr(m, "encode_top"):
+                top, last = m.encode_top(x, seq_lengths, supports)
+                with self.fp.sink:
+                    loss, self.last_logits, dz = ops.cls_head_loss_seq(top, seq_lengths, m.num_nodes, m.fc.weight, m.fc.bias, y, self.head_ticket,
+                                                                       self.task, drop_p, m._rng_state(last.device) if drop_p > 0 else None,
+                                                                       clip_w=clip_w, denom=denom)
+                    last.backward(dz)
+                return loss.detach()
             last = m.encode_last(x, seq_lengths, supports)
-            drop_p = m._drop_p()
             with self.fp.sink:
                 loss, self.last_logits, dz = ops.cls_head_loss(last, m.fc.weight, m.fc.bias, y, self.task, drop_p,
                                                                m._rng_state(last.device) if drop_p > 0 else None, clip_w=clip_w, denom=denom)
diff --git a/include/eeg_dcrnn.h b/include/eeg_dcrnn.h
--- a/include/eeg_dcrnn.h
+++ b/include/eeg_dcrnn.h
@@ -95,6 +95,14 @@
                          int N, float* const* spacks, void* stream);
 int eeg_dcrnn_spectral_ok(const eeg_layer_dims* d, int need_dx);
 size_t eeg_dcrnn_spectral_rows(size_t S);
+#define EEG_PACK_RECUR 1
+#define EEG_PACK_X 2
+#define EEG_PACK_DEC 4
+#define EEG_PACK_SPEC 8
+int eeg_dcrnn_pack_parts(const eeg_layer_dims* d, int spectral, int need_dx, int decoder);
+int eeg_dcrnn_pack_cells_parts(int n_cells, const float* const* Wg, const float* const* bg, const float* const* Wc,
+                               const float* const* bc, const int32_t* Fin, int H, int M, float* const* packs, const float* basis,
+                               int N, float* const* spacks, const int32_t* parts, void* stream);
 
 int eeg_dcrnn_diffuse_fwd(const float* X, const float* P, int p_batched, int S, int B, int N, int F,
                           int M, float* planes, void* stream);
@@ -175,6 +183,10 @@
                               int H, int C, float dropout_p, const uint64_t* rng_used, const float* clip_w, const float* denom,
                               float* logits, int32_t* arg, float* dlogits, float* dz, float* dW, float* dbias, float* loss, float* ws,
                               void* stream);
+int eeg_dcrnn_cls_head_loss_gather(const float* Htop, const int64_t* lengths, int T, const float* W, const float* bias,
+                                   const void* targets, int kind, int B, int N, int H, int C, float dropout_p, const uint64_t* rng_used,
+                                   const float* clip_w, const float* denom, float* logits, int32_t* arg, float* dlogits, float* dz,
+                                   float* dW, float* dbias, float* loss, float* ws, uint64_t* ticket, void* stream);
 int eeg_dcrnn_dropout_mask(const uint64_t* rng_used, size_t n, float dropout_p, float* mask, void* stream);
 
 int eeg_dcrnn_bce_logits(const float* logits, const float* y, int B, float* loss, float* dlogits, void* stream);
```
